# DegardinBruno/Kinetic-GAN

Measured on AMD Instinct MI355X. Metric: G+D train-step samples/sec, NTU (N,3,64,25) bs=64 at 1/2/4/8 MI355X, higher is better.
Workload: dtype f32; 1 GPU; ntu shapes (N,3,64,25), 60 classes, mlp4, G+D WGAN-GP iteration, 64 samples/GPU; global_batch=64, parallelism=dp1, launch=hipgraph

## Files before the change

### include/kgan_hip.h

```cpp
#ifndef KGAN_HIP_H
#define KGAN_HIP_H

#include <stdint.h>

#ifdef __cplusplus
extern "C" {
#endif

#define KG_ABI_VERSION 9

enum { KG_ACT_NONE = 0, KG_ACT_LRELU = 1, KG_ACT_TANH = 2 };
enum { KG_TAP_TIME = 0,
       KG_TAP_CHANBLOCK = 1  };

int         kg_abi_version(void);
const char* kg_arch(void);
const char* kg_last_error(void);
void        kg_reload_env(void);

typedef struct KgConvGroup {
    const float* x;  int64_t x_sN, x_sC;
    int32_t Cin, T_in, V_in;
    int32_t x_lead;
    const int32_t* vmap;
// ... 191 lines not shown
    const float* coef;
    const float* wg;  const float* wr;  const float* wt;  const float* b;  const float* u;
    KgPlane du, dr, gyc, zf, gx;
    KgPlane px, pu, pr;  const float* pnoise;  int32_t pact;
    const float* pmean_t;  const float* prstd_t;  const float* pgamma_t;
    const float* pmean_r;  const float* prstd_r;  const float* pgamma_r;
    float* pcoef;  float* dgamma_t;  float* dbeta_t;  float* dgamma_r;  float* dbeta_r;  float* dnw;
    float* ws;  int64_t ws_bytes;  int32_t* counters;  int32_t counters_len;
} KgGenBlockBwdArgs;
int64_t kg_genblock_lds_bytes(const KgGenBlockArgs* a);
int64_t kg_genblock_workspace_bytes(const KgGenBlockArgs* a);
int     kg_genblock_fwd(const KgGenBlockArgs* a, void* stream);
int64_t kg_genblock_bwd_lds_bytes(const KgGenBlockBwdArgs* a);
int64_t kg_genblock_bwd_workspace_bytes(const KgGenBlockBwdArgs* a);
int     kg_genblock_bwd(const KgGenBlockBwdArgs* a, void* stream);

typedef struct KgRowsumArgs {
    int32_t N, C, T, V;
    const float* x;  int64_t x_sN, x_sC;
    const float* y;  int64_t y_sN, y_sC;
    const float* shift;
    int32_t want_second;
    float* out;
    float* ws;  int64_t ws_bytes;
    int32_t accumulate;
    float* out2;
} KgRowsumArgs;

int64_t kg_rowsum_workspace_bytes(const KgRowsumArgs* a);
int     kg_rowsum(const KgRowsumArgs* a, void* stream);
int64_t kg_rowsum_many_workspace_bytes(const KgRowsumArgs* jobs, int32_t njobs);
int     kg_rowsum_many(const KgRowsumArgs* jobs, int32_t njobs, float* ws, int64_t ws_bytes, void* stream);

typedef struct KgEltArgs {
    int32_t N, C, T, V;
    const float* x;  int64_t x_sN, x_sC;
    const float* r;  int64_t r_sN, r_sC;
    const float* noise;
    const float* sx; const float* bx; const float* sr; const float* br; const float* nw;
    float* out;  int64_t o_sN, o_sC;
    int32_t act;  float slope;
    int32_t groups;
    int64_t coef_gs;
} KgEltArgs;

int kg_act_bwd(const KgEltArgs* a, void* stream);
int kg_affine_act(const KgEltArgs* a, void* stream);

typedef struct KgBnArgs {
    int32_t N, C, T, V;
    const float* x;  int64_t x_sN, x_sC;
    const float* g;  int64_t g_sN, g_sC;
    const float* gamma; const float* beta;
    float* running_mean; float* running_var;
    int64_t* num_batches_tracked;
    const float* mean; const float* rstd;
    float momentum, eps;
    int32_t training;
    float* coef;
} KgBnArgs;

int kg_bn_fwd(const KgBnArgs* a, void* stream);
int kg_bn_bwd(const KgBnArgs* a, void* stream);

typedef struct KgBnJob {
    KgBnArgs a;
    int32_t groups;
} KgBnJob;

int64_t kg_bn_bwd_many_workspace_bytes(const KgBnArgs* jobs, int32_t njobs);
int     kg_bn_bwd_many(const KgBnArgs* jobs, int32_t njobs, float* ws, int64_t ws_bytes, int32_t* counters,
                       int32_t counters_len, void* stream);
int64_t kg_bn_fwd_many_workspace_bytes(const KgBnJob* jobs, int32_t njobs);
int     kg_bn_fwd_many(const KgBnJob* jobs, int32_t njobs, float* ws, int64_t ws_bytes, int32_t* counters,
                       int32_t counters_len, void* stream);

typedef struct KgGpArgs {
    int32_t N, C, T, V;
    const float* g;  int64_t g_sN, g_sC;
    float* nrm;
    float* gp;
    const float* gout;
    float* out;  int64_t o_sN, o_sC;
} KgGpArgs;

int kg_gp_fwd(const KgGpArgs* a, void* stream);
int kg_gp_bwd(const KgGpArgs* a, void* stream);

int kg_adam_step(float* p, const float* g, float* m, float* v, int64_t n,
                 float lr, float b1, float b2, float eps, const int32_t* step, float grad_scale,
                 void* stream);
int kg_adam_step_fused(float* p, float* g, float* m, float* v, int64_t n,
                       float lr, float b1, float b2, float eps, const int32_t* step, float grad_scale,
                       int32_t zero_grad, void* stream);
int kg_adam_step_ema(float* p, float* g, float* m, float* v, float* e, int64_t n,
                     float lr, float b1, float b2, float eps, const int32_t* step, float grad_scale,
                     int32_t zero_grad, float ema_decay, float ema_warmup, void* stream);

typedef struct KgHeadArgs {
    int32_t N, C, T, V;
    const float* h;  int64_t h_sN, h_sC;
    const float* w;  const float* b;
    float* v;
    const float* gv;
    float* g;  int64_t g_sN, g_sC;
    float slope;  int32_t masked;
    float* dw;  float* db;  int32_t accumulate;
} KgHeadArgs;
int kg_head_fwd(const KgHeadArgs* a, void* stream);
int kg_head_bwd(const KgHeadArgs* a, void* stream);
int kg_head_wgrad(const KgHeadArgs* a, void* stream);

typedef struct KgLabelBiasArgs {
    int32_t N, L, J, K, C, V, W, T;
    const int64_t* labels;
    const float* emb;
    const float* w;  int64_t w_sK, w_sC;
    const float* ak;
    float* zl;
    const float* gz;  int64_t gz_sN, gz_sC;
    float* demb;  float* dw;  int32_t accumulate;
    float* dak;  int32_t dak_accumulate;
    float* ws;  int64_t ws_bytes;
} KgLabelBiasArgs;
int     kg_label_bias_fwd(const KgLabelBiasArgs* a, void* stream);
int64_t kg_label_bias_workspace_bytes(const KgLabelBiasArgs* a);
int     kg_label_bias_bwd(const KgLabelBiasArgs* a, void* stream);
int     kg_aggconv_label(const KgAggConvArgs* a, const KgLabelBiasArgs* lb, void* stream);

typedef struct KgMixArgs {
    int32_t N, C, T, V;
    const float* real;  int64_t r_sN, r_sC;
    const float* fake;  int64_t f_sN, f_sC;
    const float* alpha;
    float* out;  int64_t o_sN, o_sC;
} KgMixArgs;
int kg_mix3(const KgMixArgs* a, void* stream);

typedef struct KgMaskedAdjArgs {
    int32_t n;
    const float* a;  const float* imp;  const int64_t* sel;
    float* ak;
    const float* g;  float* dimp;  int32_t accumulate;
} KgMaskedAdjArgs;
int kg_masked_adj_fwd(const KgMaskedAdjArgs* a, void* stream);
int kg_masked_adj_bwd(const KgMaskedAdjArgs* a, void* stream);

typedef struct KgLinearArgs {
    int32_t N, Din, Dout;
    int32_t L, J;
    const float* x;  int64_t x_ld;
    const float* emb;
    const int64_t* labels;
    const float* w;  const float* bias;
    float* y;  int64_t y_ld;
    int32_t act;  float slope;
    const float* g;  int64_t g_ld;
    float* gx;  int64_t gx_ld;  int32_t gx_cols;
    float* dw;  float* db;
    float* demb;
    int32_t accumulate;
} KgLinearArgs;
int kg_linear_fwd(const KgLinearArgs* a, void* stream);
int kg_linear_bwd(const KgLinearArgs* a, void* stream);
int kg_embed_bwd(const KgLinearArgs* a, void* stream);

#define KG_COMM_ID_BYTES 128
int kg_comm_unique_id(void* id);
int kg_comm_init(void** comm, int32_t rank, int32_t world, const void* id, int32_t device);
int kg_comm_world(const void* comm);
int kg_allreduce_flat(void* comm, float* buf, int64_t n, void* stream);
int kg_comm_destroy(void* comm);

int kg_peak_mfma_f32(float* sink, int32_t iters, double* flops, void* stream);
int kg_peak_copy(const float* src, float* dst, int64_t n, void* stream);

#define KG_MMD_MAX_BW 16
typedef struct KgMmdArgs {
    const float* x;  int64_t x_sp, x_sd, x_sg, x_sc;
    const float* y;  int64_t y_sp, y_sd, y_sg, y_sc;
    int32_t m, n, dim;
    int32_t groups, classes;
    int32_t nbw;
    double bw[KG_MMD_MAX_BW];
    float* mmd2;
    float* mmd;
    float* result;
    float* mean;
    void* ws;  int64_t ws_bytes;
} KgMmdArgs;
int64_t kg_mmd_workspace_bytes(const KgMmdArgs* a);
int     kg_mmd(const KgMmdArgs* a, void* stream);

#define KG_PRDC_MAX_K 32
#define KG_PRDC_MAX_POINTS 32768
typedef struct KgPrdcArgs {
    const float* real;  int64_t r_sc, r_sp, r_so;
    const float* fake;  int64_t f_sc, f_sp, f_so;
    int32_t n, m;
    int32_t d_outer, d_inner;
    int32_t classes, k;
    float* radii_real;
    float* radii_fake;
    int32_t* fake_hits;
    uint8_t* real_flags;
    int32_t* counts;
    float* values;
    float* mean;
    void* ws;  int64_t ws_bytes;
} KgPrdcArgs;
int64_t kg_prdc_workspace_bytes(const KgPrdcArgs* a);
int     kg_prdc(const KgPrdcArgs* a, void* stream);

#define KG_PRDC_MAX_SETS 4
typedef struct KgPrdcRadiiArgs {
    const float* x;  int64_t sc, sp, so;
    int32_t n, d_outer, d_inner, classes, k;
    float* radii;
} KgPrdcRadiiArgs;
typedef struct KgPrdcSetsArgs {
    const float* real;  int64_t r_sc, r_sp, r_so;
    const float* fake[KG_PRDC_MAX_SETS];  int64_t f_sc, f_sp, f_so;
    int32_t nsets;
    int32_t n, m;
    int32_t d_outer, d_inner;
    int32_t classes, k;
    const float* radii_real;
    float* radii_fake;
    int32_t* fake_hits;
    uint8_t* real_flags;
    int32_t* counts;
    float* values;
    float* mean;
    void* ws;  int64_t ws_bytes;
} KgPrdcSetsArgs;
int     kg_prdc_radii(const KgPrdcRadiiArgs* a, void* stream);
int64_t kg_prdc_sets_workspace_bytes(const KgPrdcSetsArgs* a);
int     kg_prdc_sets(const KgPrdcSetsArgs* a, void* stream);

#define KG_NN_MAX_K 32
#define KG_NN_MAX_POINTS 16777216
#define KG_NN_MAX_SPLIT 32
typedef struct KgNnArgs {
    const float* query;  int64_t q_sc, q_sp, q_so;
// ... 221 lines not shown
```

### kinetic-gan_amd/_native.py

```python
from __future__ import annotations

import ctypes as C
import os
from typing import NamedTuple, Optional, Sequence, Tuple

import torch

_PKG = os.path.dirname(os.path.abspath(__file__))
LIB_PATH = os.environ.get("KG_LIB") or os.path.join(_PKG, "libkgan_hip.so")

ACT_NONE, ACT_LRELU, ACT_TANH = 0, 1, 2
ABI_VERSION = 9
TAP_TIME, TAP_CHANBLOCK = 0, 1

c_f32p = C.c_void_p
c_i32p = C.c_void_p


class _ConvGroup(C.Structure):
    _fields_ = [("x", c_f32p), ("x_sN", C.c_int64), ("x_sC", C.c_int64),
                ("Cin", C.c_int32), ("T_in", C.c_int32), ("V_in", C.c_int32),
                ("x_lead", C.c_int32),
                ("vmap", c_i32p),
                ("w", c_f32p), ("w_sT", C.c_int64), ("w_sO", C.c_int64), ("w_sI", C.c_int64),
# ... 39 lines not shown
    _fields_ = [("ws", c_f32p), ("dw", c_f32p), ("w_sT", C.c_int64), ("w_sO", C.c_int64), ("w_sI", C.c_int64),
                ("taps", C.c_int32), ("M", C.c_int32), ("Cin", C.c_int32), ("splits", C.c_int32),
                ("accumulate", C.c_int32)]


WGRAD_REDUCE_MAX_JOBS = 24
WGRAD_TILE_128x128, WGRAD_TILE_64x64, WGRAD_TILE_64x32, WGRAD_TILE_32x64, WGRAD_TILE_32x32 = 0, 1, 2, 3, 4
WGRAD_TILE_NAMES = {WGRAD_TILE_128x128: "128x128", WGRAD_TILE_64x64: "64x64", WGRAD_TILE_64x32: "64x32",
                    WGRAD_TILE_32x64: "32x64", WGRAD_TILE_32x32: "32x32"}
WGRAD_MAX_SPLITS = 128


class _WgradReduceJobs(C.Structure):
    _fields_ = [("njobs", C.c_int32), ("job", _WgradReduceJob * WGRAD_REDUCE_MAX_JOBS)]


class _AggArgs(C.Structure):
    _fields_ = [("N", C.c_int32), ("C", C.c_int32), ("K", C.c_int32), ("V", C.c_int32), ("W", C.c_int32),
                ("T", C.c_int32), ("rep", C.c_int32),
                ("a", c_f32p),
                ("x", c_f32p), ("x_sN", C.c_int64), ("x_sC", C.c_int64),
                ("y", c_f32p), ("y_sN", C.c_int64), ("y_sC", C.c_int64),
                ("out", c_f32p), ("o_sN", C.c_int64), ("o_sC", C.c_int64),
                ("ws", c_f32p), ("ws_bytes", C.c_int64), ("a_transposed", C.c_int32), ("defer_sum", C.c_int32),
                ("res", c_f32p), ("r_sN", C.c_int64), ("r_sC", C.c_int64), ("r_T", C.c_int32), ("r_V", C.c_int32),
                ("r_tstride", C.c_int32), ("r_inv", c_i32p),
                ("mask", c_f32p), ("m_sN", C.c_int64), ("m_sC", C.c_int64), ("slope", C.c_float)]


class _OuterSumJob(C.Structure):
    _fields_ = [("ws", c_f32p), ("out", c_f32p), ("nout", C.c_int32), ("slabs", C.c_int32)]


OUTER_SUM_MAX_JOBS = 16


class _OuterSumJobs(C.Structure):
    _fields_ = [("njobs", C.c_int32), ("job", _OuterSumJob * OUTER_SUM_MAX_JOBS)]


class _AggConvArgs(C.Structure):
    _fields_ = [("N", C.c_int32), ("Cin", C.c_int32), ("M", C.c_int32), ("T", C.c_int32), ("V", C.c_int32),
                ("W", C.c_int32), ("K", C.c_int32),
                ("x", c_f32p), ("x_sN", C.c_int64), ("x_sC", C.c_int64),
                ("a", c_f32p), ("a_transposed", C.c_int32),
                ("nbr", c_i32p), ("pcount", C.c_int32 * 3),
                ("w", c_f32p), ("w_sT", C.c_int64), ("w_sO", C.c_int64), ("w_sI", C.c_int64),
                ("out", c_f32p), ("o_sN", C.c_int64), ("o_sC", C.c_int64),
                ("add", c_f32p), ("a_sN", C.c_int64), ("a_sC", C.c_int64), ("a_tstride", C.c_int32),
                ("xa", c_f32p), ("xa_sN", C.c_int64), ("xa_sC", C.c_int64)]


class _RowsumArgs(C.Structure):
    _fields_ = [("N", C.c_int32), ("C", C.c_int32), ("T", C.c_int32), ("V", C.c_int32),
                ("x", c_f32p), ("x_sN", C.c_int64), ("x_sC", C.c_int64),
                ("y", c_f32p), ("y_sN", C.c_int64), ("y_sC", C.c_int64),
                ("shift", c_f32p),
                ("want_second", C.c_int32),
                ("out", c_f32p),
                ("ws", c_f32p), ("ws_bytes", C.c_int64), ("accumulate", C.c_int32), ("out2", c_f32p)]


class _BnArgs(C.Structure):
    _fields_ = [("N", C.c_int32), ("C", C.c_int32), ("T", C.c_int32), ("V", C.c_int32),
                ("x", c_f32p), ("x_sN", C.c_int64), ("x_sC", C.c_int64),
                ("g", c_f32p), ("g_sN", C.c_int64), ("g_sC", C.c_int64),
                ("gamma", c_f32p), ("beta", c_f32p),
                ("running_mean", c_f32p), ("running_var", c_f32p),
                ("num_batches_tracked", C.c_void_p),
                ("mean", c_f32p), ("rstd", c_f32p),
                ("momentum", C.c_float), ("eps", C.c_float),
                ("training", C.c_int32),
                ("coef", c_f32p)]


class _BnJob(C.Structure):
    _fields_ = [("a", _BnArgs), ("groups", C.c_int32)]


class _GpArgs(C.Structure):
    _fields_ = [("N", C.c_int32), ("C", C.c_int32), ("T", C.c_int32), ("V", C.c_int32),
                ("g", c_f32p), ("g_sN", C.c_int64), ("g_sC", C.c_int64),
                ("nrm", c_f32p), ("gp", c_f32p), ("gout", c_f32p),
                ("out", c_f32p), ("o_sN", C.c_int64), ("o_sC", C.c_int64)]


class _EltArgs(C.Structure):
    _fields_ = [("N", C.c_int32), ("C", C.c_int32), ("T", C.c_int32), ("V", C.c_int32),
                ("x", c_f32p), ("x_sN", C.c_int64), ("x_sC", C.c_int64),
                ("r", c_f32p), ("r_sN", C.c_int64), ("r_sC", C.c_int64),
                ("noise", c_f32p),
                ("sx", c_f32p), ("bx", c_f32p), ("sr", c_f32p), ("br", c_f32p), ("nw", c_f32p),
                ("out", c_f32p), ("o_sN", C.c_int64), ("o_sC", C.c_int64),
                ("act", C.c_int32), ("slope", C.c_float),
                ("groups", C.c_int32), ("coef_gs", C.c_int64)]


class _GenArgs(C.Structure):
    _fields_ = [("N", C.c_int32), ("C", C.c_int32), ("K", C.c_int32), ("Cr", C.c_int32), ("Tc", C.c_int32),
                ("Vc", C.c_int32), ("V", C.c_int32), ("rep", C.c_int32),
                ("a", c_f32p), ("u", c_f32p), ("b", c_f32p),
                ("y", c_f32p), ("y_out", c_f32p), ("y_sN", C.c_int64), ("y_sC", C.c_int64),
                ("z", c_f32p), ("z_sN", C.c_int64), ("z_sC", C.c_int64),
                ("zf", c_f32p), ("zf_sN", C.c_int64), ("zf_sC", C.c_int64),
                ("rs", c_f32p), ("rs_out", c_f32p), ("rs_sN", C.c_int64), ("rs_sC", C.c_int64),
                ("rbias", c_f32p),
                ("r", c_f32p), ("r_sN", C.c_int64), ("r_sC", C.c_int64)]


class _GenAdjJob(C.Structure):
    _fields_ = [("dbt", c_f32p), ("u", c_f32p), ("a", c_f32p), ("out", c_f32p),
                ("K", C.c_int32), ("Kd", C.c_int32), ("V", C.c_int32), ("Vc", C.c_int32), ("accumulate", C.c_int32)]


class _HeadArgs(C.Structure):
    _fields_ = [("N", C.c_int32), ("C", C.c_int32), ("T", C.c_int32), ("V", C.c_int32),
                ("h", c_f32p), ("h_sN", C.c_int64), ("h_sC", C.c_int64),
                ("w", c_f32p), ("b", c_f32p), ("v", c_f32p), ("gv", c_f32p),
                ("g", c_f32p), ("g_sN", C.c_int64), ("g_sC", C.c_int64),
                ("slope", C.c_float), ("masked", C.c_int32),
                ("dw", c_f32p), ("db", c_f32p), ("accumulate", C.c_int32)]


class _LinearArgs(C.Structure):
    _fields_ = [("N", C.c_int32), ("Din", C.c_int32), ("Dout", C.c_int32), ("L", C.c_int32), ("J", C.c_int32),
                ("x", c_f32p), ("x_ld", C.c_int64), ("emb", c_f32p), ("labels", C.c_void_p),
                ("w", c_f32p), ("bias", c_f32p), ("y", c_f32p), ("y_ld", C.c_int64),
                ("act", C.c_int32), ("slope", C.c_float),
                ("g", c_f32p), ("g_ld", C.c_int64),
                ("gx", c_f32p), ("gx_ld", C.c_int64), ("gx_cols", C.c_int32),
                ("dw", c_f32p), ("db", c_f32p), ("demb", c_f32p), ("accumulate", C.c_int32)]


class _LabelBiasArgs(C.Structure):
    _fields_ = [("N", C.c_int32), ("L", C.c_int32), ("J", C.c_int32), ("K", C.c_int32), ("C", C.c_int32),
                ("V", C.c_int32), ("W", C.c_int32), ("T", C.c_int32),
                ("labels", C.c_void_p), ("emb", c_f32p),
                ("w", c_f32p), ("w_sK", C.c_int64), ("w_sC", C.c_int64),
                ("ak", c_f32p), ("zl", c_f32p),
                ("gz", c_f32p), ("gz_sN", C.c_int64), ("gz_sC", C.c_int64),
                ("demb", c_f32p), ("dw", c_f32p), ("accumulate", C.c_int32),
                ("dak", c_f32p), ("dak_accumulate", C.c_int32),
                ("ws", c_f32p), ("ws_bytes", C.c_int64)]


class _MixArgs(C.Structure):
    _fields_ = [("N", C.c_int32), ("C", C.c_int32), ("T", C.c_int32), ("V", C.c_int32),
                ("real", c_f32p), ("r_sN", C.c_int64), ("r_sC", C.c_int64),
                ("fake", c_f32p), ("f_sN", C.c_int64), ("f_sC", C.c_int64),
                ("alpha", c_f32p),
                ("out", c_f32p), ("o_sN", C.c_int64), ("o_sC", C.c_int64)]


class _MaskedAdjArgs(C.Structure):
    _fields_ = [("n", C.c_int32), ("a", c_f32p), ("imp", c_f32p), ("sel", C.c_void_p), ("ak", c_f32p),
                ("g", c_f32p), ("dimp", c_f32p), ("accumulate", C.c_int32)]


class _GenTailArgs(C.Structure):
    _fields_ = [("N", C.c_int32), ("C", C.c_int32), ("T", C.c_int32), ("V", C.c_int32), ("act", C.c_int32), ("slope", C.c_float),
                ("g", c_f32p), ("g_sN", C.c_int64), ("g_sC", C.c_int64),
                ("out", c_f32p), ("o_sN", C.c_int64), ("o_sC", C.c_int64),
                ("u", c_f32p), ("u_sN", C.c_int64), ("u_sC", C.c_int64), ("mean_t", c_f32p), ("rstd_t", c_f32p), ("gamma_t", c_f32p),
                ("r", c_f32p), ("r_sN", C.c_int64), ("r_sC", C.c_int64), ("mean_r", c_f32p), ("rstd_r", c_f32p), ("gamma_r", c_f32p),
                ("noise", c_f32p), ("coef", c_f32p),
                ("dgamma_t", c_f32p), ("dbeta_t", c_f32p), ("dgamma_r", c_f32p), ("dbeta_r", c_f32p), ("dnw", c_f32p),
                ("ws", c_f32p), ("ws_bytes", C.c_int64), ("counters", C.c_void_p), ("counters_len", C.c_int32),
                ("du", c_f32p), ("du_sN", C.c_int64), ("du_sC", C.c_int64),
                ("dr", c_f32p), ("dr_sN", C.c_int64), ("dr_sC", C.c_int64)]


class _GenPrepJob(C.Structure):
    _fields_ = [("a", c_f32p), ("imp", c_f32p), ("u", c_f32p), ("aeff", c_f32p), ("b", c_f32p),
                ("K", C.c_int32), ("V", C.c_int32), ("Vc", C.c_int32)]


class _Plane(C.Structure):
    _fields_ = [("p", c_f32p), ("sN", C.c_int64), ("sC", C.c_int64)]


class _GenBnLayer(C.Structure):
    _fields_ = [("gamma", c_f32p), ("beta", c_f32p), ("running_mean", c_f32p), ("running_var", c_f32p),
                ("num_batches_tracked", C.c_void_p), ("momentum", C.c_float), ("eps", C.c_float), ("coef", c_f32p)]


class _GenBlockArgs(C.Structure):
    _fields_ = [("N", C.c_int32), ("groups", C.c_int32),
                ("Cin", C.c_int32), ("C", C.c_int32), ("K", C.c_int32), ("Kp", C.c_int32),
                ("Tc", C.c_int32), ("Vc", C.c_int32), ("T", C.c_int32), ("V", C.c_int32), ("rep", C.c_int32),
                ("res_kind", C.c_int32), ("bn_t", C.c_int32), ("act", C.c_int32), ("slope", C.c_float),
                ("x", _Plane),
                ("pu", _Plane), ("pr", _Plane), ("pcoef_t", c_f32p), ("pcoef_r", c_f32p), ("pnoise", c_f32p), ("pnw", c_f32p),
                ("pact", C.c_int32), ("xout", _Plane),
                ("wg", c_f32p), ("wr", c_f32p), ("br", c_f32p), ("wt", c_f32p), ("bt", c_f32p),
                ("b", c_f32p), ("u", c_f32p),
                ("yc", _Plane), ("z", _Plane), ("r", _Plane), ("uo", _Plane),
                ("bt_", _GenBnLayer), ("br_", _GenBnLayer),
                ("noise", c_f32p), ("nw", c_f32p), ("out", _Plane),
                ("ws", c_f32p), ("ws_bytes", C.c_int64), ("counters", C.c_void_p), ("counters_len", C.c_int32)]


class _GenBlockBwdArgs(C.Structure):
    _fields_ = [("N", C.c_int32),
                ("Cin", C.c_int32), ("C", C.c_int32), ("K", C.c_int32), ("Kp", C.c_int32),
                ("Tc", C.c_int32), ("Vc", C.c_int32), ("T", C.c_int32), ("V", C.c_int32), ("rep", C.c_int32),
                ("res_kind", C.c_int32), ("bn_t", C.c_int32), ("act", C.c_int32), ("slope", C.c_float),
                ("g", _Plane), ("out", _Plane), ("uo", _Plane), ("r", _Plane),
                ("coef", c_f32p),
                ("wg", c_f32p), ("wr", c_f32p), ("wt", c_f32p), ("b", c_f32p), ("u", c_f32p),
                ("du", _Plane), ("dr", _Plane), ("gyc", _Plane), ("zf", _Plane), ("gx", _Plane),
                ("px", _Plane), ("pu", _Plane), ("pr", _Plane), ("pnoise", c_f32p), ("pact", C.c_int32),
                ("pmean_t", c_f32p), ("prstd_t", c_f32p), ("pgamma_t", c_f32p),
                ("pmean_r", c_f32p), ("prstd_r", c_f32p), ("pgamma_r", c_f32p),
                ("pcoef", c_f32p), ("dgamma_t", c_f32p), ("dbeta_t", c_f32p), ("dgamma_r", c_f32p), ("dbeta_r", c_f32p),
                ("dnw", c_f32p),
                ("ws", c_f32p), ("ws_bytes", C.c_int64), ("counters", C.c_void_p), ("counters_len", C.c_int32)]



MMD_MAX_BW = 16


class _MmdArgs(C.Structure):
    _fields_ = [("x", c_f32p), ("x_sp", C.c_int64), ("x_sd", C.c_int64), ("x_sg", C.c_int64), ("x_sc", C.c_int64),
                ("y", c_f32p), ("y_sp", C.c_int64), ("y_sd", C.c_int64), ("y_sg", C.c_int64), ("y_sc", C.c_int64),
                ("m", C.c_int32), ("n", C.c_int32), ("dim", C.c_int32),
                ("groups", C.c_int32), ("classes", C.c_int32), ("nbw", C.c_int32),
                ("bw", C.c_double * MMD_MAX_BW),
                ("mmd2", c_f32p), ("mmd", c_f32p), ("result", c_f32p), ("mean", c_f32p),
                ("ws", C.c_void_p), ("ws_bytes", C.c_int64)]

PRDC_MAX_K = 32
PRDC_MAX_POINTS = 32768


class _PrdcArgs(C.Structure):
    _fields_ = [("real", c_f32p), ("r_sc", C.c_int64), ("r_sp", C.c_int64), ("r_so", C.c_int64),
                ("fake", c_f32p), ("f_sc", C.c_int64), ("f_sp", C.c_int64), ("f_so", C.c_int64),
                ("n", C.c_int32), ("m", C.c_int32), ("d_outer", C.c_int32), ("d_inner", C.c_int32),
# ... 1255 lines not shown

def rowsum_many(jobs: Sequence[dict]):
    lib = load_library()
    if not jobs:
        return
    arr = (_RowsumArgs * len(jobs))()
    held = []
    for i, j in enumerate(jobs):
        x = as_plane(j["x"])
        out, out2, y = j["out"], j.get("out2"), j.get("y")
        _need_cuda(x, out, out2)
        for o in (out, out2):
            if o is not None:
                _dest(o, x.shape[1], "rowsum_many: destinations must be contiguous fp32 vectors of C elements")
        _need_cuda(y)
        held.append(_rowsum_fill(arr[i], x, y, 0 if y is None else 2, out, out2, int(bool(j.get("accumulate", False)))))
    ws = _workspace("kg_rowsum_many_workspace_bytes", arr, jobs[0]["x"].device, len(jobs))
    _check(lib.kg_rowsum_many(arr, len(jobs), ws.data_ptr(), ws.numel() * 4, _stream()), "kg_rowsum_many")


def _elt_args(x, out, act, slope):
    a = _EltArgs()
    a.N, a.C, a.T, a.V = x.shape
    _bind(a, "x", "x", x)
    _bind(a, "out", "o", out)
    a.act, a.slope = act, slope
    return a


def act_bwd(g: torch.Tensor, ref: torch.Tensor, act: int, slope: float = 0.2) -> torch.Tensor:
    lib = load_library()
    g = as_plane(g)
    ref = as_plane(ref)
    _need_cuda(g, ref)
    out = new_plane(*g.shape, g.device)
    a = _elt_args(g, out, act, slope)
    _bind(a, "r", "r", ref)
    _check(lib.kg_act_bwd(C.byref(a), _stream()), "kg_act_bwd")
    return out


def affine_act(x, sx=None, bx=None, r=None, sr=None, br=None, noise=None, nw=None,
               act: int = ACT_NONE, slope: float = 0.2, out: Optional[torch.Tensor] = None,
               groups: int = 1, coef_gs: int = 0) -> torch.Tensor:
    lib = load_library()
    x = as_plane(x)
    vecs = [None if t is None else t.reshape(-1).contiguous() for t in (sx, bx, sr, br, nw)]
    _need_cuda(x, r, noise, out, *vecs)
    if out is None:
        out = new_plane(*x.shape, x.device)
    elif tuple(out.shape) != tuple(x.shape) or not is_plane(out) or out.dtype != torch.float32:
        raise ValueError("affine_act: out must be a plane tensor of x's shape")
    a = _elt_args(x, out, act, slope)
    if r is not None:
        r = _bind(a, "r", "r", r, True)
    if noise is not None:
        noise = noise.contiguous()
        a.noise = noise.data_ptr()
    a.sx, a.bx, a.sr, a.br, a.nw = [_ptr(t) for t in vecs]
    a.groups, a.coef_gs = int(groups), int(coef_gs)
    _check(lib.kg_affine_act(C.byref(a), _stream()), "kg_affine_act")
    return out


def _gp_args(g):
    a = _GpArgs()
    a.N, a.C, a.T, a.V = g.shape
    _bind(a, "g", "g", g)
    return a


def gp_fwd(g: torch.Tensor):
    lib = load_library()
    g = as_plane(g)
    _need_cuda(g)
    a = _gp_args(g)
    nrm = torch.empty(g.shape[0], dtype=torch.float32, device=g.device)
    gp = torch.empty((), dtype=torch.float32, device=g.device)
    a.nrm, a.gp = nrm.data_ptr(), gp.data_ptr()
    _check(lib.kg_gp_fwd(C.byref(a), _stream()), "kg_gp_fwd")
    return nrm, gp


def gp_bwd(g: torch.Tensor, nrm: torch.Tensor, gout: torch.Tensor) -> torch.Tensor:
    lib = load_library()
    g = as_plane(g)
    gout = gout.reshape(1).contiguous()
    _need_cuda(g, nrm, gout)
    a = _gp_args(g)
    a.nrm, a.gout = nrm.data_ptr(), gout.data_ptr()
    out = _bind(a, "out", "o", new_plane(*g.shape, g.device))
    _check(lib.kg_gp_bwd(C.byref(a), _stream()), "kg_gp_bwd")
    return out


def _vec(t: Optional[torch.Tensor], c: int, what: str):
    return None if t is None else _dest(t, c, f"{what}: expected a contiguous fp32 vector of {c} elements")


def _bn_fwd_fill(a, who: str, x, gamma, beta, running_mean, running_var, nbt, momentum, eps, training, groups: Optional[int] = None):
    n, c, t, v = x.shape
    vecs = [_vec(q, c, who) for q in (gamma, beta, running_mean, running_var)]
    _need_cuda(x, *vecs, nbt)
    a.N, a.C, a.T, a.V = n // (groups or 1), c, t, v
    _bind(a, "x", "x", x)
    a.gamma, a.beta, a.running_mean, a.running_var = [_ptr(q) for q in vecs]
    if nbt is not None:
        assert nbt.dtype == torch.int64
        a.num_batches_tracked = nbt.data_ptr()
    a.momentum, a.eps, a.training = float(momentum), float(eps), int(bool(training))
    coef = torch.empty((4, c) if groups is None else (groups, 4, c), dtype=torch.float32, device=x.device)
    a.coef = coef.data_ptr()
    return coef


def bn_fwd(x: torch.Tensor, gamma, beta, running_mean, running_var, num_batches_tracked, training: bool,
           momentum: float, eps: float) -> torch.Tensor:
    lib = load_library()
    x = as_plane(x)
    a = _BnArgs()
    coef = _bn_fwd_fill(a, "bn_fwd", x, gamma, beta, running_mean, running_var, num_batches_tracked, momentum, eps, training)
    _check(lib.kg_bn_fwd(C.byref(a), _stream()), "kg_bn_fwd")
    return coef


def _bn_many(who: str, arr, coefs):
    total_c = sum(cf.shape[-1] for cf in coefs)
    if total_c > SYNC_LEN:
        raise ValueError("%s: %d channels exceed the %d ticket counters" % (who, total_c, SYNC_LEN))
    ws = _workspace("kg_%s_workspace_bytes" % who, arr, coefs[0].device if coefs else None, len(arr))
    sync = _sync_buffer(coefs[0].device)
    _check(getattr(load_library(), "kg_" + who)(arr, len(arr), ws.data_ptr(), ws.numel() * 4, sync.data_ptr(), sync.numel(),
                                               _stream()), "kg_" + who)
    return coefs


def bn_fwd_many(jobs: Sequence[dict]):
    arr = (_BnJob * len(jobs))()
    xs, coefs = [], []
    for i, j in enumerate(jobs):
        x = as_plane(j["x"])
        groups = int(j.get("groups", 1))
        if x.shape[0] % groups:
            raise ValueError("bn_fwd_many: N=%d is not a multiple of groups=%d" % (x.shape[0], groups))
        coefs.append(_bn_fwd_fill(arr[i].a, "bn_fwd_many", x, j.get("gamma"), j.get("beta"), j.get("running_mean"),
                                  j.get("running_var"), j.get("num_batches_tracked"), j["momentum"], j["eps"], True, groups))
        arr[i].groups = groups
        xs.append(x)
    return _bn_many("bn_fwd_many", arr, coefs)


def _bn_bwd_fill(a, who: str, g, x, gamma, mean, rstd, training):
    g, x = as_plane(g), as_plane(x)
    n, c, t, v = x.shape
    gamma, mean, rstd = _vec(gamma, c, who), _vec(mean, c, who), _vec(rstd, c, who)
    _need_cuda(g, x, gamma, mean, rstd)
    a.N, a.C, a.T, a.V = n, c, t, v
    _bind(a, "x", "x", x)
    _bind(a, "g", "g", g)
    a.gamma, a.mean, a.rstd = _ptr(gamma), _ptr(mean), _ptr(rstd)
    a.training = int(bool(training))
    coef = torch.empty((5, c), dtype=torch.float32, device=x.device)
    a.coef = coef.data_ptr()
    return coef, (g, x)


def bn_bwd(g: torch.Tensor, x: torch.Tensor, gamma, mean: torch.Tensor, rstd: torch.Tensor, training: bool) -> torch.Tensor:
    lib = load_library()
    a = _BnArgs()
    coef, held = _bn_bwd_fill(a, "bn_bwd", g, x, gamma, mean, rstd, training)
    _check(lib.kg_bn_bwd(C.byref(a), _stream()), "kg_bn_bwd")
    return coef


def bn_bwd_many(jobs: Sequence[dict]):
    arr = (_BnArgs * len(jobs))()
    filled = [_bn_bwd_fill(arr[i], "bn_bwd_many", j["g"], j["x"], j.get("gamma"), j["mean"], j["rstd"], j["training"])
              for i, j in enumerate(jobs)]
    return _bn_many("bn_bwd_many", arr, [coef for coef, _ in filled])


def adam_step(p, g, m, v, lr, b1, b2, eps, step_t: torch.Tensor, grad_scale: float = 1.0, zero_grad: bool = False):
    lib = load_library()
    _need_cuda(p, g, m, v, step_t)
    assert p.is_contiguous() and g.is_contiguous() and m.is_contiguous() and v.is_contiguous()
    assert step_t.dtype == torch.int32
    if zero_grad:
        _check(lib.kg_adam_step_fused(p.data_ptr(), g.data_ptr(), m.data_ptr(), v.data_ptr(), p.numel(), lr, b1, b2, eps,
                                      step_t.data_ptr(), grad_scale, 1, _stream()), "kg_adam_step_fused")
        return
    _check(lib.kg_adam_step(p.data_ptr(), g.data_ptr(), m.data_ptr(), v.data_ptr(), p.numel(),
                            lr, b1, b2, eps, step_t.data_ptr(), grad_scale, _stream()), "kg_adam_step")


def adam_step_ema(p, g, m, v, e, lr, b1, b2, eps, step_t: torch.Tensor, grad_scale: float, zero_grad: bool, decay: float,
                  warmup: float):
    lib = load_library()
    _need_cuda(p, g, m, v, e, step_t)
    assert p.is_contiguous() and g.is_contiguous() and m.is_contiguous() and v.is_contiguous() and e.is_contiguous()
    assert g.numel() == m.numel() == v.numel() == e.numel() == p.numel() and e.dtype == torch.float32
    assert step_t.dtype == torch.int32
    _check(lib.kg_adam_step_ema(p.data_ptr(), g.data_ptr(), m.data_ptr(), v.data_ptr(), e.data_ptr(), p.numel(), lr, b1, b2, eps,
                                step_t.data_ptr(), grad_scale, 1 if zero_grad else 0, decay, warmup, _stream()),
           "kg_adam_step_ema")



def _head_args(h, w=None, gv=None):
    a = _HeadArgs()
    h = _bind(a, "h", "h", h, True)
    a.N, a.C, a.T, a.V = h.shape
    if w is not None:
        w = w.reshape(-1)
        assert w.is_contiguous() and w.numel() == h.shape[1]
        a.w = w.data_ptr()
    if gv is not None:
        assert gv.numel() == h.shape[0]
        a.gv = gv.data_ptr()
    return a, h


def head_fwd(h: torch.Tensor, w: torch.Tensor, b: Optional[torch.Tensor]) -> torch.Tensor:
    lib = load_library()
    _need_cuda(h, w, b)
    a, h = _head_args(h, w)
    a.b = _ptr(b)
    v = torch.empty(h.shape[0], dtype=torch.float32, device=h.device)
    a.v = v.data_ptr()
    _check(lib.kg_head_fwd(C.byref(a), _stream()), "kg_head_fwd")
    return v


def head_bwd(gv: torch.Tensor, w: torch.Tensor, h: torch.Tensor, masked: bool = True, slope: float = 0.2) -> torch.Tensor:
    lib = load_library()
    gv = gv.reshape(-1).contiguous()
    _need_cuda(gv, w, h)
    a, h = _head_args(h, w, gv)
    a.masked, a.slope = int(bool(masked)), slope
    g = _bind(a, "g", "g", new_plane(*h.shape, h.device))
    _check(lib.kg_head_bwd(C.byref(a), _stream()), "kg_head_bwd")
    return g


def head_wgrad(x: torch.Tensor, gv: torch.Tensor, dw: torch.Tensor, db: Optional[torch.Tensor], accumulate: bool = True):
    lib = load_library()
    gv = gv.reshape(-1).contiguous()
    _need_cuda(x, gv, dw, db)
    a, x = _head_args(x, None, gv)
    assert dw.is_contiguous() and dw.numel() == x.shape[1] and (db is None or db.numel() == 1)
    a.dw, a.db, a.accumulate = dw.data_ptr(), _ptr(db), int(bool(accumulate))
    _check(lib.kg_head_wgrad(C.byref(a), _stream()), "kg_head_wgrad")



def _cls_head_args(n: int, c: int, t: int, v: int, f: int, l: int, slope: float = 0.2) -> _ClsHeadArgs:
    a = _ClsHeadArgs()
    a.N, a.C, a.T, a.V, a.F, a.L, a.slope = int(n), int(c), int(t), int(v), int(f), int(l), float(slope)
    return a


def _cls_flat(t: torch.Tensor, n: int, dtype, what: str) -> torch.Tensor:
    if t.numel() != n or not t.is_contiguous() or t.dtype != dtype:
        raise ValueError(f"kg_cls_head: {what} must be contiguous {dtype} of {n} elements")
    return t


def cls_head_workspace_bytes(n: int, c: int, t: int, v: int, f: int, l: int) -> int:
    return _query("kg_cls_head_workspace_bytes", _cls_head_args(n, c, t, v, f, l))


def cls_head_fwd(h: torch.Tensor, w1: torch.Tensor, b1: torch.Tensor, w2: torch.Tensor, b2: torch.Tensor,
                 labels: Optional[torch.Tensor] = None, slope: float = 0.2, feat_out: Optional[torch.Tensor] = None,
                 pred_out: Optional[torch.Tensor] = None) -> dict:
    lib = load_library()
    _need_cuda(h, w1, b1, w2, b2, labels, feat_out, pred_out)
    f, l = w1.shape[0], w2.shape[0]
    a = _cls_head_args(*h.shape, f, l, slope)
    h = _bind(a, "h", "h", h, True)
    n, c = h.shape[0], h.shape[1]
    a.w1, a.b1 = _cls_flat(w1, f * c, torch.float32, "w1").data_ptr(), _cls_flat(b1, f, torch.float32, "b1").data_ptr()
    a.w2, a.b2 = _cls_flat(w2, l * f, torch.float32, "w2").data_ptr(), _cls_flat(b2, l, torch.float32, "b2").data_ptr()
    dev = h.device
    if feat_out is not None and tuple(feat_out.shape) != (n, f):
        raise ValueError(f"kg_cls_head: feat_out must be ({n}, {f}), got {tuple(feat_out.shape)}")
    if pred_out is not None and tuple(pred_out.shape) != (n,):
        raise ValueError(f"kg_cls_head: pred_out must be ({n},), got {tuple(pred_out.shape)}")
    out = dict(pooled=torch.empty((n, c), dtype=torch.float32, device=dev),
               feat=torch.empty((n, f), dtype=torch.float32, device=dev) if feat_out is None
               else _cls_flat(feat_out, n * f, torch.float32, "feat_out"),
               logits=torch.empty((n, l), dtype=torch.float32, device=dev),
               pred=torch.empty(n, dtype=torch.int32, device=dev) if pred_out is None
               else _cls_flat(pred_out, n, torch.int32, "pred_out"),
               loss_per_sample=None, loss=None, correct=None)
    a.pooled, a.feat, a.logits, a.pred = (out[k].data_ptr() for k in ("pooled", "feat", "logits", "pred"))
    if labels is not None:
        a.labels = _cls_flat(labels, n, torch.int64, "labels").data_ptr()
        out["loss_per_sample"] = torch.empty(n, dtype=torch.float32, device=dev)
        out["loss"] = torch.empty((), dtype=torch.float32, device=dev)
        out["correct"] = torch.empty((), dtype=torch.int32, device=dev)
        a.loss_per_sample, a.loss, a.correct = (out[k].data_ptr() for k in ("loss_per_sample", "loss", "correct"))
    _check(lib.kg_cls_head_fwd(C.byref(a), _stream()), "kg_cls_head_fwd")
    return out


def cls_head_bwd(gtop: torch.Tensor, h: torch.Tensor, w1: torch.Tensor, w2: torch.Tensor, labels: torch.Tensor,
                 feat: torch.Tensor, logits: torch.Tensor, masked: bool = True, slope: float = 0.2):
    lib = load_library()
    _need_cuda(gtop, h, w1, w2, labels, feat, logits)
    f, l = w1.shape[0], w2.shape[0]
    a = _cls_head_args(*h.shape, f, l, slope)
    h = _bind(a, "h", "h", h, True)
    n, c = h.shape[0], h.shape[1]
    a.w1, a.w2 = _cls_flat(w1, f * c, torch.float32, "w1").data_ptr(), _cls_flat(w2, l * f, torch.float32, "w2").data_ptr()
    a.labels = _cls_flat(labels, n, torch.int64, "labels").data_ptr()
    a.feat, a.logits = _cls_flat(feat, n * f, torch.float32, "feat").data_ptr(), _cls_flat(logits, n * l, torch.float32, "logits").data_ptr()
    a.gtop, a.masked = _cls_flat(gtop, 1, torch.float32, "gtop").data_ptr(), int(bool(masked))
    g = _bind(a, "g", "g", new_plane(*h.shape, h.device))
    ws = _workspace("kg_cls_head_workspace_bytes", a, h.device)
    _check(lib.kg_cls_head_bwd(C.byref(a), _stream()), "kg_cls_head_bwd")
    return g, ws

# ... 16 lines not shown

def cls_scores(feats: Sequence[torch.Tensor], preds: Sequence[torch.Tensor], labels: torch.Tensor, div_pairs: torch.Tensor,
               mm_pairs: torch.Tensor, n_classes: int) -> dict:
    lib = load_library()
    feats, preds, k = list(feats), list(preds), int(n_classes)
    s = len(feats)
    if len(preds) != s:
        raise ValueError(f"kg_cls_scores: {s} feature sets, {len(preds)} prediction vectors")
    if not 1 <= s <= CLS_MAX_SETS:
        raise ValueError(f"kg_cls_scores: nsets={s} outside [1, {CLS_MAX_SETS}]")
    _need_cuda(labels, div_pairs, mm_pairs, *feats, *preds)
    n, f = feats[0].shape
    ld = feats[0].stride(0) if n > 1 else max(f, feats[0].stride(0))
    for t in feats:
        if t.dtype != torch.float32 or tuple(t.shape) != (n, f) or (f > 1 and t.stride(1) != 1) or (n > 1 and t.stride(0) != ld):
            raise ValueError(f"kg_cls_scores: every feature set must be fp32 ({n}, {f}) with unit column stride and row stride {ld}")
    preds = [_cls_flat(t, n, torch.int32, "pred") for t in preds]
    labels = _cls_flat(labels, n, torch.int64, "labels")
    if div_pairs.dim() != 2 or div_pairs.shape[1] != 2 or mm_pairs.dim() != 2 or mm_pairs.shape[1] != 2 \
            or mm_pairs.shape[0] % max(k, 1):
        raise ValueError("kg_cls_scores: div_pairs (Sd, 2) and mm_pairs (n_classes * Sl, 2) expected")
    sd, sl = div_pairs.shape[0], mm_pairs.shape[0] // max(k, 1)
    div_pairs = _cls_flat(div_pairs, 2 * sd, torch.int32, "div_pairs")
    mm_pairs = _cls_flat(mm_pairs, 2 * k * sl, torch.int32, "mm_pairs")
    dev = feats[0].device
    out = dict(scores=torch.empty((s, 3), dtype=torch.float32, device=dev),
               scores64=torch.empty((s, 3), dtype=torch.float64, device=dev),
               correct=torch.empty(s, dtype=torch.int32, device=dev),
               correct_per_class=torch.empty((s, max(k, 1)), dtype=torch.int32, device=dev),
               count_per_class=torch.empty(max(k, 1), dtype=torch.int32, device=dev),
               dist=torch.empty((s, max(1, sd + k * sl)), dtype=torch.float64, device=dev))
    a = _ClsScoresArgs()
    a.nsets, a.N, a.F, a.K, a.Sd, a.Sl, a.feat_ld = s, n, f, k, sd, sl, ld
    for g in range(s):
        a.feat[g], a.pred[g] = feats[g].data_ptr(), preds[g].data_ptr()
    a.labels, a.div_pairs, a.mm_pairs = labels.data_ptr(), div_pairs.data_ptr(), mm_pairs.data_ptr()
    for key in ("dist", "scores64", "scores", "correct", "correct_per_class", "count_per_class"):
        setattr(a, key, out[key].data_ptr())
    _count("kg_cls_scores", 3.0 * s * (sd + k * sl) * f)
    _check(lib.kg_cls_scores(C.byref(a), _stream()), "kg_cls_scores")
    return out


def _label_bias_args(labels, emb, wg, K, C_out, cin, J, ak):
    a = _LabelBiasArgs()
    k, v, w = ak.shape
    assert k == K and ak.is_contiguous() and emb.is_contiguous() and labels.dtype == torch.int64 and labels.is_contiguous()
    a.N, a.L, a.J, a.K, a.C, a.V, a.W = labels.numel(), emb.shape[0], J, K, C_out, v, w
    a.labels, a.emb = labels.data_ptr(), emb.data_ptr()
    assert wg.is_contiguous()
    a.w, a.w_sK, a.w_sC = wg.data_ptr(), C_out * cin, cin
    a.ak = ak.data_ptr()
    return a


def label_bias_fwd(labels, emb, wg, K: int, C_out: int, cin: int, J: int, ak) -> torch.Tensor:
    lib = load_library()
    _need_cuda(labels, emb, wg, ak)
    a = _label_bias_args(labels, emb, wg, K, C_out, cin, J, ak)
    zl = torch.empty((labels.numel(), C_out, 1, ak.shape[2]), dtype=torch.float32, device=emb.device)
    a.zl = zl.data_ptr()
    ws = _workspace("kg_label_bias_workspace_bytes", a, emb.device)
    _check(lib.kg_label_bias_fwd(C.byref(a), _stream()), "kg_label_bias_fwd")
    return zl


def label_bias_bwd(gz, labels, emb, wg, K: int, C_out: int, cin: int, J: int, ak, demb=None, dw=None, dak=None,
                   accumulate: bool = True, dak_accumulate: bool = True):
    lib = load_library()
    gz = as_plane(gz)
    _need_cuda(gz, labels, emb, wg, ak, demb, dw, dak)
    a = _label_bias_args(labels, emb, wg, K, C_out, cin, J, ak)
    assert gz.shape[0] == labels.numel() and gz.shape[1] == C_out and gz.shape[3] == ak.shape[2]
    a.T = gz.shape[2]
    _bind(a, "gz", "gz", gz)
    for t in (demb, dw, dak):
        assert t is None or t.is_contiguous()
    a.demb, a.dw, a.dak = _ptr(demb), _ptr(dw), _ptr(dak)
    a.accumulate, a.dak_accumulate = int(bool(accumulate)), int(bool(dak_accumulate))
    ws = _workspace("kg_label_bias_workspace_bytes", a, gz.device)
    _check(lib.kg_label_bias_bwd(C.byref(a), _stream()), "kg_label_bias_bwd")


def mix3(real: torch.Tensor, fake: torch.Tensor, alpha: torch.Tensor) -> torch.Tensor:
    lib = load_library()
    real, fake = as_plane(real), as_plane(fake)
    alpha = alpha.reshape(-1).contiguous()
    _need_cuda(real, fake, alpha)
    n, c, t, v = real.shape
    assert tuple(fake.shape) == (n, c, t, v) and alpha.numel() == n
    out = torch.empty((3 * n, c, t, v), dtype=torch.float32, device=real.device)
    a = _MixArgs()
    a.N, a.C, a.T, a.V = n, c, t, v
    _bind(a, "real", "r", real)
    _bind(a, "fake", "f", fake)
    a.alpha = alpha.data_ptr()
    a.out, a.o_sN, a.o_sC = out.data_ptr(), c * t * v, t * v
    _check(lib.kg_mix3(C.byref(a), _stream()), "kg_mix3")
    return out


def masked_adj_fwd(A_all: torch.Tensor, imp_all: Optional[torch.Tensor], sel: Optional[torch.Tensor]) -> torch.Tensor:
    lib = load_library()
    _need_cuda(A_all, imp_all, sel)
    n = sel.numel() if sel is not None else A_all.numel()
    ak = torch.empty(n, dtype=torch.float32, device=A_all.device)
    a = _MaskedAdjArgs()
    a.n = n
    a.a, a.imp, a.sel, a.ak = A_all.data_ptr(), _ptr(imp_all), _ptr(sel), ak.data_ptr()
    assert A_all.is_contiguous() and (imp_all is None or imp_all.is_contiguous()) and (sel is None or (sel.dtype == torch.int64 and sel.is_contiguous()))
    _check(lib.kg_masked_adj_fwd(C.byref(a), _stream()), "kg_masked_adj_fwd")
    return ak


def masked_adj_bwd(g: torch.Tensor, A_all: torch.Tensor, sel: Optional[torch.Tensor], dimp: torch.Tensor, accumulate: bool):
    lib = load_library()
    g = g.reshape(-1).contiguous()
    _need_cuda(g, A_all, sel, dimp)
    a = _MaskedAdjArgs()
    a.n = g.numel()
    assert dimp.is_contiguous() and dimp.numel() == A_all.numel() and (sel is None or sel.numel() == g.numel())
    a.a, a.sel, a.g, a.dimp, a.accumulate = A_all.data_ptr(), _ptr(sel), g.data_ptr(), dimp.data_ptr(), int(bool(accumulate))
    _check(lib.kg_masked_adj_bwd(C.byref(a), _stream()), "kg_masked_adj_bwd")



def _linear_args(x, w, emb, labels):
    a = _LinearArgs()
    assert w.dim() == 2 and w.is_contiguous()
    a.Dout, a.Din = w.shape
    a.w = w.data_ptr()
    J = 0
    if emb is not None:
        assert emb.dim() == 2 and emb.is_contiguous() and labels is not None and labels.dtype == torch.int64 and labels.is_contiguous()
        a.L, J = emb.shape
        a.emb, a.labels = emb.data_ptr(), labels.data_ptr()
    a.J = J
    assert x.dim() == 2 and x.stride(1) == 1 and x.shape[1] == a.Din - J, (tuple(x.shape), a.Din, J)
    a.N = x.shape[0]
    a.x, a.x_ld = x.data_ptr(), x.stride(0)
    return a


def linear_fwd(x: torch.Tensor, w: torch.Tensor, b: Optional[torch.Tensor], act: int = ACT_LRELU, slope: float = 0.2,
               emb: Optional[torch.Tensor] = None, labels: Optional[torch.Tensor] = None) -> torch.Tensor:
    lib = load_library()
    _need_cuda(x, w, b, emb, labels)
    a = _linear_args(x, w, emb, labels)
    y = torch.empty(a.N, a.Dout, dtype=torch.float32, device=x.device)
    a.bias = _ptr(b)
    a.y, a.y_ld = y.data_ptr(), a.Dout
    a.act, a.slope = act, slope
    _check(lib.kg_linear_fwd(C.byref(a), _stream()), "kg_linear_fwd")
    return y


def linear_bwd(g: torch.Tensor, y: torch.Tensor, x: torch.Tensor, w: torch.Tensor, act: int = ACT_LRELU, slope: float = 0.2,
               emb: Optional[torch.Tensor] = None, labels: Optional[torch.Tensor] = None, gx_cols: Optional[int] = None,
               dw: Optional[torch.Tensor] = None, db: Optional[torch.Tensor] = None, accumulate: bool = False):
    lib = load_library()
    _need_cuda(g, y, x, w, emb, labels, dw, db)
    a = _linear_args(x, w, emb, labels)
    assert g.shape == (a.N, a.Dout) and y.shape == (a.N, a.Dout) and g.stride(1) == 1 and y.stride(1) == 1
    a.g, a.g_ld = g.data_ptr(), g.stride(0)
    a.y, a.y_ld = y.data_ptr(), y.stride(0)
    a.act, a.slope = act, slope
    cols = a.Din if gx_cols is None else gx_cols
    gx = None
    if cols > 0:
        gx = torch.empty(a.N, cols, dtype=torch.float32, device=g.device)
        a.gx, a.gx_ld = gx.data_ptr(), cols
    a.gx_cols = cols
    if dw is not None:
        assert dw.is_contiguous() and dw.numel() == a.Dout * a.Din
    if db is not None:
        assert db.is_contiguous() and db.numel() == a.Dout
    a.dw, a.db, a.accumulate = _ptr(dw), _ptr(db), int(bool(accumulate))
    _check(lib.kg_linear_bwd(C.byref(a), _stream()), "kg_linear_bwd")
    return gx


def embed_bwd(gx: torch.Tensor, labels: torch.Tensor, demb: torch.Tensor, accumulate: bool = False):
    lib = load_library()
    _need_cuda(gx, labels, demb)
    a = _LinearArgs()
    assert gx.dim() == 2 and gx.stride(1) == 1 and demb.dim() == 2 and demb.is_contiguous() and demb.shape[1] <= gx.shape[1]
    assert labels.dtype == torch.int64 and labels.is_contiguous()
    a.N = gx.shape[0]
    a.L, a.J = demb.shape
    a.gx, a.gx_ld = gx.data_ptr(), gx.stride(0)
    a.labels, a.demb, a.accumulate = labels.data_ptr(), demb.data_ptr(), int(bool(accumulate))
    _check(lib.kg_embed_bwd(C.byref(a), _stream()), "kg_embed_bwd")



COMM_ID_BYTES = 128



class MmdView(NamedTuple):
    t: torch.Tensor
    sp: int
    sd: int
    sg: int
    sc: int


def _mmd_extent_ok(v: MmdView, m: int, dim: int, groups: int, classes: int) -> bool:
    if min(v.sp, v.sd, v.sg, v.sc) < 0:
        return False
    last = (classes - 1) * v.sc + (groups - 1) * v.sg + (m - 1) * v.sp + (dim - 1) * v.sd
    return v.t.storage_offset() + last < v.t.untyped_storage().nbytes() // 4


def mmd(x: MmdView, y: MmdView, m: int, n: int, dim: int, groups: int, classes: int,
        bandwidths: Sequence[float], want_mean: bool = False) -> dict:
    lib = load_library()
    for v in (x, y):
        if v.t.dtype != torch.float32:
            raise TypeError(f"kg_mmd: fp32 only, got {v.t.dtype}")
    _need_cuda(x.t, y.t)
    bws = [float(b) for b in bandwidths]
    a = _MmdArgs()
    a.x, a.x_sp, a.x_sd, a.x_sg, a.x_sc = x.t.data_ptr(), x.sp, x.sd, x.sg, x.sc
    a.y, a.y_sp, a.y_sd, a.y_sg, a.y_sc = y.t.data_ptr(), y.sp, y.sd, y.sg, y.sc
    a.m, a.n, a.dim, a.groups, a.classes, a.nbw = int(m), int(n), int(dim), int(groups), int(classes), len(bws)
    for i, b in enumerate(bws[:MMD_MAX_BW]):
        a.bw[i] = b
    nbytes = _query("kg_mmd_workspace_bytes", a)
    for name, v, p in (("x", x, m), ("y", y, n)):
        if not _mmd_extent_ok(v, p, dim, groups, classes):
            raise ValueError(f"kg_mmd: the strides of {name} reach outside its tensor")
    dev = x.t.device
    ws = torch.empty(max(1, nbytes // 4), dtype=torch.float32, device=dev)
    out = dict(mmd2=torch.empty((classes * groups, len(bws)), dtype=torch.float32, device=dev),
               mmd=torch.empty((classes, len(bws)), dtype=torch.float32, device=dev),
               result=torch.empty(classes, dtype=torch.float32, device=dev),
# ... 655 lines not shown
```

### kinetic-gan_amd/csrc/kg_disc.hip

```cpp
#include "kg_common.h"

namespace {

constexpr int NT = 256;

__device__ __forceinline__ float wave_sum(float v) {
#pragma unroll
    for (int off = 32; off > 0; off >>= 1) v += __shfl_down(v, off, 64);
    return v;
}

__device__ __forceinline__ float block_sum(float s, float* red) {
    s = wave_sum(s);
    __syncthreads();
    if ((threadIdx.x & 63) == 0) red[threadIdx.x >> 6] = s;
    __syncthreads();
    float t = 0.f;
    if (threadIdx.x == 0)
        for (int i = 0; i < NT / 64; ++i) t += red[i];
    return t;
}

__global__ __launch_bounds__(NT) void kg_head_fwd_kernel(const KgHeadArgs a) {
    __shared__ float red[NT / 64];
    const int n = blockIdx.x, L = a.T * a.V;
    const float* base = a.h + (long)n * a.h_sN;
    float s = 0.f;
    for (int e = threadIdx.x; e < a.C * L; e += NT) {
        const int c = e / L, r = e - c * L;
        s = fmaf(a.w[c], base[(long)c * a.h_sC + r], s);
    }
    const float t = block_sum(s, red);
    if (threadIdx.x == 0) a.v[n] = t / (float)L + (a.b ? a.b[0] : 0.f);
}

__global__ __launch_bounds__(NT) void kg_head_bwd_kernel(const KgHeadArgs a) {
    const int L = a.T * a.V;
    const long total = (long)a.N * a.C * L;
    const float inv = 1.f / (float)L;
    for (long i = (long)blockIdx.x * NT + threadIdx.x; i < total; i += (long)gridDim.x * NT) {
        const int c = (int)(i / ((long)a.N * L));
        const long rem = i - (long)c * a.N * L;
        const int n = (int)(rem / L), r = (int)(rem - (long)n * L);
        float v = a.gv[n] * a.w[c] * inv;
        if (a.masked) v *= a.h[(long)n * a.h_sN + (long)c * a.h_sC + r] > 0.f ? 1.f : a.slope;
        a.g[(long)n * a.g_sN + (long)c * a.g_sC + r] = v;
    }
}

__global__ __launch_bounds__(NT) void kg_head_wgrad_kernel(const KgHeadArgs a) {
    __shared__ float red[NT / 64];
    const int c = blockIdx.x, L = a.T * a.V;
    float s = 0.f;
    if (c < a.C) {
        for (int e = threadIdx.x; e < a.N * L; e += NT) {
            const int n = e / L, r = e - n * L;
            s = fmaf(a.gv[n], a.h[(long)n * a.h_sN + (long)c * a.h_sC + r], s);
        }
        const float t = block_sum(s, red);
        if (threadIdx.x == 0) a.dw[c] = (a.accumulate ? a.dw[c] : 0.f) + t / (float)L;
    } else {
        for (int n = threadIdx.x; n < a.N; n += NT) s += a.gv[n];
        const float t = block_sum(s, red);
        if (threadIdx.x == 0 && a.db) a.db[0] = (a.accumulate ? a.db[0] : 0.f) + t;
    }
}

constexpr int LB_MAXKW = 3 * 32, LB_MAXKC = 3 * 64, LB_MAXCW = 64 * 32, LB_MAXW = 12288;

__device__ __forceinline__ void colsums(const KgLabelBiasArgs& a, float* S, float* scratch) {
    const int n = a.K * a.V * a.W;
    for (int i = threadIdx.x; i < n; i += NT) scratch[i] = a.ak[i];
    __syncthreads();
    for (int i = threadIdx.x; i < a.K * a.W; i += NT) {
        const int k = i / a.W, w = i - k * a.W;
        float s = 0.f;
        for (int v = 0; v < a.V; ++v) s += scratch[(k * a.V + v) * a.W + w];
        S[i] = s;
    }
    __syncthreads();
}

__device__ __forceinline__ void stage_wc(const KgLabelBiasArgs& a, float* Wl) {
    const int lane = threadIdx.x & 63, wave = threadIdx.x >> 6;
    const int rows = a.K * a.C;
    for (int r0 = wave * 4; r0 < rows; r0 += (NT / 64) * 4) {
        for (int j0 = 0; j0 < a.J; j0 += 64) {
            const int j = j0 + lane;
            float v[4];
#pragma unroll
            for (int q = 0; q < 4; ++q) {
                const int kc = r0 + q;
                const int k = kc / a.C, c = kc - k * a.C;
                v[q] = (kc < rows && j < a.J) ? a.w[(long)k * a.w_sK + (long)c * a.w_sC + j] : 0.f;
            }
#pragma unroll
            for (int q = 0; q < 4; ++q)
                if (r0 + q < rows && j < a.J) Wl[(r0 + q) * a.J + j] = v[q];
        }
    }
}

__global__ __launch_bounds__(NT) void kg_label_bias_table_kernel(const KgLabelBiasArgs a, float* table) {
    __shared__ float S[LB_MAXKW], P[LB_MAXKC], El[512], Wl[LB_MAXW];
    const int l = blockIdx.x;
    colsums(a, S, Wl);
    stage_wc(a, Wl);
    for (int j = threadIdx.x; j < a.J; j += NT) El[j] = a.emb[(long)l * a.J + j];
    __syncthreads();
    for (int i = threadIdx.x; i < a.K * a.C; i += NT) {
        const float* wp = Wl + i * a.J;
        float s0 = 0.f, s1 = 0.f, s2 = 0.f, s3 = 0.f;
        int j = 0;
        for (; j + 3 < a.J; j += 4) {
            s0 = fmaf(wp[j], El[j], s0);
            s1 = fmaf(wp[j + 1], El[j + 1], s1);
            s2 = fmaf(wp[j + 2], El[j + 2], s2);
            s3 = fmaf(wp[j + 3], El[j + 3], s3);
        }
        for (; j < a.J; ++j) s0 = fmaf(wp[j], El[j], s0);
        P[i] = (s0 + s1) + (s2 + s3);
    }
    __syncthreads();
    for (int i = threadIdx.x; i < a.C * a.W; i += NT) {
        const int c = i / a.W, w = i - c * a.W;
        float s = 0.f;
        for (int k = 0; k < a.K; ++k) s = fmaf(S[k * a.W + w], P[k * a.C + c], s);
        table[(long)l * a.C * a.W + i] = s;
    }
}

__global__ __launch_bounds__(NT) void kg_label_bias_lookup_kernel(const KgLabelBiasArgs a, const float* table) {
    const int CW = a.C * a.W;
    const int i = blockIdx.x * NT + threadIdx.x;
    if (i >= a.N * CW) return;
    const int n = i / CW, e = i - n * CW;
    const long lab = a.labels[n];
    a.zl[i] = (lab >= 0 && lab < a.L) ? table[lab * CW + e] : __builtin_nanf("");
}

__host__ __device__ __forceinline__ long lb_rec(const KgLabelBiasArgs& a) { return 2L * a.K * a.C + (long)a.C * a.W; }

constexpr int LB_BATCH = 4;

__global__ __launch_bounds__(NT) void kg_label_bias_bwd_class_kernel(const KgLabelBiasArgs a) {
    __shared__ float S[LB_MAXKW], El[512], Wr[3 * 512], red[LB_BATCH][NT], dT[NT], Pk[3];
    __shared__ int lst[NT], wcnt[NT / 64];
    extern __shared__ float kg_lbsm[];
// ... 76 lines not shown
        rec[tid * a.C + c] = s;
        rec[a.K * a.C + tid * a.C + c] = Pk[tid];
    }
}

__global__ __launch_bounds__(NT) void kg_label_bias_bwd_finish_kernel(const KgLabelBiasArgs a) {
    extern __shared__ float kg_lbsm[];
    const int b = blockIdx.x, tid = threadIdx.x;
    const long per = lb_rec(a);
    if (b < a.L) {
        if (!a.demb) return;
        float* Wl = kg_lbsm;
        __shared__ float Q[LB_MAXKC];
        stage_wc(a, Wl);
        for (int i = tid; i < a.K * a.C; i += NT) Q[i] = a.ws[b * per + i];
        __syncthreads();
        for (int j = tid; j < a.J; j += NT) {
            float s = 0.f;
#pragma unroll 8
            for (int i = 0; i < a.K * a.C; ++i) s = fmaf(Wl[i * a.J + j], Q[i], s);
            float* d = a.demb + (long)b * a.J + j;
            *d = (a.accumulate ? *d : 0.f) + s;
        }
        return;
    }
    if (b < a.L + a.K * a.W) {
        if (!a.dak) return;
        __shared__ float R[NT];
        __shared__ float tot;
        const int kw = b - a.L;
        const int k = kw / a.W, w = kw - k * a.W;
        float s = 0.f;
        for (int l0 = 0; l0 < a.L; l0 += NT) {
            const int l = l0 + tid;
            if (l < a.L) {
                const float* rec = a.ws + l * per;
                float r = 0.f;
#pragma unroll 8
                for (int c = 0; c < a.C; ++c) r = fmaf(rec[2 * a.K * a.C + c * a.W + w], rec[a.K * a.C + k * a.C + c], r);
                R[tid] = r;
            }
            __syncthreads();
            if (tid == 0) {
                const int nl = a.L - l0 < NT ? a.L - l0 : NT;
                for (int i = 0; i < nl; ++i) s += R[i];
            }
            __syncthreads();
        }
        if (tid == 0) tot = s;
        __syncthreads();
        for (int v = tid; v < a.V; v += NT) {
            float* d = a.dak + ((long)k * a.V + v) * a.W + w;
            *d = (a.dak_accumulate ? *d : 0.f) + tot;
        }
        return;
    }
    const int i = (b - a.L - a.K * a.W) * NT + tid;
    if (!a.dw || i >= a.K * a.C * a.J) return;
    const int kc = i / a.J, j = i - kc * a.J;
    float s = 0.f;
#pragma unroll 8
    for (int l = 0; l < a.L; ++l) s = fmaf(a.emb[(long)l * a.J + j], a.ws[l * per + kc], s);
    const int k = kc / a.C, c = kc - k * a.C;
    float* d = a.dw + (long)k * a.w_sK + (long)c * a.w_sC + j;
    *d = (a.accumulate ? *d : 0.f) + s;
}

__global__ __launch_bounds__(NT) void kg_mix3_kernel(const KgMixArgs a) {
    const int L = a.T * a.V;
    const long per = (long)a.C * L;
    const long total = (long)a.N * per;
    for (long i = (long)blockIdx.x * NT + threadIdx.x; i < total; i += (long)gridDim.x * NT) {
        const int n = (int)(i / per);
        const long rem = i - (long)n * per;
        const int c = (int)(rem / L), r = (int)(rem - (long)c * L);
        const float x = a.real[(long)n * a.r_sN + (long)c * a.r_sC + r];
        const float f = a.fake[(long)n * a.f_sN + (long)c * a.f_sC + r];
        const float al = a.alpha[n];
        float* o = a.out + (long)c * a.o_sC + r;
        o[(long)n * a.o_sN] = x;
        o[(long)(n + a.N) * a.o_sN] = f;
        o[(long)(n + 2 * a.N) * a.o_sN] = al * x + (1.f - al) * f;
    }
}

__global__ __launch_bounds__(NT) void kg_masked_adj_kernel(const KgMaskedAdjArgs a, const int backward) {
    const int i = blockIdx.x * NT + threadIdx.x;
    if (i >= a.n) return;
    const long s = a.sel ? a.sel[i] : i;
    if (!backward) {
        a.ak[i] = a.a[s] * (a.imp ? a.imp[s] : 1.f);
    } else {
        const float v = a.g[i] * a.a[s];
        a.dimp[s] = (a.accumulate ? a.dimp[s] : 0.f) + v;
    }
}

int validate_head(const KgHeadArgs* a, const char* who) {
    KG_REQUIRE(a != nullptr, "%s: null args", who);
    KG_REQUIRE(a->N > 0 && a->C > 0 && a->T > 0 && a->V > 0, "%s: bad dims", who);
    KG_REQUIRE((long)a->N * a->C * a->T * a->V < (1L << 31), "%s: too large", who);
    return 0;
}

int validate_lb(const KgLabelBiasArgs* a, const char* who) {
    KG_REQUIRE(a != nullptr, "%s: null args", who);
    KG_REQUIRE(a->N > 0 && a->L > 0 && a->J > 0 && a->K >= 1 && a->K <= 3 && a->C > 0 && a->V > 0 && a->W > 0, "%s: bad dims", who);
    KG_REQUIRE(a->K * a->W <= LB_MAXKW && a->K * a->C <= LB_MAXKC && a->C * a->W <= LB_MAXCW && a->J <= 512 &&
               a->K * a->C * a->J <= LB_MAXW && a->W <= NT && a->K * a->V * a->W <= LB_MAXW,
               "%s: K=%d C=%d W=%d J=%d exceed the kernel's LDS tables", who, a->K, a->C, a->W, a->J);
    KG_REQUIRE(a->labels && a->emb && a->w && a->ak, "%s: null pointer", who);
    return 0;
}

}

extern "C" int kg_head_fwd(const KgHeadArgs* a, void* stream) {
    if (int rc = validate_head(a, "kg_head_fwd")) return rc;
    KG_REQUIRE(a->h && a->w && a->v, "kg_head_fwd: null pointer");
    hipLaunchKernelGGL(kg_head_fwd_kernel, dim3(a->N), dim3(NT), 0, (hipStream_t)stream, *a);
    return kg_launch_status("kg_head_fwd");
}

extern "C" int kg_head_bwd(const KgHeadArgs* a, void* stream) {
    if (int rc = validate_head(a, "kg_head_bwd")) return rc;
    KG_REQUIRE(a->gv && a->w && a->g && (!a->masked || a->h), "kg_head_bwd: null pointer");
    const long total = (long)a->N * a->C * a->T * a->V;
    long grid = (total + NT - 1) / NT;
    if (grid > 4096) grid = 4096;
    hipLaunchKernelGGL(kg_head_bwd_kernel, dim3((int)grid), dim3(NT), 0, (hipStream_t)stream, *a);
    return kg_launch_status("kg_head_bwd");
}

extern "C" int kg_head_wgrad(const KgHeadArgs* a, void* stream) {
    if (int rc = validate_head(a, "kg_head_wgrad")) return rc;
    KG_REQUIRE(a->gv && a->h && a->dw, "kg_head_wgrad: null pointer");
    hipLaunchKernelGGL(kg_head_wgrad_kernel, dim3(a->C + 1), dim3(NT), 0, (hipStream_t)stream, *a);
    return kg_launch_status("kg_head_wgrad");
}

extern "C" int kg_label_bias_fwd(const KgLabelBiasArgs* a, void* stream) {
    if (int rc = validate_lb(a, "kg_label_bias_fwd")) return rc;
    KG_REQUIRE(a->zl, "kg_label_bias_fwd: null zl");
    KG_REQUIRE(a->ws && a->ws_bytes >= (int64_t)a->L * a->C * a->W * (int64_t)sizeof(float),
               "kg_label_bias_fwd: workspace too small (kg_label_bias_workspace_bytes)");
    hipLaunchKernelGGL(kg_label_bias_table_kernel, dim3(a->L), dim3(NT), 0, (hipStream_t)stream, *a, a->ws);
    if (int rc = kg_launch_status("kg_label_bias_fwd (class table)")) return rc;
    hipLaunchKernelGGL(kg_label_bias_lookup_kernel, dim3(kg_cdiv((long)a->N * a->C * a->W, NT)), dim3(NT), 0, (hipStream_t)stream,
                       *a, (const float*)a->ws);
    return kg_launch_status("kg_label_bias_fwd (lookup)");
}

extern "C" int64_t kg_label_bias_workspace_bytes(const KgLabelBiasArgs* a) {
    if (validate_lb(a, "kg_label_bias_workspace_bytes")) return -1;
    const int64_t bwd = (int64_t)a->L * lb_rec(*a);
    const int64_t fwd = (int64_t)a->L * a->C * a->W;
    return (bwd > fwd ? bwd : fwd) * (int64_t)sizeof(float);
}

extern "C" int kg_label_bias_bwd(const KgLabelBiasArgs* a, void* stream) {
    if (int rc = validate_lb(a, "kg_label_bias_bwd")) return rc;
    KG_REQUIRE(a->gz && a->T > 0, "kg_label_bias_bwd: null gz");
    KG_REQUIRE(a->ws && a->ws_bytes >= kg_label_bias_workspace_bytes(a), "kg_label_bias_bwd: workspace too small");
    KG_REQUIRE((long)a->L * a->C < (1L << 31), "kg_label_bias_bwd: L * C too large");
    static unsigned long long attr_mask = 0;
    if (kg_first_on_device(attr_mask)) {
        KG_SET_DYN_LDS(kg_label_bias_bwd_class_kernel, LB_MAXW * sizeof(float));
        KG_SET_DYN_LDS(kg_label_bias_bwd_finish_kernel, LB_MAXW * sizeof(float));
    }
    hipLaunchKernelGGL(kg_label_bias_bwd_class_kernel, dim3(a->L * a->C), dim3(NT), (size_t)a->K * a->V * a->W * sizeof(float),
                       (hipStream_t)stream, *a);
    if (int rc = kg_launch_status("kg_label_bias_bwd (classes)")) return rc;
    const int blocks = a->L + a->K * a->W + kg_cdiv((long)a->K * a->C * a->J, NT);
    hipLaunchKernelGGL(kg_label_bias_bwd_finish_kernel, dim3(blocks), dim3(NT), (size_t)a->K * a->C * a->J * sizeof(float),
                       (hipStream_t)stream, *a);
    return kg_launch_status("kg_label_bias_bwd (finish)");
}

extern "C" int kg_mix3(const KgMixArgs* a, void* stream) {
    KG_REQUIRE(a != nullptr && a->N > 0 && a->C > 0 && a->T > 0 && a->V > 0, "kg_mix3: bad dims");
    KG_REQUIRE(a->real && a->fake && a->alpha && a->out, "kg_mix3: null pointer");
    const long total = (long)a->N * a->C * a->T * a->V;
    long grid = (total + NT - 1) / NT;
    if (grid > 4096) grid = 4096;
    hipLaunchKernelGGL(kg_mix3_kernel, dim3((int)grid), dim3(NT), 0, (hipStream_t)stream, *a);
    return kg_launch_status("kg_mix3");
}

extern "C" int kg_masked_adj_fwd(const KgMaskedAdjArgs* a, void* stream) {
    KG_REQUIRE(a != nullptr && a->n > 0 && a->a && a->ak, "kg_masked_adj_fwd: bad args");
    hipLaunchKernelGGL(kg_masked_adj_kernel, dim3(kg_cdiv(a->n, NT)), dim3(NT), 0, (hipStream_t)stream, *a, 0);
    return kg_launch_status("kg_masked_adj_fwd");
}

extern "C" int kg_masked_adj_bwd(const KgMaskedAdjArgs* a, void* stream) {
    KG_REQUIRE(a != nullptr && a->n > 0 && a->a && a->g && a->dimp, "kg_masked_adj_bwd: bad args");
    hipLaunchKernelGGL(kg_masked_adj_kernel, dim3(kg_cdiv(a->n, NT)), dim3(NT), 0, (hipStream_t)stream, *a, 1);
    return kg_launch_status("kg_masked_adj_bwd");
}
```

### kinetic-gan_amd/csrc/kg_map.hip

```cpp
#include "kg_common.h"

namespace {

constexpr int NTM = 1024;
constexpr int NWV = 16;
constexpr int NJB = 6;
constexpr int NJA = 5;
constexpr unsigned OOB = 0x80000000u;
typedef float kg_f32x4 __attribute__((ext_vector_type(4)));
typedef float kg_f32x2 __attribute__((ext_vector_type(2)));

__device__ __forceinline__ __amdgpu_buffer_rsrc_t rsrc_of(const void* p, long bytes) {
    return __builtin_amdgcn_make_buffer_rsrc(kg_uniform_ptr(p), 0, p ? (int)(bytes > 0x7fffffffL ? 0x7fffffffL : bytes) : 0, 0x00020000);
}
__device__ __forceinline__ float load1(__amdgpu_buffer_rsrc_t r, unsigned off) {
    return __builtin_bit_cast(float, __builtin_amdgcn_raw_buffer_load_b32(r, off, 0, 0));
}

template <int VW>
__device__ __forceinline__ void load_vec(__amdgpu_buffer_rsrc_t r, unsigned off, float (&v)[VW]) {
    if constexpr (VW == 4) {
        const kg_f32x4 t = __builtin_bit_cast(kg_f32x4, __builtin_amdgcn_raw_buffer_load_b128(r, off, 0, 0));
        v[0] = t[0]; v[1] = t[1]; v[2] = t[2]; v[3] = t[3];
    } else if constexpr (VW == 2) {
        const kg_f32x2 t = __builtin_bit_cast(kg_f32x2, __builtin_amdgcn_raw_buffer_load_b64(r, off, 0, 0));
        v[0] = t[0]; v[1] = t[1];
    } else {
        v[0] = load1(r, off);
    }
}
template <int VW>
__device__ __forceinline__ void mask_tail(float (&v)[VW], int k, int len) {
    if (k + VW > len) {
#pragma unroll
        for (int t = 0; t < VW; ++t)
            if (k + t >= len) v[t] = 0.f;
    }
}

__device__ __forceinline__ float reduce_rows(const kg_f32x16& acc, float* red, int wave, int lane) {
#pragma unroll
    for (int r = 0; r < 16; ++r) red[(wave * 16 + r) * 64 + lane] = acc[r];
    __syncthreads();
    float v = 0.f;
#pragma unroll
    for (int w = 0; w < NWV; ++w) v += red[(w * 16 + wave) * 64 + lane];
    return v;
}
__device__ __forceinline__ int row_of_reg(int r, int h) { return (r & 3) + 8 * (r >> 2) + 4 * h; }

template <int VW>
__device__ __forceinline__ void load_xin(const KgLinearArgs& a, __amdgpu_buffer_rsrc_t rx, __amdgpu_buffer_rsrc_t re, int n, long lab, int k,
                                         bool ok, float (&v)[VW]) {
    const bool in_emb = k < a.J;
    const unsigned off_x = (unsigned)((long)n * a.x_ld + (k - a.J)) * 4u;
    const unsigned off_e = (unsigned)(lab * a.J + k) * 4u;
    load_vec<VW>(in_emb ? re : rx, (ok && k < a.Din) ? (in_emb ? off_e : off_x) : OOB, v);
    mask_tail<VW>(v, k, a.Din);
}

template <int VW>
__global__ __launch_bounds__(NTM) void kg_linear_fwd_kernel(const KgLinearArgs a) {
    __shared__ float red[NWV * 16 * 64];
    const int tid = threadIdx.x, lane = tid & 63, wave = tid >> 6;
    const int l32 = lane & 31, h = lane >> 5;
    const int o0 = blockIdx.x * 32, n0 = blockIdx.y * 32;
    const __amdgpu_buffer_rsrc_t rx = rsrc_of(a.x, (long)a.N * a.x_ld * 4), re = rsrc_of(a.emb, (long)a.L * a.J * 4);
    const __amdgpu_buffer_rsrc_t rw = rsrc_of(a.w, (long)a.Dout * a.Din * 4), rb = rsrc_of(a.bias, (long)a.Dout * 4);
    const int n = n0 + l32, o = o0 + l32;
    const bool n_ok = n < a.N, o_ok = o < a.Dout;
    const float bias = load1(rb, o_ok ? (unsigned)o * 4u : OOB);
    long lab = 0;
    if (a.J > 0 && n_ok) {
        lab = a.labels[n];
        if (lab < 0 || lab >= a.L) lab = -1;
    }
    kg_f32x16 acc;
#pragma unroll
    for (int r = 0; r < 16; ++r) acc[r] = 0.f;
    constexpr int CH = 2 * VW;
    const int nch = (a.Din + CH - 1) / CH;
    for (int c0 = wave; c0 < nch; c0 += NWV * NJB) {
        float av[NJB][VW], bv[NJB][VW];
#pragma unroll
        for (int j = 0; j < NJB; ++j) {
            const int c = c0 + NWV * j;
            const int k = c * CH + VW * h;
            const bool live = c < nch;
            load_xin<VW>(a, rx, re, n, lab < 0 ? 0 : lab, k, live && n_ok, av[j]);
            load_vec<VW>(rw, (live && o_ok && k < a.Din) ? (unsigned)((long)o * a.Din + k) * 4u : OOB, bv[j]);
            mask_tail<VW>(bv[j], k, a.Din);
            if (lab < 0 && k < a.J) {
#pragma unroll
                for (int t = 0; t < VW; ++t) av[j][t] = __builtin_nanf("");
            }
        }
#pragma unroll
        for (int j = 0; j < NJB; ++j)
#pragma unroll
            for (int t = 0; t < VW; ++t) acc = __builtin_amdgcn_mfma_f32_32x32x2f32(av[j][t], bv[j][t], acc, 0, 0, 0);
    }
    const float v = reduce_rows(acc, red, wave, lane);
    const int nn = n0 + row_of_reg(wave, h);
    if (o_ok && nn < a.N) a.y[(long)nn * a.y_ld + o] = kg_act(v + bias, a.act, a.slope);
}

template <int VW>
__global__ __launch_bounds__(NTM) void kg_linear_bwd_kernel(const KgLinearArgs a, int nwg_a, int itiles_a, int igroups_b) {
    __shared__ float red[NWV * 16 * 64];
    const int tid = threadIdx.x, lane = tid & 63, wave = tid >> 6;
    const int l32 = lane & 31, h = lane >> 5;
    const __amdgpu_buffer_rsrc_t rg = rsrc_of(a.g, (long)a.N * a.g_ld * 4), ry = rsrc_of(a.y, (long)a.N * a.y_ld * 4);
    kg_f32x16 acc;
#pragma unroll
    for (int r = 0; r < 16; ++r) acc[r] = 0.f;
    const float slope = a.slope;
    const bool lrelu = a.act == KG_ACT_LRELU;
    auto dact = [&](float gv, float yv) { return (lrelu && !(yv > 0.f)) ? gv * slope : gv; };
    if ((int)blockIdx.x < nwg_a) {
        const int it = blockIdx.x % itiles_a, nt = blockIdx.x / itiles_a;
        const int n0 = nt * 32, i0 = it * 32;
        const __amdgpu_buffer_rsrc_t rw = rsrc_of(a.w, (long)a.Dout * a.Din * 4);
        const int n = n0 + l32, i = i0 + l32;
        const bool n_ok = n < a.N, i_ok = i < a.gx_cols;
        constexpr int CH = 2 * VW;
        const int nch = (a.Dout + CH - 1) / CH;
        for (int c0 = wave; c0 < nch; c0 += NWV * NJA) {
            float gv[NJA][VW], yv[NJA][VW], bv[NJA][VW];
#pragma unroll
            for (int j = 0; j < NJA; ++j) {
                const int c = c0 + NWV * j;
                const int k = c * CH + VW * h;
                const bool live = c < nch && k < a.Dout;
                load_vec<VW>(rg, (live && n_ok) ? (unsigned)((long)n * a.g_ld + k) * 4u : OOB, gv[j]);
                load_vec<VW>(ry, (live && n_ok) ? (unsigned)((long)n * a.y_ld + k) * 4u : OOB, yv[j]);
#pragma unroll
                for (int t = 0; t < VW; ++t)
                    bv[j][t] = load1(rw, (live && i_ok && k + t < a.Dout) ? (unsigned)((long)(k + t) * a.Din + i) * 4u : OOB);
            }
#pragma unroll
            for (int j = 0; j < NJA; ++j) {
                const int k = (c0 + NWV * j) * CH + VW * h;
#pragma unroll
                for (int t = 0; t < VW; ++t) {
                    const float av = k + t < a.Dout ? dact(gv[j][t], yv[j][t]) : 0.f;
                    acc = __builtin_amdgcn_mfma_f32_32x32x2f32(av, bv[j][t], acc, 0, 0, 0);
                }
            }
        }
        const float v = reduce_rows(acc, red, wave, lane);
        const int nn = n0 + row_of_reg(wave, h);
        if (i_ok && nn < a.N) a.gx[(long)nn * a.gx_ld + i] = v;
        return;
    }
    const int wg = (int)blockIdx.x - nwg_a;
    const int ot = wg / igroups_b, ig = wg - ot * igroups_b;
    const int itl = wave & 3, kg = wave >> 2;
    const int o0 = ot * 32, i0 = (ig * 4 + itl) * 32;
    const __amdgpu_buffer_rsrc_t rx = rsrc_of(a.x, (long)a.N * a.x_ld * 4), re = rsrc_of(a.emb, (long)a.L * a.J * 4);
    const int o = o0 + l32, i = i0 + l32;
    const bool o_ok = o < a.Dout, i_ok = i < a.Din;
    const bool from_emb = i < a.J;
    float bsum = 0.f;
    const int npairs = (a.N + 1) / 2;
    for (int s0 = kg; s0 < npairs; s0 += 4 * NJB) {
        float gv[NJB], yv[NJB], xv[NJB];
        long lab[NJB];
        if (from_emb) {
#pragma unroll
            for (int j = 0; j < NJB; ++j) {
                const int n = 2 * (s0 + 4 * j) + h;
                lab[j] = n < a.N ? (long)a.labels[n] : -1;
            }
        }
#pragma unroll
        for (int j = 0; j < NJB; ++j) {
            const int n = 2 * (s0 + 4 * j) + h;
            const bool n_ok = n < a.N;
            gv[j] = load1(rg, (n_ok && o_ok) ? (unsigned)((long)n * a.g_ld + o) * 4u : OOB);
            yv[j] = load1(ry, (n_ok && o_ok) ? (unsigned)((long)n * a.y_ld + o) * 4u : OOB);
            if (from_emb) xv[j] = load1(re, (n_ok && lab[j] >= 0 && lab[j] < a.L) ? (unsigned)(lab[j] * a.J + i) * 4u : OOB);
            else          xv[j] = load1(rx, (n_ok && i_ok) ? (unsigned)((long)n * a.x_ld + (i - a.J)) * 4u : OOB);
        }
#pragma unroll
        for (int j = 0; j < NJB; ++j) {
            const float av = dact(gv[j], yv[j]);
            bsum += av;
// ... 121 lines not shown
```

### kinetic-gan_amd/csrc/kg_misc.hip

```cpp
#include <stdarg.h>
#include <stdio.h>

#include "kg_bn_math.h"
#include "kg_common.h"
#include "kg_handoff.h"

static thread_local char kg_err_buf[512] = "";

void kg_set_error(const char* fmt, ...) {
    va_list ap;
    va_start(ap, fmt);
    vsnprintf(kg_err_buf, sizeof(kg_err_buf), fmt, ap);
    va_end(ap);
}

extern "C" const char* kg_last_error(void) { return kg_err_buf; }

#include <stdlib.h>
static int kg_env_tri(const char* name) {
    const char* e = getenv(name);
    if (e && e[0] == '0') return 0;
    if (e && e[0] == '1') return 1;
    return -1;
}
// ... 618 lines not shown
    BnMany m;
    int64_t wsf = 0;
    int nc = 0;
    if (int rc = bn_many_layout(jobs, njobs, &m, &wsf, &nc)) return rc;
    KG_REQUIRE(ws != nullptr && ws_bytes >= wsf * (int64_t)sizeof(float), "kg_bn_fwd_many: workspace too small");
    KG_REQUIRE(counters != nullptr && counters_len >= nc, "kg_bn_fwd_many: %d zeroed counters needed", nc);
    m.ws = ws;
    m.counters = counters;
    hipLaunchKernelGGL(kg_bn_fwd_many_kernel, dim3(m.beg[njobs]), dim3(NT), 0, (hipStream_t)stream, m);
    return kg_launch_status("kg_bn_fwd_many");
}

extern "C" int kg_bn_bwd(const KgBnArgs* a, void* stream) {
    if (int rc = validate_bn(a, "kg_bn_bwd")) return rc;
    KG_REQUIRE(a->g && a->mean && a->rstd, "kg_bn_bwd: null pointer");
    if ((long)a->N * a->T * a->V >= 16384)
        hipLaunchKernelGGL(kg_bn_bwd_kernel<1024>, dim3(a->C), dim3(1024), 0, (hipStream_t)stream, *a);
    else
        hipLaunchKernelGGL(kg_bn_bwd_kernel<256>, dim3(a->C), dim3(256), 0, (hipStream_t)stream, *a);
    return kg_launch_status("kg_bn_bwd");
}

static int bn_bwd_many_layout(const KgBnArgs* jobs, int32_t njobs, BnBwdMany* m, int64_t* ws_floats, int* ncounters) {
    KG_REQUIRE(jobs != nullptr && njobs >= 1 && njobs <= BN_MANY_MAX, "kg_bn_bwd_many: 1..%d jobs", BN_MANY_MAX);
    long wg = 0, wsf = 0;
    int cb = 0;
    for (int i = 0; i < njobs; ++i) {
        const KgBnArgs* a = &jobs[i];
        if (int rc = validate_bn(a, "kg_bn_bwd_many")) return rc;
        KG_REQUIRE(!m || (a->g && a->mean && a->rstd), "kg_bn_bwd_many: job %d null pointer", i);
        const int P = kg_cdiv((long)a->N * a->T * a->V, BN_CHUNK);
        if (m) { m->beg[i] = (int)wg; m->P[i] = P; m->cbeg[i] = cb; m->wbeg[i] = wsf; m->job[i] = *a; }
        wg += (long)a->C * P;
        wsf += (long)a->C * P * 2;
        cb += a->C;
    }
    KG_REQUIRE(!m || wg < (1L << 31), "kg_bn_bwd_many: grid too large");
    if (m) { m->beg[njobs] = (int)wg; m->njobs = njobs; }
    *ws_floats = wsf;
    *ncounters = cb;
    return 0;
}

extern "C" int64_t kg_bn_bwd_many_workspace_bytes(const KgBnArgs* jobs, int32_t njobs) {
    int64_t wsf = 0;
    int nc = 0;
    if (bn_bwd_many_layout(jobs, njobs, nullptr, &wsf, &nc)) return -1;
    return wsf * (int64_t)sizeof(float);
}

extern "C" int kg_bn_bwd_many(const KgBnArgs* jobs, int32_t njobs, float* ws, int64_t ws_bytes, int32_t* counters,
                              int32_t counters_len, void* stream) {
    BnBwdMany m;
    int64_t wsf = 0;
    int nc = 0;
    if (int rc = bn_bwd_many_layout(jobs, njobs, &m, &wsf, &nc)) return rc;
    KG_REQUIRE(ws != nullptr && ws_bytes >= wsf * (int64_t)sizeof(float), "kg_bn_bwd_many: workspace too small");
    KG_REQUIRE(counters != nullptr && counters_len >= nc, "kg_bn_bwd_many: %d zeroed counters needed", nc);
    m.ws = ws;
    m.counters = counters;
    hipLaunchKernelGGL(kg_bn_bwd_many_kernel, dim3(m.beg[njobs]), dim3(NT), 0, (hipStream_t)stream, m);
    return kg_launch_status("kg_bn_bwd_many");
}

extern "C" int kg_act_bwd(const KgEltArgs* a, void* stream) {
    if (int rc = validate_elt(a, "kg_act_bwd")) return rc;
    KG_REQUIRE(a->r != nullptr, "kg_act_bwd: null ref");
    dim3 grid(kg_cdiv((long)a->N * a->T * a->V, NT), a->C);
    hipLaunchKernelGGL(kg_act_bwd_kernel, grid, dim3(NT), 0, (hipStream_t)stream, *a);
    return kg_launch_status("kg_act_bwd");
}

extern "C" int kg_affine_act(const KgEltArgs* a, void* stream) {
    if (int rc = validate_elt(a, "kg_affine_act")) return rc;
    KG_REQUIRE(a->groups <= 1 || (a->N % a->groups == 0 && a->coef_gs >= a->C), "kg_affine_act: groups=%d N=%d coef_gs=%ld",
               a->groups, a->N, (long)a->coef_gs);
    dim3 grid(kg_cdiv((long)a->N * a->T * a->V, NT), a->C);
    hipLaunchKernelGGL(kg_affine_act_kernel, grid, dim3(NT), 0, (hipStream_t)stream, *a);
    return kg_launch_status("kg_affine_act");
}

namespace {

__global__ __launch_bounds__(NT) void kg_gp_norm_kernel(const KgGpArgs a) {
    __shared__ float red[NT / 64];
    const int n = blockIdx.x;
    const int L = a.T * a.V;
    const long total = (long)a.C * L;
    const float* base = a.g + (long)n * a.g_sN;
    float s = 0.f;
    constexpr int PER = 8;
    for (long e0 = threadIdx.x; e0 < total; e0 += (long)NT * PER) {
        float v[PER];
#pragma unroll
        for (int u = 0; u < PER; ++u) {
            const long e = e0 + (long)u * NT;
            const bool ok = e < total;
            const int c = ok ? (int)(e / L) : 0, r = ok ? (int)(e - (long)c * L) : 0;
            const float x = base[(long)c * a.g_sC + r];
            v[u] = ok ? x : 0.f;
        }
#pragma unroll
        for (int u = 0; u < PER; ++u) s = fmaf(v[u], v[u], s);
    }
    s = wave_sum(s);
    if ((threadIdx.x & 63) == 0) red[threadIdx.x >> 6] = s;
    __syncthreads();
    if (threadIdx.x == 0) {
        float t = 0.f;
        for (int i = 0; i < NT / 64; ++i) t += red[i];
        a.nrm[n] = sqrtf(t);
    }
}

__global__ __launch_bounds__(NT) void kg_gp_mean_kernel(const KgGpArgs a) {
    __shared__ float red[NT / 64];
    float s = 0.f;
    for (int n = threadIdx.x; n < a.N; n += NT) {
        const float d = a.nrm[n] - 1.f;
        s = fmaf(d, d, s);
    }
    s = wave_sum(s);
    if ((threadIdx.x & 63) == 0) red[threadIdx.x >> 6] = s;
    __syncthreads();
    if (threadIdx.x == 0) {
        float t = 0.f;
        for (int i = 0; i < NT / 64; ++i) t += red[i];
        a.gp[0] = t / (float)a.N;
    }
}

__global__ __launch_bounds__(NT) void kg_gp_bwd_kernel(const KgGpArgs a) {
    const int L = a.T * a.V;
    const int n = blockIdx.z, c = blockIdx.y;
    const int r = blockIdx.x * NT + threadIdx.x;
    if (r >= L) return;
    const float nr = a.nrm[n];
    const float coef = nr > 0.f ? (2.f / (float)a.N) * (1.f - 1.f / nr) * a.gout[0] : 0.f;
    a.out[(long)n * a.o_sN + (long)c * a.o_sC + r] = coef * a.g[(long)n * a.g_sN + (long)c * a.g_sC + r];
}

int validate_gp(const KgGpArgs* a, const char* who) {
    KG_REQUIRE(a != nullptr, "%s: null args", who);
    KG_REQUIRE(a->N > 0 && a->C > 0 && a->T > 0 && a->V > 0 && a->N <= 65535 && a->C <= 65535, "%s: bad dims", who);
    KG_REQUIRE(a->g && a->nrm, "%s: null pointer", who);
    return 0;
}

}

extern "C" int kg_gp_fwd(const KgGpArgs* a, void* stream) {
    if (int rc = validate_gp(a, "kg_gp_fwd")) return rc;
    KG_REQUIRE(a->gp != nullptr, "kg_gp_fwd: null gp");
    hipLaunchKernelGGL(kg_gp_norm_kernel, dim3(a->N), dim3(NT), 0, (hipStream_t)stream, *a);
    if (int rc = kg_launch_status("kg_gp_fwd (norms)")) return rc;
    hipLaunchKernelGGL(kg_gp_mean_kernel, dim3(1), dim3(NT), 0, (hipStream_t)stream, *a);
    return kg_launch_status("kg_gp_fwd (mean)");
}

extern "C" int kg_gp_bwd(const KgGpArgs* a, void* stream) {
    if (int rc = validate_gp(a, "kg_gp_bwd")) return rc;
    KG_REQUIRE(a->gout && a->out, "kg_gp_bwd: null pointer");
    hipLaunchKernelGGL(kg_gp_bwd_kernel, dim3(kg_cdiv((long)a->T * a->V, NT), a->C, a->N), dim3(NT), 0, (hipStream_t)stream, *a);
    return kg_launch_status("kg_gp_bwd");
}

extern "C" int kg_adam_step(float* p, const float* g, float* m, float* v, int64_t n, float lr, float b1,
                            float b2, float eps, const int32_t* step, float grad_scale, void* stream) {
    KG_REQUIRE(p && g && m && v && step, "kg_adam_step: null pointer");
    KG_REQUIRE(n > 0, "kg_adam_step: n=%ld", (long)n);
    const bool vec = (((uintptr_t)p | (uintptr_t)g | (uintptr_t)m | (uintptr_t)v) & 15) == 0;
    if (vec)
        hipLaunchKernelGGL((kg_adam_kernel<true, false>), dim3(kg_cdiv(kg_cdiv(n, 4), NT)), dim3(NT), 0, (hipStream_t)stream, p,
                           const_cast<float*>(g), m, v, (long)n, lr, b1, b2, eps, step, grad_scale, 0);
    else
        hipLaunchKernelGGL((kg_adam_kernel<false, false>), dim3(kg_cdiv(n, NT)), dim3(NT), 0, (hipStream_t)stream, p,
                           const_cast<float*>(g), m, v, (long)n, lr, b1, b2, eps, step, grad_scale, 0);
    return kg_launch_status("kg_adam_step");
}

extern "C" int kg_adam_step_fused(float* p, float* g, float* m, float* v, int64_t n, float lr, float b1, float b2, float eps,
                                  const int32_t* step, float grad_scale, int32_t zero_grad, void* stream) {
    KG_REQUIRE(p && g && m && v && step, "kg_adam_step_fused: null pointer");
    KG_REQUIRE(n > 0, "kg_adam_step_fused: n=%ld", (long)n);
    const bool vec = (((uintptr_t)p | (uintptr_t)g | (uintptr_t)m | (uintptr_t)v) & 15) == 0;
    if (vec)
        hipLaunchKernelGGL((kg_adam_kernel<true, true>), dim3(kg_cdiv(kg_cdiv(n, 4), NT)), dim3(NT), 0, (hipStream_t)stream, p, g, m,
                           v, (long)n, lr, b1, b2, eps, step, grad_scale, (int)zero_grad);
    else
        hipLaunchKernelGGL((kg_adam_kernel<false, true>), dim3(kg_cdiv(n, NT)), dim3(NT), 0, (hipStream_t)stream, p, g, m, v,
                           (long)n, lr, b1, b2, eps, step, grad_scale, (int)zero_grad);
    return kg_launch_status("kg_adam_step_fused");
}

extern "C" int kg_adam_step_ema(float* p, float* g, float* m, float* v, float* e, int64_t n, float lr, float b1, float b2,
                                float eps, const int32_t* step, float grad_scale, int32_t zero_grad, float ema_decay,
                                float ema_warmup, void* stream) {
    KG_REQUIRE(p && g && m && v && e && step, "kg_adam_step_ema: null pointer");
    KG_REQUIRE(n > 0, "kg_adam_step_ema: n=%ld", (long)n);
    KG_REQUIRE(ema_decay >= 0.f && ema_decay < 1.f, "kg_adam_step_ema: ema_decay=%g (need 0 <= decay < 1)", (double)ema_decay);
    KG_REQUIRE(ema_warmup >= 0.f, "kg_adam_step_ema: ema_warmup=%g", (double)ema_warmup);
    const bool vec = (((uintptr_t)p | (uintptr_t)g | (uintptr_t)m | (uintptr_t)v | (uintptr_t)e) & 15) == 0;
    if (vec)
        hipLaunchKernelGGL((kg_adam_ema_kernel<true>), dim3(kg_cdiv(kg_cdiv(n, 4), NT)), dim3(NT), 0, (hipStream_t)stream, p, g, m,
                           v, e, (long)n, lr, b1, b2, eps, step, grad_scale, (int)zero_grad, ema_decay, ema_warmup);
    else
        hipLaunchKernelGGL((kg_adam_ema_kernel<false>), dim3(kg_cdiv(n, NT)), dim3(NT), 0, (hipStream_t)stream, p, g, m, v, e,
                           (long)n, lr, b1, b2, eps, step, grad_scale, (int)zero_grad, ema_decay, ema_warmup);
    return kg_launch_status("kg_adam_step_ema");
}


namespace {
constexpr int PEAK_WGS = 256 * 4;

__global__ __launch_bounds__(256) void kg_peak_mfma_kernel(float* sink, int iters) {
    kg_f32x16 acc[4];
#pragma unroll
    for (int i = 0; i < 4; ++i)
#pragma unroll
        for (int r = 0; r < 16; ++r) acc[i][r] = 0.f;
    float av[8], bv[8];
    unsigned st = 0x9e3779b9u * (threadIdx.x + 1u) + 0x85ebca6bu * (blockIdx.x + 1u);
    auto rnd = [&]() {
        float u = 0.f;
#pragma unroll
        for (int k = 0; k < 4; ++k) {
            st ^= st << 13; st ^= st >> 17; st ^= st << 5;
            u += (float)(st >> 8) * (1.f / 16777216.f);
        }
        return (u - 2.f) * 1.7320508f;
    };
#pragma unroll
    for (int i = 0; i < 8; ++i) { av[i] = rnd(); bv[i] = rnd() * 0.01f; }
    for (int it = 0; it < iters; ++it) {
#pragma unroll
// ... 33 lines not shown
```

### kinetic-gan_amd/disc_trunk.py

```python
from __future__ import annotations

import os

from typing import List, Optional

import torch
from torch.autograd import Function

from . import _native as nv
from . import ops
from ._native import ACT_LRELU, ACT_NONE, TAP_TIME, Group, WView

SLOPE = 0.2
D0_FUSED = os.environ.get("KG_D0_FUSED", "1") != "0"
_NV_LABEL_BIAS_FWD, _NV_AGGCONV = nv.label_bias_fwd, nv.aggconv


class BlockGeom:

    def __init__(self, blk, T, V, device, const_channels=0):
        p = blk._plan(T, V, device)
        self.res = blk.res_kind
        self.cin, self.cout, self.K = blk.in_channels, blk.out_channels, blk.gcn.kernel_size
        self.dw_s = blk.dw_s
# ... 44 lines not shown


class TrunkMeta:
    def __init__(self, geoms: List[BlockGeom], A_list=None, head: bool = False, label_bias: bool = False):
        self.geoms = geoms
        self.nb = len(geoms)
        self.head, self.lb = bool(head), bool(label_bias) and geoms[0].cc > 0
        self.poff = []
        off = 0
        for g in geoms:
            self.poff.append(off)
            off += g.nparam
        self.nparams = off
        self.any_single = any(g.single for g in geoms)
        self.ak_off, self.ak_shape, self.a_off = [], [], []
        if A_list is not None:
            dev = A_list[0].device
            a_parts, sel_parts = [], []
            aoff = koff = 0
            for g, A in zip(geoms, A_list):
                K, V, _ = A.shape
                idx = torch.arange(A.numel(), device=dev).view(K, V, V)
                if g.dw_s:
                    idx = idx[:, :, g.keep_l]
                sel_parts.append((idx + aoff).reshape(-1))
                a_parts.append(A.reshape(-1))
                self.a_off.append(aoff)
                self.ak_off.append(koff)
                self.ak_shape.append((K, V, g.W))
                aoff += A.numel()
                koff += K * V * g.W
            self.A_all = torch.cat(a_parts).contiguous()
            self.sel = torch.cat(sel_parts).contiguous()
            self.A_sel = self.A_all[self.sel].contiguous()
            self.ak_numel = koff

    def ak_views(self, ak_all):
        return [ak_all[o:o + s[0] * s[1] * s[2]].view(s) for o, s in zip(self.ak_off, self.ak_shape)]


def _pack(params):
    p0 = params[0]
    off = p0.storage_offset()
    ok = all(p.is_contiguous() and p.untyped_storage().data_ptr() == p0.untyped_storage().data_ptr() for p in params)
    if ok:
        for p in params:
            if p.storage_offset() != off:
                ok = False
                break
            off += p.numel()
    total = sum(p.numel() for p in params)
    if ok:
        return torch.as_strided(p0.detach(), (total,), (1,), p0.storage_offset())
    return torch.cat([p.detach().reshape(-1) for p in params])


class AdjacencyPack:

    def __init__(self, A_list):
        self.A_all = torch.cat([A.reshape(-1) for A in A_list]).contiguous()
        self.sel = None
        self.split = True
        self.ak_off, self.ak_shape = [], []
        off = 0
        for A in A_list:
            self.ak_off.append(off)
            self.ak_shape.append(tuple(A.shape))
            off += A.numel()

    def ak_views(self, ak_all):
        return [ak_all[o:o + s[0] * s[1] * s[2]].view(s) for o, s in zip(self.ak_off, self.ak_shape)]


class MaskedAdjacencyFn(Function):

    @staticmethod
    def forward(ctx, meta, *importances):
        imp_all = _pack(importances)
        ctx.meta = meta
        ctx.shapes = [tuple(p.shape) for p in importances]
        ctx.sinks = [ops._sink_of(p) for p in importances]
        ctx.split = bool(getattr(meta, "split", False))
        ak = nv.masked_adj_fwd(meta.A_all, imp_all, meta.sel)
        if ctx.split:
            ctx.set_materialize_grads(False)
            return tuple(meta.ak_views(ak))
        return ak

    @staticmethod
    @torch.autograd.function.once_differentiable
    def backward(ctx, *gs):
        meta = ctx.meta
        ops.flush_outer()
        if ctx.split:
            if all(g is None for g in gs):
                return (None,) * (1 + len(ctx.shapes))
            g = torch.cat([(g if g is not None else torch.zeros(s, device=meta.A_all.device)).reshape(-1)
                           for g, s in zip(gs, meta.ak_shape)])
        else:
            g = gs[0]
        if g is None:
            return (None,) * (1 + len(ctx.shapes))
        sinks = ctx.sinks
        if all(v is not None for v in sinks):
            adjacent = all(sinks[i + 1].data_ptr() == sinks[i].data_ptr() + 4 * sinks[i].numel() for i in range(len(sinks) - 1))
            if adjacent:
                flat = torch.as_strided(sinks[0], (meta.A_all.numel(),), (1,), sinks[0].storage_offset())
                nv.masked_adj_bwd(g, meta.A_all, meta.sel, flat, accumulate=True)
                return (None,) * (1 + len(ctx.shapes))
        dimp = torch.zeros_like(meta.A_all) if meta.sel is not None else torch.empty_like(meta.A_all)
        nv.masked_adj_bwd(g, meta.A_all, meta.sel, dimp, accumulate=False)
        outs, off = [], 0
        for shp in ctx.shapes:
            n = shp[0] * shp[1] * shp[2]
            outs.append(dimp[off:off + n].view(shp))
            off += n
        return (None,) + tuple(outs)


def _wg_view(geom: BlockGeom, wg: torch.Tensor) -> torch.Tensor:
    return wg.reshape(-1)[geom.cc:] if geom.cc else wg


def _sub(t: Optional[torch.Tensor], lo: int, hi: int):
    return None if t is None else t[lo:hi]



def _gcn(geom: BlockGeom, xa, wg, add=None, add_tstride=1):
    sp = geom.spec_g
    grp = Group(xa, _wg_view(geom, wg), sp.wv, sp.Cin, sp.taps, sp.tap_mode, 1, False, None)
    return nv.conv([grp], xa.shape[0], sp.M, sp.T_out, sp.V_out, add=add, add_tstride=add_tstride)


def _tail(geom: BlockGeom, z, x, wt, bt, wr, br, linear: bool, mask=None):
    st, sr = geom.spec_t, geom.spec_r
    groups = [Group(z, wt, st.wv, st.Cin, 3, TAP_TIME, st.t_stride, False, None)]
    add = None
    if geom.res == "conv":
        groups.append(Group(x, wr, sr.wv, sr.Cin, 1, TAP_TIME, sr.t_stride, False, sr.vmap))
    elif geom.res == "identity":
        add = x[:, :, :, geom.keep_l] if geom.dw_s else x
    return nv.conv(groups, z.shape[0], st.M, st.T_out, st.V_out,
                   bias0=None if linear else bt, bias1=None if (linear or geom.res != "conv") else br,
                   add=add, add_tstride=st.t_stride,
                   act=ACT_NONE if linear else ACT_LRELU, slope=SLOPE, mask=mask)


def _tcn_transposed_jobs(gm, wt, st):
    n = gm.shape[0]
    gz = nv.new_plane(n, st.Cin, st.T_in, st.V_in, gm.device)
    if not (st.t_stride == 2 and st.T_in % 2 == 0 and st.T_in >= 4 and wt.is_contiguous()):
        return [dict(groups=[Group(gm, wt, WView(st.wv.sT, st.wv.sI, st.wv.sO), st.M, 3, TAP_TIME, st.t_stride, True, None)],
                     N=n, M=st.Cin, T_out=st.T_in, V_out=st.V_in, out=gz)], gz
    flat = wt.reshape(-1)
    wv = WView(0, st.wv.sI, st.wv.sO)
    half = st.T_in // 2
    tap = [flat[d * st.wv.sT:] for d in range(3)]
    return [dict(groups=[Group(gm, tap[1], wv, st.M, 1)], N=n, M=st.Cin, T_out=half, V_out=st.V_in, out=gz, out_t0=0, out_tstride=2),
            dict(groups=[Group(gm, tap[2], wv, st.M, 1), Group(gm[:, :, 1:], tap[0], wv, st.M, 1)], N=n, M=st.Cin, T_out=half,
                 V_out=st.V_in, out=gz, out_t0=1, out_tstride=2)], gz


def _tcn_transposed(gm, wt, st):
    jobs, gz = _tcn_transposed_jobs(gm, wt, st)
    nv.conv_many(jobs)
    return gz


def _agg_gcn(g: BlockGeom, x, ak, wg, add, want_xa: bool):
    tstride = 0 if add is not None else 1
    if g.single:
        xa = nv.agg_expand(x, ak[:1], 1)
        sp = g.spec_g1
        return nv.conv([Group(xa, wg, sp.wv, sp.Cin, 1)], x.shape[0], sp.M, sp.T_out, sp.V_out, add=add, add_tstride=tstride), xa
    if g.fused_gcn(x.shape[0] * x.shape[2] * g.W) and not (want_xa and g.cout >= 256):
        sp = g.spec_g
        return nv.aggconv(x, ak, g.nbr, g.pcount, _wg_view(g, wg), WView(sp.wv.sT, sp.wv.sO, sp.wv.sI), sp.M,
                          add=add, add_tstride=tstride, want_xa=want_xa)
    xa = nv.agg_expand(x, ak, 1)
    return _gcn(g, xa, wg, add=add, add_tstride=tstride), xa


def _d0_fused_route(meta: TrunkMeta, x, labels, emb, want_xa: bool) -> bool:
    g = meta.geoms[0]
    if not (D0_FUSED and x.is_cuda and labels.is_cuda and nv.label_bias_fwd is _NV_LABEL_BIAS_FWD
            and nv.aggconv is _NV_AGGCONV):
        return False
    if g.single or (want_xa and g.cout >= 256) or not g.fused_gcn(x.shape[0] * x.shape[2] * g.W):
        return False
    return nv.aggconv_label_supported(g.K, g.cin - g.cc, g.cout, g.V, g.W, g.cc) and emb.shape[1] == g.cc


def fwd_pass(meta: TrunkMeta, x, zl, aks, params, want_xa: bool = True, lb0=None):
    tape = []
    for i, g in enumerate(meta.geoms):
        wg, wt, bt = params[meta.poff[i]:meta.poff[i] + 3]
        wr, br = (params[meta.poff[i] + 3], params[meta.poff[i] + 4]) if g.res == "conv" else (None, None)
        if i == 0 and lb0 is not None:
            sp = g.spec_g
            z, xa = nv.aggconv_label(x, aks[0], g.nbr, g.pcount, _wg_view(g, wg), WView(sp.wv.sT, sp.wv.sO, sp.wv.sI), sp.M,
                                     lb0[0], lb0[1], wg, g.cin, g.cc, want_xa=want_xa)
        else:
            z, xa = _agg_gcn(g, x, aks[i], wg, zl if g.cc else None, want_xa)
        out = _tail(g, z, x, wt, bt, wr, br, linear=False)
        tape.append((x, xa, z, out.detach()))
        x = out
    return x, tape


def _rows(t, r):
    return t if (r is None or t is None) else t[r[0]:r[1]]


def bwd_pass(meta: TrunkMeta, tape, g, aks, params, need_gx0: bool, want_params: bool, keep: bool,
             use_sink: bool = True, prow=None, krow=None, xrow=None, top_masked: bool = False, lb=None):
    nb = meta.nb
    dak = None
    if want_params:
        dak = (torch.zeros if meta.any_single else torch.empty)(meta.ak_numel, dtype=torch.float32, device=g.device)
    dviews = meta.ak_views(dak) if dak is not None else None
    pgr = [None] * meta.nparams if want_params else None
    tape2 = [None] * nb
    gzl = None
    outer_jobs = []
    masked = bool(top_masked)
    lb_job = None
    for i in range(nb - 1, -1, -1):
        geo = meta.geoms[i]
        x, xa, z, out = tape[i]
        wg, wt, bt = params[meta.poff[i]:meta.poff[i] + 3]
        wr = params[meta.poff[i] + 3] if geo.res == "conv" else None
        br = params[meta.poff[i] + 4] if geo.res == "conv" else None
        st, sr, sg = geo.spec_t, geo.spec_r, geo.spec_g
        gm = g if masked else nv.act_bwd(g, out, ACT_LRELU, SLOPE)
        masked = False
        need_gx = i > 0 or need_gx0
        jobs, gz = _tcn_transposed_jobs(gm, wt, st)
        sel = xrow if i == 0 else None
        gm_s = _rows(gm, sel)
        res_scatter = need_gx and geo.res == "conv" and (sr.t_stride > 1 or sr.inv_vmap is not None)
        if res_scatter:
            jobs.append(dict(groups=[Group(gm_s, wr, WView(0, sr.wv.sI, sr.wv.sO), sr.M, 1)], N=gm_s.shape[0], M=sr.Cin,
                             T_out=gm_s.shape[2], V_out=gm_s.shape[3]))
        outs = nv.conv_many(jobs)
        rs = outs[-1] if res_scatter else None
        gxa = None
        ak_i = aks[i][:1] if geo.single else aks[i]
        if need_gx or want_params:
            if geo.single:
                s1 = geo.spec_g1
                gxa = nv.conv([Group(gz, wg, WView(0, s1.wv.sI, s1.wv.sO), s1.M, 1)], gz.shape[0], s1.Cin, s1.T_in, s1.V_in)
            else:
                gxa = nv.conv([Group(gz, _wg_view(geo, wg), WView(0, sg.wv.sI, sg.wv.sO, sg.wv.sT, sg.Cin), sg.M, 1)],
                              gz.shape[0], sg.Cin * sg.taps, sg.T_in, sg.V_in)
        gx = None
        if need_gx:
            gxa_s, akT = _rows(gxa, sel), ak_i.transpose(1, 2)
            if geo.res == "conv":
                masked = i > 0
                mask_t = tape[i - 1][3] if masked else None
                if res_scatter:
                    gx = nv.agg_reduce(gxa_s, akT, 1, res=rs, res_tstride=sr.t_stride, res_inv=sr.inv_vmap, mask=mask_t, slope=SLOPE)
                else:
                    gx = nv.agg_reduce(gxa_s, akT, 1)
                    gx = nv.conv([Group(gm_s, wr, WView(0, sr.wv.sI, sr.wv.sO), sr.M, 1, TAP_TIME, sr.t_stride, True,
                                        sr.inv_vmap)], gm_s.shape[0], sr.Cin, sr.T_in, sr.V_in, add=gx,
                                 mask=mask_t, slope=SLOPE)
            elif geo.res == "identity":
                masked = i > 0
                gx = nv.agg_reduce(gxa_s, akT, 1, res=gm_s, res_tstride=geo.stride, res_inv=geo.inv_keep,
                                   mask=tape[i - 1][3] if masked else None, slope=SLOPE)
            else:
                gx = nv.agg_reduce(gxa_s, akT, 1)
        if want_params:
            po = meta.poff[i]
            xp, zp, gmp, gzp, gxap = _rows(x, prow), _rows(z, prow), _rows(gm, prow), _rows(gz, prow), _rows(gxa, prow)
            xap = nv.agg_expand(xp, ak_i, 1) if xa is None else _rows(xa, prow)
            sk = ops._sink_of if use_sink else (lambda t: None)
            pgr[po + 0] = _gcn_wgrad(geo, use_sink, xap, gzp, wg)
            pgr[po + 1] = _param_wgrad(sk(wt), zp, gmp, st, wt)
            if geo.res == "conv":
                pgr[po + 3] = _param_wgrad(sk(wr), xp, gmp, sr, wr)
            s_bt = sk(bt)
            s_br = sk(br) if br is not None else None
            if s_bt is not None and (br is None or s_br is not None):
                ops._rowsum_into([s_bt] + ([s_br] if s_br is not None else []), gmp)
            else:
                gb = nv.rowsum(gmp)[0]
                pgr[po + 2] = gb
                if br is not None:
                    pgr[po + 4] = gb
            nv.agg_outer(xp, gxap, 1 if geo.single else geo.K, 1, out=dviews[i][:1] if geo.single else dviews[i], defer=outer_jobs)
            if geo.cc and lb is not None:
                lb_job = (gzp, geo, wg, pgr, po)
            elif geo.cc:
                gzl = gzp.sum(2, keepdim=True)
        if keep:
            tape2[i] = (_rows(gm, krow), _rows(gz, krow), _rows(gxa, krow))
        g = gx
    if outer_jobs:
        nv.agg_outer_finish(outer_jobs)
    if lb_job is not None:
        gzp, geo, wg, pgr_, po = lb_job
        emb = lb["emb"]
        labels = lb["labels"] if prow is None else lb["labels"][prow[0]:prow[1]]
        s_emb = ops._sink_of(emb) if use_sink else None
        s_wg = ops._sink_of(wg) if use_sink else None
        demb = s_emb.view(emb.shape) if s_emb is not None else torch.zeros_like(emb)
        if s_wg is not None:
            dwg = s_wg
        else:
            dwg = pgr_[po + 0]
            if dwg is None:
                dwg = pgr_[po + 0] = torch.zeros_like(wg)
        nv.label_bias_bwd(gzp, labels, emb, wg, geo.K, geo.cout, geo.cin, geo.cc, aks[0].contiguous(),
                          demb=demb, dw=dwg.reshape(-1), dak=dviews[0], accumulate=True, dak_accumulate=True)
        gzl = None if s_emb is not None else demb
    return g, gzl, dak, pgr, (tape2 if keep else None)


def dbl_pass(meta: TrunkMeta, outs, tape2, h, aks, params, want_params: bool = True):
    dak = (torch.zeros if meta.any_single else torch.empty)(meta.ak_numel, dtype=torch.float32, device=h.device) if want_params else None
    dviews = meta.ak_views(dak) if dak is not None else None
    pgr = [None] * meta.nparams
    outer_jobs = []
    for i, geo in enumerate(meta.geoms):
        gm, gz, gxa = tape2[i]
        wg, wt, bt = params[meta.poff[i]:meta.poff[i] + 3]
        wr = params[meta.poff[i] + 3] if geo.res == "conv" else None
        st, sr, sg = geo.spec_t, geo.spec_r, geo.spec_g
        z, xa = _agg_gcn(geo, h, aks[i], wg, None, want_params)
        u = _tail(geo, z, h, wt, None, wr, None, linear=True, mask=outs[i])
        if want_params:
            po = meta.poff[i]
            pgr[po + 0] = _gcn_wgrad(geo, True, xa, gz, wg)
            pgr[po + 1] = _param_wgrad(ops._sink_of(wt), z, gm, st, wt)
            if geo.res == "conv":
                pgr[po + 3] = _param_wgrad(ops._sink_of(wr), h, gm, sr, wr)
            nv.agg_outer(h, gxa, 1 if geo.single else geo.K, 1, out=dviews[i][:1] if geo.single else dviews[i], defer=outer_jobs)
        h = u
    if outer_jobs:
        nv.agg_outer_finish(outer_jobs)
    return h, dak, pgr


def _gcn_wgrad(geo: BlockGeom, use_sink: bool, xa, gz, wg):
    if geo.single:
        n1 = geo.cout * geo.cin
        v = ops._sink_of(wg) if use_sink else None
        if v is not None:
            ops._wgrad_into(v[:n1], xa, gz, geo.spec_g1)
            return None
        full = torch.zeros(wg.numel(), dtype=wg.dtype, device=wg.device)
        s1 = geo.spec_g1
        nv.wgrad(gz, xa, s1.Cin, 1, s1.tap_mode, 1, None, n1, WView(s1.wv.sT, s1.wv.sO, s1.wv.sI), out=full[:n1])
        return full.view(wg.shape)
    return _param_wgrad(_sink_view(wg, geo.cc) if use_sink else None, xa, gz, geo.spec_g, wg, geo.cc)


def _sink_view(wg, cc):
    v = ops._sink_of(wg)
    if v is None or not cc:
        return v
    return v[cc:]


def _param_wgrad(view, x, g, spec, w, cc: int = 0):
    if view is not None:
        ops._wgrad_into(view, x, g, spec)
        return None
    wv = WView(spec.wv.sT, spec.wv.sO, spec.wv.sI)
    if not cc:
        flat = nv.wgrad(g, x, spec.Cin, spec.taps, spec.tap_mode, spec.t_stride, spec.vmap, w.numel(), wv)
        return flat.view(w.shape)
    full = torch.zeros(w.numel(), dtype=w.dtype, device=w.device)
    nv.wgrad(g, x, spec.Cin, spec.taps, spec.tap_mode, spec.t_stride, spec.vmap, w.numel() - cc, wv, out=full[cc:])
    return full.view(w.shape)



_CHECK_PROMISE = os.environ.get("KG_TRUNK_CHECK", "0") == "1"

def _join_parts(parts):
    if len(parts) == 1:
        return parts[0]
    a, b = parts
    if (a.is_contiguous() and b.is_contiguous() and a.untyped_storage().data_ptr() == b.untyped_storage().data_ptr()
            and b.storage_offset() == a.storage_offset() + a.numel() and a.shape[1:] == b.shape[1:]):
        return torch.as_strided(a, (a.shape[0] + b.shape[0],) + tuple(a.shape[1:]), a.stride(), a.storage_offset())
    return torch.cat((a, b), 0)


def _split_params(meta: TrunkMeta, params):
    n = meta.nparams
    blk, extra = list(params[:n]), list(params[n:])
    fw = fb = emb = None
    if meta.head:
        fw, fb = extra[0], extra[1]
        extra = extra[2:]
    if meta.lb:
        emb = extra[0]
    return blk, fw, fb, emb


def _n_extra(meta: TrunkMeta) -> int:
    return (2 if meta.head else 0) + (1 if meta.lb else 0)


def _extra_grads(meta: TrunkMeta, dfw=None, dfb=None, demb=None):
    out = []
    if meta.head:
        out += [dfw, dfb]
    if meta.lb:
        out += [demb]
    return out


def _head_param_grads(fw, fb, x, gv, use_sink: bool = True):
    sw = ops._sink_of(fw) if use_sink else None
    sb = ops._sink_of(fb) if (use_sink and fb is not None) else None
    dw = sw if sw is not None else torch.zeros(fw.numel(), dtype=torch.float32, device=fw.device)
    db = None
    if fb is not None:
        db = sb if sb is not None else torch.zeros(1, dtype=torch.float32, device=fw.device)
    nv.head_wgrad(x, gv, dw, db, accumulate=True)
    return (None if sw is not None else dw.view(fw.shape)), (None if (sb is not None or fb is None) else db.view(fb.shape))


class DiscTrunkFn(Function):

    @staticmethod
    def forward(ctx, meta: TrunkMeta, x_a, x_b, zl, ak_all, *params):
        ctx.set_materialize_grads(False)
        ctx.ga = None
        if isinstance(meta, tuple):
            meta, ctx.ga = meta
        ctx.merged = None
        params = list(params)
        blk, fw, fb, emb = _split_params(meta, params)
        aks = meta.ak_views(ak_all.detach())
        parts = [x_a] if x_b is None else [x_a, x_b]
        x = _join_parts([p.detach() for p in parts])
        want_xa = any(ctx.needs_input_grad[5:])
        with torch.no_grad():
            lb0 = None
            if meta.lb:
                g0 = meta.geoms[0]
                ctx.labels = zl
                if _d0_fused_route(meta, x, zl, emb, want_xa):
                    zl_v, lb0 = None, (zl, emb.detach())
                else:
                    zl_v = nv.label_bias_fwd(zl, emb.detach(), blk[0].detach(), g0.K, g0.cout, g0.cin, g0.cc, aks[0].contiguous())
            else:
                zl_v = None if zl is None else zl.detach()
            h, tape = fwd_pass(meta, x, zl_v, aks, [p.detach() for p in blk], want_xa, lb0=lb0)
            v = nv.head_fwd(h, fw.detach(), None if fb is None else fb.detach()).view(-1, 1) if meta.head else None
        ctx.meta = meta
        ctx.n_a = x_a.shape[0]
        ctx.n_b = 0 if x_b is None else x_b.shape[0]
        ctx.has_zl = zl is not None and not meta.lb
        ctx.tape = tape
        ctx.save_for_backward(ak_all, *params)
        res = v if meta.head else h
        if x_b is None:
            return (res,)
        return res[:ctx.n_a], res[ctx.n_a:]

    @staticmethod
    def backward(ctx, *gs):
        meta, n_a, n_b = ctx.meta, ctx.n_a, ctx.n_b
        saved = ctx.saved_tensors
        ak_all, params = saved[0], list(saved[1:])
        blk, fw, fb, emb = _split_params(meta, params)
        aks = meta.ak_views(ak_all.detach())
        nret = 5 + len(params)
        if all(g is None for g in gs):
            return (None,) * nret
        stash = None
        if ctx.merged is not None and gs[0] is not None and "result" in ctx.merged:
            if _CHECK_PROMISE and not (gs[0].is_cuda and torch.cuda.is_current_stream_capturing()):
                want = ctx.ga.view(-1, 1) if meta.head else ctx.ga.expand_as(gs[0])
                assert torch.allclose(gs[0], want, rtol=1e-6, atol=0), \
                    "DiscTrunkFn: the gradient of part a differs from the promised one"
            stash = ctx.merged.pop("result")
            gs = (None, gs[1] if len(gs) > 1 else None)
            if gs[1] is None:
                gzl_a, dak_a = stash
                gzl_full = None
                if gzl_a is not None and ctx.has_zl and ctx.needs_input_grad[3]:
                    gzl_full = gzl_a.new_zeros((n_a + n_b,) + tuple(gzl_a.shape[1:]))
                    gzl_full[:n_a] = gzl_a
                demb = gzl_a if meta.lb else None
                return (None, None, None, gzl_full, dak_a) + (None,) * meta.nparams + tuple(_extra_grads(meta, None, None, demb))
        if n_b == 0 or (gs[0] is not None and gs[1] is not None):
            lo, hi = 0, n_a + n_b
            g = gs[0] if n_b == 0 else torch.cat((gs[0], gs[1]), 0)
        elif gs[0] is not None:
            lo, hi, g = 0, n_a, gs[0]
        else:
            lo, hi, g = n_a, n_a + n_b, gs[1]
        need = ctx.needs_input_grad
        need_x = [need[1] and lo < n_a, n_b > 0 and need[2] and hi > n_a]
        need_gx0 = any(need_x)
        want_params = (not ops._SKIP_PARAM_GRADS) and any(need[3:])
        tape = [tuple(_sub(t, lo, hi) for t in b_) for b_ in ctx.tape]
        lb = dict(labels=ctx.labels[lo:hi], emb=emb.detach()) if meta.lb else None
        dfw = dfb = None
        if torch.is_grad_enabled():
            gx0 = gzl = dak = pgr = None
            merge = (ctx.ga is not None and ctx.merged is None and n_b > 0 and lo == n_a and need_gx0 and not need[1]
                     and any(need[3:]) and all(ops._sink_of(p) is not None for p in params))
            if need_gx0:
                outs = [b_[3] for b_ in tape]
                if merge:
                    ctx.merged = dict(ga=ctx.ga, tape=ctx.tape, n_a=n_a, n_b=n_b,
                                      labels=ctx.labels if meta.lb else None)
                    gx0 = DiscTrunkBwdFn.apply((meta, ctx.merged), g, ak_all, *params, *outs)
                else:
                    gx0 = DiscTrunkBwdFn.apply(meta, g, ak_all, *params, *outs)
            if want_params:
                with torch.no_grad():
                    gd = g.detach()
                    top = nv.head_bwd(gd, fw.detach(), tape[-1][3]) if meta.head else gd
                    _, gzl, dak, pgr, _ = bwd_pass(meta, tape, top, aks, [p.detach() for p in blk], False, True,
                                                   keep=False, use_sink=False, top_masked=meta.head, lb=lb)
                    if meta.head:
                        dfw, dfb = _head_param_grads(fw.detach(), fb, tape[-1][3], gd, use_sink=False)
        else:
            with torch.no_grad():
                top = nv.head_bwd(g, fw, tape[-1][3]) if meta.head else g
                gx0, gzl, dak, pgr, _ = bwd_pass(meta, tape, top, aks, blk, need_gx0, want_params, keep=False,
                                                 top_masked=meta.head, lb=lb)
                if meta.head and want_params:
                    dfw, dfb = _head_param_grads(fw, fb, tape[-1][3], g)
        gxa = gxb = None
        if gx0 is not None:
            if n_b == 0:
                gxa = gx0
            elif lo == 0 and hi == n_a + n_b:
                gxa, gxb = (gx0[:n_a] if need_x[0] else None), (gx0[n_a:] if need_x[1] else None)
            elif lo == 0:
                gxa = gx0
            else:
                gxb = gx0
        gzl_full = None
        demb = None
        if meta.lb:
            demb = gzl
        elif gzl is not None and ctx.has_zl and need[3]:
            if lo == 0 and hi == n_a + n_b:
                gzl_full = gzl
            else:
                gzl_full = gzl.new_zeros((n_a + n_b,) + tuple(gzl.shape[1:]))
                gzl_full[lo:hi] = gzl
        if stash is not None:
            gzl_a, dak_a = stash
            dak = dak_a if dak is None else dak + dak_a
            if meta.lb:
                if gzl_a is not None:
                    demb = gzl_a if demb is None else demb + gzl_a
            elif gzl_a is not None and ctx.has_zl and need[3]:
                if gzl_full is None:
                    gzl_full = gzl_a.new_zeros((n_a + n_b,) + tuple(gzl_a.shape[1:]))
                gzl_full[:n_a] += gzl_a
        out = [None, gxa, gxb, gzl_full, dak]
        out += (pgr if pgr is not None else [None] * meta.nparams)
        out += _extra_grads(meta, dfw, dfb, demb)
        return tuple(out)


class DiscTrunkBwdFn(Function):

    @staticmethod
    def forward(ctx, meta: TrunkMeta, g, ak_all, *rest):
        ctx.set_materialize_grads(False)
        merged = None
        if isinstance(meta, tuple):
            meta, merged = meta
        nb = meta.nb
        npar = meta.nparams + _n_extra(meta)
        params, outs = list(rest[:npar]), list(rest[npar:])
        blk, fw, fb, emb = _split_params(meta, params)
        with torch.no_grad():
            blk_d = [p.detach() for p in blk]
            aks = meta.ak_views(ak_all.detach())
            if merged is not None:
                n_a, n_b = merged["n_a"], merged["n_b"]
                top = merged["tape"][-1][3]
                if meta.head:
                    gv = torch.cat((merged["ga"].reshape(-1).to(g.dtype), g.detach().reshape(-1)))
                    g3 = nv.head_bwd(gv, fw.detach(), top)
                else:
                    g3 = nv.new_plane(*top.shape, top.device)
                    g3[:n_a].copy_(merged["ga"].expand(n_a, *top.shape[1:]))
                    g3[n_a:].copy_(g)
                lb = dict(labels=merged["labels"], emb=emb.detach()) if meta.lb else None
                gx0, gzl, dak, _, tape2 = bwd_pass(meta, merged["tape"], g3, aks, blk_d, need_gx0=True, want_params=True,
                                                   keep=True, prow=(0, n_a), krow=(n_a, n_a + n_b),
                                                   xrow=(n_a, n_a + n_b), top_masked=meta.head, lb=lb)
                if meta.head:
                    _head_param_grads(fw.detach(), fb, top[:n_a], gv[:n_a])
                merged["result"] = (gzl, dak)
            else:
                tape = [(None, None, None, o) for o in outs]
                top = nv.head_bwd(g.detach(), fw.detach(), outs[-1]) if meta.head else g
                gx0, _, _, _, tape2 = bwd_pass(meta, tape, top, aks, blk_d, need_gx0=True, want_params=False, keep=True,
                                               top_masked=meta.head)
        ctx.meta = meta
        ctx.tape2 = tape2
        ctx.gv = g.detach() if meta.head else None
        ctx.save_for_backward(ak_all, *params, *outs)
        return gx0

    @staticmethod
    @torch.autograd.function.once_differentiable
    def backward(ctx, h):
        meta = ctx.meta
        nb = meta.nb
        npar = meta.nparams + _n_extra(meta)
        nret = 3 + npar + nb
        if h is None:
            return (None,) * nret
        saved = ctx.saved_tensors
        ak_all, params, outs = saved[0], list(saved[1:1 + npar]), list(saved[1 + npar:])
        blk, fw, fb, emb = _split_params(meta, params)
        want = not ops._SKIP_PARAM_GRADS
        gg, dak, pgr = dbl_pass(meta, outs, ctx.tape2, h, meta.ak_views(ak_all.detach()), blk, want_params=want)
        if not meta.head:
            return (None, gg, dak) + tuple(pgr) + tuple(_extra_grads(meta)) + (None,) * nb
        dfw = None
        if want and ctx.needs_input_grad[3 + meta.nparams]:
            dfw, _ = _head_param_grads(fw, None, gg, ctx.gv)
        return (None, None, dak) + tuple(pgr) + tuple(_extra_grads(meta, dfw, None, None)) + (None,) * nb
```

### kinetic-gan_amd/generator.py

```python
from __future__ import annotations

import os

import numpy as np
import torch
import torch.nn as nn

from . import ops
from ._native import ACT_LRELU, ACT_TANH, TAP_TIME, WView
from .discriminator import _GraphModule, _adjacency_list
from .graph import build_graph
from .tgcn import ConvTemporalGraphical


def truncate_z(latent, mean_size, truncation, t=None):
    if t is None:
        t = torch.as_tensor(np.random.normal(0, 1, (mean_size, *latent.shape[1:])), dtype=latent.dtype,
                            device=latent.device)
    m = t.mean(0, keepdim=True)
    return m + truncation * (latent - m)


class NoiseInjection(nn.Module):
    def __init__(self, channel):
        super().__init__()
        self.weight = nn.Parameter(torch.zeros(1, channel, 1, 1))

    def forward(self, image, noise):
        return image + self.weight * noise


class Mapping_Net(nn.Module):
    def __init__(self, latent=1024, mlp=4):
        super().__init__()
        layers = []
        for _ in range(mlp):
            linear = nn.Linear(latent, latent)
            linear.weight.data.normal_()
            linear.bias.data.zero_()
            layers.append(linear)
            layers.append(nn.LeakyReLU(0.2))
        self.mlp = nn.Sequential(*layers)

    def forward(self, x):
        for layer in self.mlp:
            x = ops.SinkLinear.apply(x, layer.weight, layer.bias) if isinstance(layer, nn.Linear) else layer(x)
        return x


def _cat_batch(a, b):
    if a.is_contiguous() and b.is_contiguous() and a.shape == b.shape and a.dtype == b.dtype and a.device == b.device and \
            a.untyped_storage().data_ptr() == b.untyped_storage().data_ptr() and \
            b.storage_offset() == a.storage_offset() + a.numel():
        return a.as_strided((2 * a.shape[0],) + tuple(a.shape[1:]), a.stride())
    return torch.cat((a, b), 0)


class Generator(_GraphModule):
    def __init__(self, in_channels, out_channels, n_classes, t_size, mlp_dim=4,
                 edge_importance_weighting=True, dataset='ntu', **kwargs):
        super().__init__()
        self.graph = build_graph(dataset)
        self.A = _adjacency_list(self.graph)

        spatial_kernel_size = [A.size(0) for A in self.A]
        temporal_kernel_size = [3 for _ in self.A]
        kernel_size = (temporal_kernel_size, spatial_kernel_size)
        self.t_size = t_size
        g = self.graph
        self.mlp = Mapping_Net(in_channels + n_classes, mlp_dim)
        self.st_gcn_networks = nn.ModuleList((
            st_gcn(in_channels + n_classes, 512, kernel_size, 1, graph=g, lvl=3, bn=False, residual=False, up_s=False, up_t=1, **kwargs),
            st_gcn(512, 256, kernel_size, 1, graph=g, lvl=3, up_s=False, up_t=int(t_size / 16), **kwargs),
            st_gcn(256, 128, kernel_size, 1, graph=g, lvl=2, bn=False, up_s=True, up_t=int(t_size / 16), **kwargs),
            st_gcn(128, 64, kernel_size, 1, graph=g, lvl=2, up_s=False, up_t=int(t_size / 8), **kwargs),
            st_gcn(64, 32, kernel_size, 1, graph=g, lvl=1, bn=False, up_s=True, up_t=int(t_size / 4), **kwargs),
            st_gcn(32, out_channels, kernel_size, 1, graph=g, lvl=1, up_s=False, up_t=int(t_size / 2), **kwargs),
            st_gcn(out_channels, out_channels, kernel_size, 1, graph=g, lvl=0, bn=False, up_s=True, up_t=t_size, tan=True, **kwargs),
        ))
        if edge_importance_weighting:
            self.edge_importance = nn.ParameterList([
                nn.Parameter(torch.ones(self.A[i.lvl].size())) for i in self.st_gcn_networks])
        else:
            self.edge_importance = [1] * len(self.st_gcn_networks)
        self.label_emb = nn.Embedding(n_classes, n_classes)
        self._adj_pack = None
        self.use_trunk = os.environ.get("KG_GEN_TRUNK", "1") != "0"
        self.map_kernels = os.environ.get("KG_MAP_KERNELS", "1") != "0"
        self.exact_bn = os.environ.get("KG_EXACT_BN", "0") == "1"
        self.bn_group = None
        self._trunk = None

    def forward(self, x, labels, trunc=None, noise=None):
        return self.synthesis(self.mapping(x, labels, trunc), noise)

    def mapping(self, x, labels, trunc=None):
        layers = list(self.mlp.mlp)
        on_dev = (x.is_cuda and self.label_emb.weight.is_cuda) or ops.emulated()
        fused = self.map_kernels and on_dev and x.dim() == 2 and x.dtype == torch.float32 and labels.dtype == torch.int64 and \
            all(isinstance(m, nn.Linear if i % 2 == 0 else nn.LeakyReLU) for i, m in enumerate(layers)) and \
            len({m.negative_slope for m in layers[1::2]}) == 1
        if fused:
            wb = [p for m in layers[0::2] for p in (m.weight, m.bias)]
            w = ops.MappingFn.apply(x.contiguous(), labels.contiguous(), self.label_emb.weight, float(layers[1].negative_slope), *wb)
        else:
            c = self.label_emb(labels)
            x = torch.cat((c, x), -1)
            w = self.mlp(x)
        return self.truncate(w, 1000, trunc) if trunc is not None else w

    def synthesis_pair(self, w, noise_a=None, noise_b=None):
        n = w.shape[0]
        if (noise_a is None) != (noise_b is None):
            raise ValueError("synthesis_pair: give both noise lists or neither")
        noise = None if noise_a is None else [_cat_batch(a, b) for a, b in zip(noise_a, noise_b)]
        wd = w.detach()
        out, out_b = self.synthesis(torch.cat((wd, wd), 0), noise, w_b=w)
        return out[:n], out_b

    def synthesis(self, w, noise=None, w_b=None):
        trunk = self._trunk_state(w)
        x = w.view((*w.shape, 1, 1))
        x_b = w_b.view((*w_b.shape, 1, 1)) if w_b is not None else None
        if noise is None:
            n = x.shape[0]
            shapes = [(n, 1, gcn.up_t, self.graph.num_node[gcn.lvl]) for gcn in self.st_gcn_networks]
            sizes = [a * b * c * d for a, b, c, d in shapes]
            buf = torch.randn(sum(sizes), device=x.device, dtype=x.dtype)
            noise, off = [], 0
            for shp, sz in zip(shapes, sizes):
                noise.append(buf[off:off + sz].view(shp))
                off += sz
        if trunk is not None:
            from .gen_trunk import GenTrunkFn
            meta, params, bns = trunk
            cfg = (meta, bns, 2 if w_b is not None else 1)
            return GenTrunkFn.apply(cfg, w, w_b, *noise, *self.edge_importance, *params)
        if isinstance(self.edge_importance, nn.ParameterList) and x.is_cuda or getattr(self, "_pack_always", False):
            from .disc_trunk import AdjacencyPack, MaskedAdjacencyFn
            key = str(x.device)
            if self._adj_pack is None or self._adj_pack[0] != key:
                self._adj_pack = (key, AdjacencyPack([self.A[g.lvl] for g in self.st_gcn_networks]))
            pack = self._adj_pack[1]
            adjs = MaskedAdjacencyFn.apply(pack, *self.edge_importance)
            packed = True
        else:
            packed = False
            adjs = [self.A[gcn.lvl] * importance for gcn, importance in zip(self.st_gcn_networks, self.edge_importance)]
        sync = self.bn_group if self._exact_bn_active() else False
        for i, gcn in enumerate(self.st_gcn_networks):
            gcn.sync_bn = sync
            gcn.gcn.lazy_outer = packed
            if x_b is not None:
                (x, x_b), _ = gcn(x, adjs[i], noise[i], x_b)
            else:
                x, _ = gcn(x, adjs[i], noise[i])
        return x if w_b is None else (x, x_b)

    def _trunk_state(self, w):
        if not (self.use_trunk and self.training and isinstance(self.edge_importance, nn.ParameterList)):
            return None
        if self._exact_bn_active():
            return None
        if not (w.is_cuda or getattr(self, "_pack_always", False)):
            return None
        from . import gen_trunk as gt
        key = str(w.device)
        if self._trunk is None or self._trunk[0] != key:
            meta = gt.GenTrunkMeta(self, w.device)
            params, bns = gt.collect_params(self)
            self._trunk = (key, meta, params, bns, meta.ok and gt.trunk_supported(self, bns))
        _, meta, params, bns, ok = self._trunk
        if not ok:
            return None
        if torch.is_grad_enabled() and any(p.requires_grad for p in params) and not gt.all_sinks_registered(self):
            return None
        return meta, params, bns

    def _exact_bn_active(self) -> bool:
        if not (self.exact_bn and self.training):
            return False
        import torch.distributed as dist
        if not (dist.is_available() and dist.is_initialized()):
            if not getattr(self, "_exact_bn_warned", False):
                import warnings
                warnings.warn("Generator.exact_bn / KG_EXACT_BN=1 needs an initialised torch.distributed process group; "
                              "BatchNorm statistics stay per process")
                self._exact_bn_warned = True
            return False
        return dist.get_world_size(self.bn_group) > 1

    def truncate(self, w, mean, truncation, t=None):
        if t is None:
            t = torch.as_tensor(np.random.normal(0, 1, (mean, *w.shape[1:])), dtype=w.dtype, device=w.device)
        m = self.mlp(t).mean(0, keepdim=True)
        return m + truncation * (w - m)


class st_gcn(nn.Module):
    def __init__(self, in_channels, out_channels, kernel_size, stride=1, graph=None, lvl=3, dropout=0,
# ... 133 lines not shown
```

### kinetic-gan_amd/ops.py

```python
from __future__ import annotations

import os
from dataclasses import dataclass
from typing import Optional, Tuple

import torch
from torch.autograd import Function
from torch.autograd.function import once_differentiable

from . import _native as nv
from ._native import ACT_LRELU, ACT_NONE, ACT_TANH, TAP_CHANBLOCK, TAP_TIME, Group, WView

_SKIP_PARAM_GRADS = False


class no_param_grads:
    def __enter__(self):
        global _SKIP_PARAM_GRADS
        self.prev = _SKIP_PARAM_GRADS
        _SKIP_PARAM_GRADS = True

    def __exit__(self, *exc):
        global _SKIP_PARAM_GRADS
        _SKIP_PARAM_GRADS = self.prev
# ... 298 lines not shown
class AggExpand(Function):

    @staticmethod
    def forward(ctx, x, A, rep: int, pre=None):
        ctx.set_materialize_grads(False)
        ctx.rep = rep
        ctx.save_for_backward(x, A)
        return pre if pre is not None else nv.agg_expand(x, A, rep)

    @staticmethod
    def backward(ctx, g):
        if g is None:
            return (None, None, None, None)
        x, A = ctx.saved_tensors
        gx = AggReduce.apply(g, _t12(A), ctx.rep) if ctx.needs_input_grad[0] else None
        gA = None
        if ctx.needs_input_grad[1] and not _SKIP_PARAM_GRADS:
            gA = AggOuter.apply(x, g, A.shape[0], ctx.rep)
        return gx, gA, None, None


class AggReduce(Function):

    @staticmethod
    def forward(ctx, y, A, fold: int, pre=None, lazy_outer: bool = False):
        ctx.set_materialize_grads(False)
        ctx.fold = fold
        ctx.lazy_outer = lazy_outer
        ctx.save_for_backward(y, A)
        return pre if pre is not None else nv.agg_reduce(y, A, fold)

    @staticmethod
    def backward(ctx, g):
        if g is None:
            return (None, None, None, None)
        y, A = ctx.saved_tensors
        gy = AggExpand.apply(g, _t12(A), ctx.fold) if ctx.needs_input_grad[0] else None
        gA = None
        if ctx.needs_input_grad[1] and not _SKIP_PARAM_GRADS:
            if ctx.lazy_outer and not torch.is_grad_enabled():
                gA = nv.agg_outer(g, y, A.shape[0], ctx.fold, defer=_OUTER_PENDING).transpose(1, 2)
            else:
                gA = AggOuter.apply(g, y, A.shape[0], ctx.fold).transpose(1, 2)
        return gy, gA, None, None, None


class SinkLinear(Function):

    @staticmethod
    def forward(ctx, x, w, b):
        ctx.set_materialize_grads(False)
        ctx.sinks = (_sink_of(w), _sink_of(b))
        ctx.save_for_backward(x, w)
        return torch.nn.functional.linear(x, w, b)

    @staticmethod
    def backward(ctx, g):
        if g is None:
            return None, None, None
        x, w = ctx.saved_tensors
        gx = g @ w if ctx.needs_input_grad[0] else None
        gw = gb = None
        if not _SKIP_PARAM_GRADS:
            direct = _direct_param_grads()
            sw, sb = ctx.sinks
            g2, x2 = g.reshape(-1, g.shape[-1]), x.reshape(-1, x.shape[-1])
            if ctx.needs_input_grad[1]:
                if direct and sw is not None:
                    sw.view(w.shape).addmm_(g2.t(), x2)
                else:
                    gw = g2.t() @ x2
            if ctx.needs_input_grad[2]:
                if direct and sb is not None:
                    sb.add_(g2.sum(0))
                else:
                    gb = g2.sum(0)
        return gx, gw, gb


def emulated() -> bool:
    return getattr(nv.linear_fwd, "__module__", nv.__name__) != nv.__name__


class SyncBatchNorm2dFn(Function):

    @staticmethod
    def forward(ctx, x, gamma, beta, running_mean, running_var, nbt, momentum, eps, group):
        import torch.distributed as dist
        C = x.shape[1]
        xs = x.detach()
        cnt = torch.full((1,), float(x.numel() // C), dtype=xs.dtype, device=xs.device)
        packed = torch.cat((xs.sum((0, 2, 3)), (xs * xs).sum((0, 2, 3)), cnt))
        dist.all_reduce(packed, group=group)
        n = float(packed[2 * C].item())
        mean = packed[:C] / n
        var = (packed[C:2 * C] / n - mean * mean).clamp_min_(0.0)
        rstd = torch.rsqrt(var + eps)
        if running_mean is not None:
            with torch.no_grad():
                nbt += 1
                f = momentum if momentum is not None else 1.0 / float(nbt)
                running_mean.mul_(1 - f).add_(mean, alpha=f)
                running_var.mul_(1 - f).add_(var * (n / max(n - 1.0, 1.0)), alpha=f)
        xhat = (xs - mean.view(1, C, 1, 1)) * rstd.view(1, C, 1, 1)
        ctx.save_for_backward(xhat, rstd, gamma)
        ctx.n, ctx.group = n, group
        y = xhat
        if gamma is not None:
            y = y * gamma.view(1, C, 1, 1)
        if beta is not None:
            y = y + beta.view(1, C, 1, 1)
        return y

    @staticmethod
    @torch.autograd.function.once_differentiable
    def backward(ctx, g):
        import torch.distributed as dist
        xhat, rstd, gamma = ctx.saved_tensors
        C = xhat.shape[1]
        sg, sgx = g.sum((0, 2, 3)), (g * xhat).sum((0, 2, 3))
        dgamma = sgx.clone() if gamma is not None and ctx.needs_input_grad[1] else None
        dbeta = sg.clone() if ctx.needs_input_grad[2] else None
        gx = None
        if ctx.needs_input_grad[0]:
            packed = torch.cat((sg, sgx)) if gamma is None else torch.cat((sg * gamma, sgx * gamma))
            dist.all_reduce(packed, group=ctx.group)
            gs = g if gamma is None else g * gamma.view(1, C, 1, 1)
            gx = (gs - (packed[:C] / ctx.n).view(1, C, 1, 1) - xhat * (packed[C:2 * C] / ctx.n).view(1, C, 1, 1)) * rstd.view(1, C, 1, 1)
        return gx, dgamma, dbeta, None, None, None, None, None, None


class MappingFn(Function):

    @staticmethod
    def forward(ctx, z, labels, emb, slope, *wb):
        ctx.set_materialize_grads(False)
        ws, bs = wb[0::2], wb[1::2]
        ys = []
        y = nv.linear_fwd(z, ws[0], bs[0], nv.ACT_LRELU, slope, emb=emb, labels=labels)
        ys.append(y)
        for w, b in zip(ws[1:], bs[1:]):
            y = nv.linear_fwd(y, w, b, nv.ACT_LRELU, slope)
            ys.append(y)
        ctx.slope, ctx.nl = slope, len(ws)
        ctx.sinks = [(_sink_of(w), _sink_of(b)) for w, b in zip(ws, bs)] + [(_sink_of(emb), None)]
        ctx.save_for_backward(z, labels, emb, *ws, *ys)
        return y

    @staticmethod
    @torch.autograd.function.once_differentiable
    def backward(ctx, g):
        nl = ctx.nl
        if g is None:
            return (None,) * (4 + 2 * nl)
        z, labels, emb = ctx.saved_tensors[:3]
        ws = ctx.saved_tensors[3:3 + nl]
        ys = ctx.saved_tensors[3 + nl:]
        want_params = not _SKIP_PARAM_GRADS
        direct = want_params and _direct_param_grads()
        J = emb.shape[1]
        need_z = ctx.needs_input_grad[0]
        need_e = want_params and ctx.needs_input_grad[2]
        grads = [None] * (2 * nl)
        gz = gemb = None
        g = g.contiguous()
        for l in range(nl - 1, -1, -1):
            w, first = ws[l], l == 0
            x = z if first else ys[l - 1]
            sw, sb = ctx.sinks[l]
            need_w = want_params and ctx.needs_input_grad[4 + 2 * l]
            need_b = want_params and ctx.needs_input_grad[5 + 2 * l]
            dw = db = None
            acc = False
            if direct and (not need_w or sw is not None) and (not need_b or sb is not None):
                dw, db, acc = (sw if need_w else None), (sb if need_b else None), True
            else:
                dw = torch.empty_like(w) if need_w else None
                db = torch.empty(w.shape[0], dtype=w.dtype, device=w.device) if need_b else None
                grads[2 * l], grads[2 * l + 1] = dw, db
            cols = None if not first else (w.shape[1] if need_z else (J if need_e else 0))
            if first and cols == 0 and dw is None and db is None:
                break
            gx = nv.linear_bwd(g, ys[l], x, w, nv.ACT_LRELU, ctx.slope, emb=emb if first else None,
                               labels=labels if first else None, gx_cols=cols, dw=dw, db=db, accumulate=acc)
            if not first:
                g = gx
                continue
            if need_e:
                se = ctx.sinks[nl][0]
                if direct and se is not None:
                    nv.embed_bwd(gx, labels, se.view(emb.shape), accumulate=True)
                else:
                    gemb = torch.empty_like(emb)
                    nv.embed_bwd(gx, labels, gemb, accumulate=False)
            if need_z:
                gz = gx[:, J:]
        return (gz, None, gemb, None) + tuple(grads)


_OUTER_PENDING: list = []


def flush_outer():
    if _OUTER_PENDING:
        nv.agg_outer_finish(_OUTER_PENDING)


def pair_apply(F, xf, xb, *rest):
    with torch.no_grad():
        of = F.apply(xf, *rest)
    ob = F.apply(xb, *rest, of[of.shape[0] - xb.shape[0]:])
    return of, ob


class AggOuter(Function):

    @staticmethod
    def forward(ctx, x, y, K: int, rep: int):
        ctx.set_materialize_grads(False)
        ctx.K, ctx.rep = K, rep
        ctx.save_for_backward(x, y)
        return nv.agg_outer(x, y, K, rep)

    @staticmethod
    def backward(ctx, gA):
        if gA is None:
            return (None, None, None, None)
        x, y = ctx.saved_tensors
        gx = AggReduce.apply(y, _t12(gA), ctx.rep) if ctx.needs_input_grad[0] else None
        gy = AggExpand.apply(x, gA, ctx.rep) if ctx.needs_input_grad[1] else None
        return gx, gy, None, None



class ActBwd(Function):

    @staticmethod
    def forward(ctx, g, ref, act: int):
        ctx.set_materialize_grads(False)
        ctx.act = act
        ctx.save_for_backward(ref)
        return nv.act_bwd(g, ref, act)

    @staticmethod
    def backward(ctx, gg):
        if gg is None:
            return (None, None, None)
        (ref,) = ctx.saved_tensors
        if ctx.act == ACT_TANH:
            raise NotImplementedError("second derivative through tanh is not on the hot path "
                                      "(the generator is only differentiated once)")
        return ActBwd.apply(gg, ref, ctx.act), None, None


class RowSum(Function):

    @staticmethod
    def forward(ctx, x):
        ctx.set_materialize_grads(False)
        ctx.shape = tuple(x.shape)
        return nv.rowsum(x)[0]

    @staticmethod
    def backward(ctx, g):
        if g is None:
            return (None,)
        return g.view(1, -1, 1, 1).expand(ctx.shape)


class GradPenalty(Function):

    @staticmethod
    def forward(ctx, g):
        nrm, gp = nv.gp_fwd(g)
        ctx.save_for_backward(g, nrm)
        return gp

    @staticmethod
    @once_differentiable
    def backward(ctx, gout):
        g, nrm = ctx.saved_tensors
        return nv.gp_bwd(g, nrm, gout)


class CriticLoss(Function):

    @staticmethod
    def forward(ctx, both, gp, wvec, lam: float):
        ctx.lam = lam
        ctx.save_for_backward(wvec)
        ctx.shape = both.shape
        return torch.add(torch.dot(both.reshape(-1), wvec), gp, alpha=lam)

    @staticmethod
    @once_differentiable
    def backward(ctx, gout):
        (wvec,) = ctx.saved_tensors
        if getattr(gout, "_kg_unit_seed", False):
            key = (float(ctx.lam), str(gout.device), gout.dtype)
            lam = _LAM_CONSTS.get(key)
            if lam is None and not (gout.is_cuda and torch.cuda.is_current_stream_capturing()):
                lam = _LAM_CONSTS[key] = torch.full((), float(ctx.lam), dtype=gout.dtype, device=gout.device)
            if lam is not None:
                return wvec.view(ctx.shape), lam, None, None
        return (wvec * gout).view(ctx.shape), gout * ctx.lam, None, None


_LAM_CONSTS: dict = {}


def time_scatter(g, stride: int, T_in: int):
    if stride == 1:
        return g
    n, c, t, v = g.shape
    out = nv.new_plane(n, c, T_in, v, g.device, zero=True)
    out[:, :, 0:t * stride:stride] = g
    return out



class DiscTail(Function):

    @staticmethod
    def forward(ctx, z, x, wt, bt, wr, br, spec_t: ConvSpec, spec_r: Optional[ConvSpec], res: str):
        ctx.set_materialize_grads(False)
        ctx.spec_t, ctx.spec_r, ctx.res = spec_t, spec_r, res
        ctx.sinks = (_sink_of(wt), _sink_of(bt), _sink_of(wr) if res == "conv" else None,
                     _sink_of(br) if res == "conv" else None)
        groups = [Group(z, wt, spec_t.wv, spec_t.Cin, spec_t.taps, TAP_TIME, spec_t.t_stride, False, None)]
        add = None
        if res == "conv":
            groups.append(Group(x, wr, spec_r.wv, spec_r.Cin, 1, TAP_TIME, spec_r.t_stride, False, spec_r.vmap))
        elif res == "identity":
            add = x
        out = nv.conv(groups, z.shape[0], spec_t.M, spec_t.T_out, spec_t.V_out,
                      bias0=bt, bias1=br if res == "conv" else None,
                      add=add, add_tstride=spec_t.t_stride, act=ACT_LRELU, slope=0.2)
        ctx.save_for_backward(z, x, wt, wr, out)
        return out

    @staticmethod
    def backward(ctx, g):
        if g is None:
            return (None, None, None, None, None, None, None, None, None)
        z, x, wt, wr, out = ctx.saved_tensors
        st, sr, res = ctx.spec_t, ctx.spec_r, ctx.res
        need = ctx.needs_input_grad
        gm = ActBwd.apply(g, out, ACT_LRELU)
        gz = ConvT.apply(gm, wt, st) if need[0] else None
        gx = gwt = gbt = gwr = gbr = None
        params = not _SKIP_PARAM_GRADS
        direct = _direct_param_grads()
        s_wt, s_bt, s_wr, s_br = ctx.sinks
        if params and need[2]:
            if direct and s_wt is not None:
                _wgrad_into(s_wt, z, gm, st)
            else:
                gwt = WGrad.apply(z, gm, st)
        want_bt, want_br = need[3], res == "conv" and need[5]
        if params and (want_bt or want_br):
            sunk = [v for v, want in ((s_bt, want_bt), (s_br, want_br)) if want and direct and v is not None]
            if sunk:
                _rowsum_into(sunk, gm)
            if (want_bt and not (direct and s_bt is not None)) or (want_br and not (direct and s_br is not None)):
                gb = RowSum.apply(gm)
                gbt = gb if want_bt and not (direct and s_bt is not None) else None
                gbr = gb if want_br and not (direct and s_br is not None) else None
        if res == "conv":
            if need[1]:
                gx = ConvT.apply(gm, wr, sr)
            if params and need[4]:
                if direct and s_wr is not None:
                    _wgrad_into(s_wr, x, gm, sr)
                else:
                    gwr = WGrad.apply(x, gm, sr)
        elif res == "identity" and need[1]:
            gx = time_scatter(gm, st.t_stride, x.shape[2])
        return gz, gx, gwt, gbt, gwr, gbr, None, None, None



def _bn_coeffs(u, gamma, beta, rm, rv, nbt, training, momentum, eps):
    cma = training and rm is not None and momentum is None
    coef = nv.bn_fwd(u, gamma, beta, rm, rv, nbt, training, -1.0 if cma else (0.0 if momentum is None else momentum), eps)
    return coef[0], coef[1], coef[2], coef[3]


class GenTail(Function):

    @staticmethod
    def forward(ctx, u, r, noise, nw, gt, bt_, gr, br_, bn_t, bn_r, act: int, groups: int = 1, u_b=None, r_b=None):
# ... 108 lines not shown
```

### kinetic-gan_amd/wgan_gp.py

```python
from __future__ import annotations

from typing import List, Optional

import contextlib
import os
import weakref

import torch
import torch.distributed as dist

from . import _native as nv
from . import ops


def rebuild_generator(G):
    from .graph import Graph_h36m
    n_classes = G.label_emb.num_embeddings
    weighted = isinstance(G.edge_importance, torch.nn.ParameterList)
    with torch.random.fork_rng(devices=[]):
        E = type(G)(G.mlp.mlp[0].in_features - n_classes, G.st_gcn_networks[-1].out_channels, n_classes, G.t_size,
                    sum(isinstance(m, torch.nn.Linear) for m in G.mlp.mlp), edge_importance_weighting=weighted,
                    dataset="h36m" if isinstance(G.graph, Graph_h36m) else "ntu")
    E.to(next(G.parameters()).device)
    live, mine = list(G.named_parameters()), list(E.named_parameters())
# ... 36 lines not shown
        self._clean = False
        self.ema = None
        self.ema_decay = self.ema_warmup = None
        self.views = []
        keys = []
        for p, off in zip(self.params, self.offsets):
            n = p.numel()
            self.flat[off:off + n].copy_(p.data.reshape(-1))
            p.data = self.flat[off:off + n].view(p.shape)
            self.views.append(self.grad[off:off + n])
            p.grad = None
            keys.append(ops.register_param_sink(p, self.views[-1]))
        weakref.finalize(self, ops.unregister_param_sinks, keys)

    def zero_grad(self):
        ops.reset_param_sink(self.grad)
        if not self._clean:
            self.grad.zero_()
        self._clean = False
        for p in self.params:
            p.grad = None

    def gather_grads(self):
        ops.join_param_sink()
        dst, src = [], []
        for p, v in zip(self.params, self.views):
            g = p.grad
            if g is not None and g.data_ptr() != v.data_ptr():
                dst.append(v)
                src.append(g.reshape(-1))
        if dst:
            torch._foreach_add_(dst, src)
        for p, v in zip(self.params, self.views):
            p.grad = v.view(p.shape)

    def set_requires_grad(self, flag: bool):
        for p in self.params:
            p.requires_grad_(flag)

    def broadcast(self, src: int = 0):
        dist.broadcast(self.flat, src)

    def enable_ema(self, decay: float, warmup: float = 10.0):
        decay, warmup = float(decay), float(warmup)
        if not 0.0 < decay < 1.0:
            raise ValueError("FlatParams.enable_ema: decay must lie in (0, 1), got %r" % decay)
        if warmup < 0.0:
            raise ValueError("FlatParams.enable_ema: warmup must be >= 0, got %r" % warmup)
        self.ema = self.flat.detach().clone()
        self.ema_decay, self.ema_warmup = decay, warmup

    def allreduce_and_step(self, lr, b1, b2, eps=1e-8, world: int = 1, gather: bool = True, comm=None):
        if gather:
            self.gather_grads()
        if comm is not None:
            if comm.world > 1 or comm.force:
                comm.allreduce_(self.grad)
        elif world > 1:
            dist.all_reduce(self.grad, op=dist.ReduceOp.SUM)
        self.step += 1
        if self.ema is None:
            nv.adam_step(self.flat, self.grad, self.exp_avg, self.exp_avg_sq, lr, b1, b2, eps, self.step,
                         1.0 / world, zero_grad=self.fused_step)
        else:
            nv.adam_step_ema(self.flat, self.grad, self.exp_avg, self.exp_avg_sq, self.ema, lr, b1, b2, eps, self.step,
                             1.0 / world, self.fused_step, self.ema_decay, self.ema_warmup)
        self._clean = self.fused_step

    def state_dict(self) -> dict:
        return {"flat": self.flat.cpu(), "exp_avg": self.exp_avg.cpu(), "exp_avg_sq": self.exp_avg_sq.cpu(),
                "adam_step": self.step.cpu()}

    def load_state_dict(self, sd: dict) -> None:
        if sd["flat"].numel() != self.flat.numel():
            raise ValueError("FlatParams.load_state_dict: the state holds %d parameters, this module %d" % (
                sd["flat"].numel(), self.flat.numel()))
        self.flat.copy_(sd["flat"])
        self.exp_avg.copy_(sd["exp_avg"])
        self.exp_avg_sq.copy_(sd["exp_avg_sq"])
        self.step.copy_(sd["adam_step"])
        self.grad.zero_()


def penalty_of(d_inter, inter, keep: Optional[dict] = None):
    ones = _const_like(d_inter, 1.0)
    with ops.no_param_grads():
        (grads,) = torch.autograd.grad(outputs=d_inter, inputs=inter, grad_outputs=ones,
                                       create_graph=True, retain_graph=True, only_inputs=True)
    if keep is not None:
        keep["gp_grads"] = grads.detach()
    return ops.GradPenalty.apply(grads)


_CONSTS: dict = {}


def _const_like(t: torch.Tensor, value: float) -> torch.Tensor:
    key = (tuple(t.shape), t.dtype, str(t.device), float(value))
    c = _CONSTS.get(key)
    if c is None:
        if t.is_cuda and torch.cuda.is_current_stream_capturing():
            return torch.full(tuple(t.shape), float(value), dtype=t.dtype, device=t.device)
        if len(_CONSTS) > 64:
            _CONSTS.clear()
        c = _CONSTS[key] = torch.full(tuple(t.shape), float(value), dtype=t.dtype, device=t.device)
        if float(value) == 1.0:
            c._kg_unit_seed = True
    return c


def gradient_penalty(D, real, fake, labels, alpha, keep: Optional[dict] = None):
    inter = (alpha * real + (1 - alpha) * fake).requires_grad_(True)
    d_inter = D(inter, labels)
    ones = torch.ones_like(d_inter)
    with ops.no_param_grads():
        (grads,) = torch.autograd.grad(outputs=d_inter, inputs=inter, grad_outputs=ones,
                                       create_graph=True, retain_graph=True, only_inputs=True)
    if keep is not None:
        keep["gp_grads"] = grads.detach()
    grads = grads.reshape(grads.size(0), -1)
    return ((grads.norm(2, dim=1) - 1) ** 2).mean()


class Trainer:
    def __init__(self, G, D, lr=2e-4, b1=0.5, b2=0.999, lambda_gp=10.0, n_critic=5,
                 world_size: int = 1, flatten: bool = True, overlap: Optional[bool] = None, comm=None,
                 fused_step: bool = True, ema_decay: Optional[float] = None, ema_warmup: float = 10.0):
        self.G, self.D = G, D
        if ema_decay and not flatten:
            raise ValueError("Trainer: ema_decay needs the flat parameter buffers (flatten=True)")
        self.comm = comm
        if comm is not None and comm.world != world_size:
            raise ValueError("Trainer: comm.world=%d but world_size=%d" % (comm.world, world_size))
        self.lr, self.b1, self.b2 = lr, b1, b2
        self.lambda_gp, self.n_critic = lambda_gp, n_critic
        self.world = world_size
        self.fG = FlatParams(G) if flatten else None
        self.fD = FlatParams(D) if flatten else None
        for f in (self.fG, self.fD):
            if f is not None:
                f.fused_step = bool(fused_step)
        dev = next(D.parameters()).device
        self.overlap = bool(overlap) and dev.type == "cuda" and flatten
        self._side = None
        self._wvec = None
        self._promise = bool(flatten) and os.environ.get("KG_TRUNK_MERGE", "1") != "0"
        self._share_mapping = False
        self._w = None
        self._fake_g = None
        self._noise_g = None
        if self.world > 1:
            self.fG.broadcast(0)
            self.fD.broadcast(0)
            self.broadcast_buffers()
        self._ema_G = None
        if ema_decay:
            self.fG.enable_ema(ema_decay, ema_warmup)

    def ema_generator(self):
        if self.fG is None or self.fG.ema is None:
            raise RuntimeError("Trainer.ema_generator: the average is off (pass ema_decay)")
        if self._ema_G is not None:
            return self._ema_G
        G, f = self.G, self.fG
        E = rebuild_generator(G)
        live, mine = list(G.named_parameters()), list(E.named_parameters())
        if len(live) != len(f.offsets):
            raise RuntimeError("Trainer.ema_generator: could not rebuild the generator's structure")
        for (_, p), off in zip(mine, f.offsets):
            p.data = f.ema[off:off + p.numel()].view(p.shape)
            p.requires_grad_(False)
        for me, lm in zip(E.modules(), G.modules()):
            for k, b in lm._buffers.items():
                me._buffers[k] = b
        self._ema_G = E
        return E

    def broadcast_buffers(self, src: int = 0):
        for m in (self.G, self.D):
            for b in m.buffers():
                dist.broadcast(b, src)

    def d_losses(self, real, labels, z, alpha, noise: Optional[List[torch.Tensor]] = None, fake=None,
                 promise: bool = False):
        n = real.shape[0]
        if fake is None:
            exact_bn = getattr(self.G, "_exact_bn_active", None) is not None and self.G._exact_bn_active()
            if self._share_mapping and hasattr(self.G, "synthesis_pair") and self.G.training and not exact_bn and \
                    ((noise is None) == (self._noise_g is None)):
                w = self.G.mapping(z, labels)
                fake, self._fake_g = self.G.synthesis_pair(w, noise, self._noise_g)
            elif self._share_mapping and hasattr(self.G, "synthesis"):
                self._w = self.G.mapping(z, labels)
                with torch.no_grad():
                    fake = self.G.synthesis(self._w.detach(), noise)
            else:
                with torch.no_grad():
                    fake = self.G(z, labels, noise=noise)
        if getattr(self.D, "use_trunk", False):
            labels3 = torch.cat((labels, labels, labels), 0)
            buf = nv.mix3(real, fake, alpha)
            inter = buf[2 * n:].requires_grad_(True)
            key = (n, str(buf.device))
            if self._wvec is None or self._wvec[0] != key:
                w = torch.cat((torch.full((n,), -1.0 / n), torch.full((n,), 1.0 / n))).to(buf.device)
                self._wvec = (key, w)
            both, d_inter = self.D.forward_parts([(buf[:2 * n], labels3[:2 * n]), (inter, labels3[2 * n:])],
                                                 promised_grad=self._wvec[1] if promise else None)
            real_v, fake_v = both[:n], both[n:]
            out = {"fake": fake, "real_validity": real_v, "fake_validity": fake_v}
            gp = penalty_of(d_inter, inter, out)
            out["gradient_penalty"] = gp
            out["d_loss"] = ops.CriticLoss.apply(both, gp, self._wvec[1], float(self.lambda_gp))
            return out
        share = getattr(self.D, "shared_adjacency", None)
        with (share() if share is not None else contextlib.nullcontext()):
            both = self.D(torch.cat((real, fake), 0), torch.cat((labels, labels), 0))
            real_v, fake_v = both[:n], both[n:]
            out = {"fake": fake, "real_validity": real_v, "fake_validity": fake_v}
            gp = gradient_penalty(self.D, real, fake, labels, alpha, out)
        out["gradient_penalty"] = gp
        out["d_loss"] = -real_v.mean() + fake_v.mean() + self.lambda_gp * gp
        return out

    def g_losses(self, labels, z, noise: Optional[List[torch.Tensor]] = None):
        fake = self.G(z, labels, noise=noise)
        fake_v = self.D(fake, labels)
        return {"fake": fake, "fake_validity": fake_v, "g_loss": -fake_v.mean()}

    def d_compute(self, real, labels, z, alpha, noise=None, fake=None, keep: Optional[dict] = None):
        self.fD.zero_grad()
        r = self.d_losses(real, labels, z, alpha, noise, fake=fake, promise=self._promise)
        r["d_loss"].backward(_const_like(r["d_loss"], 1.0))
        self.fD.gather_grads()
        if keep is not None:
            keep.update({k: v.detach() for k, v in r.items()})
        return r["d_loss"].detach()

    def d_apply(self):
        self.fD.allreduce_and_step(self.lr, self.b1, self.b2, world=self.world, gather=False, comm=self.comm)

    def d_apply_async(self):
        if self._side is None:
            self._side = torch.cuda.Stream(device=self.fD.flat.device)
        cur = torch.cuda.current_stream(self.fD.flat.device)
        self._side.wait_stream(cur)
        with torch.cuda.stream(self._side):
            self.d_apply()

    def wait_d_apply(self):
        if self._side is not None:
            torch.cuda.current_stream(self.fD.flat.device).wait_stream(self._side)

    def g_forward(self, labels, z, noise=None):
        self.fG.zero_grad()
        fake, self._fake_g = self._fake_g, None
        if fake is not None:
            return fake
        w, self._w = self._w, None
        if w is not None:
            return self.G.synthesis(w, noise)
        return self.G(z, labels, noise=noise)

    def g_backward(self, fake, labels):
        self.fD.set_requires_grad(False)
        try:
            v = self.D(fake, labels)
            seed = _const_like(v, -1.0 / v.numel())
            g_loss = torch.dot(v.detach().reshape(-1), seed.reshape(-1))
            v.backward(seed)
        finally:
            self.fD.set_requires_grad(True)
        self.fG.gather_grads()
        return g_loss.detach()

    def g_compute(self, labels, z, noise=None):
        return self.g_backward(self.g_forward(labels, z, noise), labels)

    def g_apply(self):
        self.fG.allreduce_and_step(self.lr, self.b1, self.b2, world=self.world, gather=False, comm=self.comm)

    def d_step(self, real, labels, z, alpha, noise=None):
        loss = self.d_compute(real, labels, z, alpha, noise)
        self.d_apply()
        return loss

    def g_step(self, labels, z, noise=None):
        loss = self.g_compute(labels, z, noise)
        self.g_apply()
        return loss

    @contextlib.contextmanager
    def sharing_mapping(self, noise_g=None):
        prev, self._share_mapping = self._share_mapping, self.fG is not None
        self._noise_g = noise_g
        try:
            yield
        finally:
            self._share_mapping = prev
            self._noise_g = None

    def iteration(self, real, labels, z, alpha, noise_d=None, noise_g=None, with_g: bool = True):
        self._share_mapping = bool(with_g) and self.fG is not None and not self.overlap
        self._noise_g = noise_g if (with_g and not self.overlap) else None
        try:
            if not (self.overlap and with_g):
                d_loss = self.d_step(real, labels, z, alpha, noise_d)
                g_loss = self.g_step(labels, z, noise_g) if with_g else None
                return d_loss, g_loss
            d_loss = self.d_compute(real, labels, z, alpha, noise_d)
        finally:
            self._share_mapping = False
            self._noise_g = None
        self.d_apply_async()
        fake = self.g_forward(labels, z, noise_g)
        self.wait_d_apply()
        g_loss = self.g_backward(fake, labels)
        self.g_apply()
        return d_loss, g_loss
```

Measured before the change: 20730 samples/s.

## Fold step-end reductions and small glue ops into existing kernels

Several small launches at the ends of the G and D steps are folded into neighbouring kernels. The gradient-penalty kernel now also computes the critic loss via a last-block ticket. The head forward computes the generator loss, and the head backward fuses wgrad and zeroing. mix3 also builds the tripled label tensor, and the mapping network's last linear writes a duplicated output so synthesis_pair skips a concat. This cuts kernel count and launch overhead in a small-batch hipgraph workload, at the cost of more complex kernels using cross-block atomics/handoff counters and an N<=512 limit.

```diff
diff --git a/include/kgan_hip.h b/include/kgan_hip.h
--- a/include/kgan_hip.h
+++ b/include/kgan_hip.h
@@ -297,6 +297,9 @@
     float* gp;
     const float* gout;
     float* out;  int64_t o_sN, o_sC;
+    const float* vals;  const float* wvec;  int32_t nvals;  float lam;
+    float* d_loss;
+    int32_t* counter;
 } KgGpArgs;
 
 int kg_gp_fwd(const KgGpArgs* a, void* stream);
@@ -321,6 +324,11 @@
     float* g;  int64_t g_sN, g_sC;
     float slope;  int32_t masked;
     float* dw;  float* db;  int32_t accumulate;
+    const float* gv2;  int32_t n1;
+    int32_t wgrad_n;
+    float loss_scale;  float* loss;
+    int32_t* counter;
+    float* zero;  int32_t zero_n;
 } KgHeadArgs;
 int kg_head_fwd(const KgHeadArgs* a, void* stream);
 int kg_head_bwd(const KgHeadArgs* a, void* stream);
@@ -349,6 +357,7 @@
     const float* fake;  int64_t f_sN, f_sC;
     const float* alpha;
     float* out;  int64_t o_sN, o_sC;
+    const int64_t* labels;  int64_t* labels3;
 } KgMixArgs;
 int kg_mix3(const KgMixArgs* a, void* stream);
 
@@ -357,6 +366,7 @@
     const float* a;  const float* imp;  const int64_t* sel;
     float* ak;
     const float* g;  float* dimp;  int32_t accumulate;
+    const float* g2;
 } KgMaskedAdjArgs;
 int kg_masked_adj_fwd(const KgMaskedAdjArgs* a, void* stream);
 int kg_masked_adj_bwd(const KgMaskedAdjArgs* a, void* stream);
@@ -375,6 +385,7 @@
     float* dw;  float* db;
     float* demb;
     int32_t accumulate;
+    float* y2;
 } KgLinearArgs;
 int kg_linear_fwd(const KgLinearArgs* a, void* stream);
 int kg_linear_bwd(const KgLinearArgs* a, void* stream);
diff --git a/kinetic-gan_amd/_native.py b/kinetic-gan_amd/_native.py
--- a/kinetic-gan_amd/_native.py
+++ b/kinetic-gan_amd/_native.py
@@ -145,7 +145,9 @@
     _fields_ = [("N", C.c_int32), ("C", C.c_int32), ("T", C.c_int32), ("V", C.c_int32),
                 ("g", c_f32p), ("g_sN", C.c_int64), ("g_sC", C.c_int64),
                 ("nrm", c_f32p), ("gp", c_f32p), ("gout", c_f32p),
-                ("out", c_f32p), ("o_sN", C.c_int64), ("o_sC", C.c_int64)]
+                ("out", c_f32p), ("o_sN", C.c_int64), ("o_sC", C.c_int64),
+                ("vals", c_f32p), ("wvec", c_f32p), ("nvals", C.c_int32), ("lam", C.c_float),
+                ("d_loss", c_f32p), ("counter", C.c_void_p)]
 
 
 class _EltArgs(C.Structure):
@@ -182,7 +184,10 @@
                 ("w", c_f32p), ("b", c_f32p), ("v", c_f32p), ("gv", c_f32p),
                 ("g", c_f32p), ("g_sN", C.c_int64), ("g_sC", C.c_int64),
                 ("slope", C.c_float), ("masked", C.c_int32),
-                ("dw", c_f32p), ("db", c_f32p), ("accumulate", C.c_int32)]
+                ("dw", c_f32p), ("db", c_f32p), ("accumulate", C.c_int32),
+                ("gv2", c_f32p), ("n1", C.c_int32), ("wgrad_n", C.c_int32),
+                ("loss_scale", C.c_float), ("loss", c_f32p), ("counter", C.c_void_p),
+                ("zero", c_f32p), ("zero_n", C.c_int32)]
 
 
 class _LinearArgs(C.Structure):
@@ -192,7 +197,8 @@
                 ("act", C.c_int32), ("slope", C.c_float),
                 ("g", c_f32p), ("g_ld", C.c_int64),
                 ("gx", c_f32p), ("gx_ld", C.c_int64), ("gx_cols", C.c_int32),
-                ("dw", c_f32p), ("db", c_f32p), ("demb", c_f32p), ("accumulate", C.c_int32)]
+                ("dw", c_f32p), ("db", c_f32p), ("demb", c_f32p), ("accumulate", C.c_int32),
+                ("y2", c_f32p)]
 
 
 class _LabelBiasArgs(C.Structure):
@@ -212,12 +218,13 @@
                 ("real", c_f32p), ("r_sN", C.c_int64), ("r_sC", C.c_int64),
                 ("fake", c_f32p), ("f_sN", C.c_int64), ("f_sC", C.c_int64),
                 ("alpha", c_f32p),
-                ("out", c_f32p), ("o_sN", C.c_int64), ("o_sC", C.c_int64)]
+                ("out", c_f32p), ("o_sN", C.c_int64), ("o_sC", C.c_int64),
+                ("labels", C.c_void_p), ("labels3", C.c_void_p)]
 
 
 class _MaskedAdjArgs(C.Structure):
     _fields_ = [("n", C.c_int32), ("a", c_f32p), ("imp", c_f32p), ("sel", C.c_void_p), ("ak", c_f32p),
-                ("g", c_f32p), ("dimp", c_f32p), ("accumulate", C.c_int32)]
+                ("g", c_f32p), ("dimp", c_f32p), ("accumulate", C.c_int32), ("g2", c_f32p)]
 
 
 class _GenTailArgs(C.Structure):
@@ -1639,6 +1646,29 @@
     return nrm, gp
 
 
+GP_ONE_LAUNCH_MAX = 512
+
+
+def gp_fwd_loss(g: torch.Tensor, vals: Optional[torch.Tensor] = None, wvec: Optional[torch.Tensor] = None, lam: float = 0.0):
+    lib = load_library()
+    g = as_plane(g)
+    _need_cuda(g, vals, wvec)
+    a = _gp_args(g)
+    nrm = torch.empty(g.shape[0], dtype=torch.float32, device=g.device)
+    gp = torch.empty((), dtype=torch.float32, device=g.device)
+    a.nrm, a.gp = nrm.data_ptr(), gp.data_ptr()
+    d_loss = None
+    if vals is not None:
+        vals, wvec = vals.reshape(-1), wvec.reshape(-1)
+        assert vals.is_contiguous() and wvec.is_contiguous() and vals.numel() == wvec.numel()
+        assert vals.dtype == torch.float32 and wvec.dtype == torch.float32
+        d_loss = torch.empty((), dtype=torch.float32, device=g.device)
+        a.vals, a.wvec, a.nvals, a.lam, a.d_loss = vals.data_ptr(), wvec.data_ptr(), vals.numel(), float(lam), d_loss.data_ptr()
+    a.counter = _sync_buffer(g.device).data_ptr()
+    _check(lib.kg_gp_fwd(C.byref(a), _stream()), "kg_gp_fwd")
+    return nrm, gp, d_loss
+
+
 def gp_bwd(g: torch.Tensor, nrm: torch.Tensor, gout: torch.Tensor) -> torch.Tensor:
     lib = load_library()
     g = as_plane(g)
@@ -1763,7 +1793,7 @@
 
 
 
-def _head_args(h, w=None, gv=None):
+def _head_args(h, w=None, gv=None, gv2=None):
     a = _HeadArgs()
     h = _bind(a, "h", "h", h, True)
     a.N, a.C, a.T, a.V = h.shape
@@ -1772,28 +1802,46 @@
         assert w.is_contiguous() and w.numel() == h.shape[1]
         a.w = w.data_ptr()
     if gv is not None:
-        assert gv.numel() == h.shape[0]
+        assert gv.numel() + (0 if gv2 is None else gv2.numel()) == h.shape[0]
         a.gv = gv.data_ptr()
+        if gv2 is not None:
+            a.gv2, a.n1 = gv2.data_ptr(), gv.numel()
     return a, h
 
 
-def head_fwd(h: torch.Tensor, w: torch.Tensor, b: Optional[torch.Tensor]) -> torch.Tensor:
+def head_fwd(h: torch.Tensor, w: torch.Tensor, b: Optional[torch.Tensor], loss_scale: Optional[float] = None):
     lib = load_library()
     _need_cuda(h, w, b)
     a, h = _head_args(h, w)
     a.b = _ptr(b)
     v = torch.empty(h.shape[0], dtype=torch.float32, device=h.device)
     a.v = v.data_ptr()
+    loss = None
+    if loss_scale is not None:
+        loss = torch.empty((), dtype=torch.float32, device=h.device)
+        a.loss_scale, a.loss, a.counter = float(loss_scale), loss.data_ptr(), _sync_buffer(h.device).data_ptr()
     _check(lib.kg_head_fwd(C.byref(a), _stream()), "kg_head_fwd")
-    return v
-
-
-def head_bwd(gv: torch.Tensor, w: torch.Tensor, h: torch.Tensor, masked: bool = True, slope: float = 0.2) -> torch.Tensor:
+    return v if loss_scale is None else (v, loss)
+
+
+def head_bwd(gv: torch.Tensor, w: torch.Tensor, h: torch.Tensor, masked: bool = True, slope: float = 0.2,
+             gv2: Optional[torch.Tensor] = None, wgrad=None, zero: Optional[torch.Tensor] = None) -> torch.Tensor:
     lib = load_library()
     gv = gv.reshape(-1).contiguous()
-    _need_cuda(gv, w, h)
-    a, h = _head_args(h, w, gv)
+    if gv2 is not None:
+        gv2 = gv2.reshape(-1).contiguous()
+    _need_cuda(gv, w, h, gv2)
+    a, h = _head_args(h, w, gv, gv2)
     a.masked, a.slope = int(bool(masked)), slope
+    if wgrad is not None:
+        wn, dw, db, acc = wgrad
+        _need_cuda(dw, db)
+        assert dw.is_contiguous() and dw.numel() == h.shape[1] and (db is None or db.numel() == 1) and 0 < wn <= h.shape[0]
+        a.wgrad_n, a.dw, a.db, a.accumulate = int(wn), dw.data_ptr(), _ptr(db), int(bool(acc))
+    if zero is not None:
+        _need_cuda(zero)
+        assert zero.is_contiguous() and zero.dtype == torch.float32 and 0 < zero.numel() < (1 << 31)
+        a.zero, a.zero_n = zero.data_ptr(), zero.numel()
     g = _bind(a, "g", "g", new_plane(*h.shape, h.device))
     _check(lib.kg_head_bwd(C.byref(a), _stream()), "kg_head_bwd")
     return g
@@ -1976,7 +2024,7 @@
     _check(lib.kg_label_bias_bwd(C.byref(a), _stream()), "kg_label_bias_bwd")
 
 
-def mix3(real: torch.Tensor, fake: torch.Tensor, alpha: torch.Tensor) -> torch.Tensor:
+def mix3(real: torch.Tensor, fake: torch.Tensor, alpha: torch.Tensor, labels: Optional[torch.Tensor] = None):
     lib = load_library()
     real, fake = as_plane(real), as_plane(fake)
     alpha = alpha.reshape(-1).contiguous()
@@ -1990,8 +2038,14 @@
     _bind(a, "fake", "f", fake)
     a.alpha = alpha.data_ptr()
     a.out, a.o_sN, a.o_sC = out.data_ptr(), c * t * v, t * v
+    labels3 = None
+    if labels is not None:
+        _need_cuda(labels)
+        assert labels.dtype == torch.int64 and labels.is_contiguous() and labels.numel() == n
+        labels3 = torch.empty(3 * n, dtype=torch.int64, device=real.device)
+        a.labels, a.labels3 = labels.data_ptr(), labels3.data_ptr()
     _check(lib.kg_mix3(C.byref(a), _stream()), "kg_mix3")
-    return out
+    return out if labels is None else (out, labels3)
 
 
 def masked_adj_fwd(A_all: torch.Tensor, imp_all: Optional[torch.Tensor], sel: Optional[torch.Tensor]) -> torch.Tensor:
@@ -2007,14 +2061,19 @@
     return ak
 
 
-def masked_adj_bwd(g: torch.Tensor, A_all: torch.Tensor, sel: Optional[torch.Tensor], dimp: torch.Tensor, accumulate: bool):
+def masked_adj_bwd(g: torch.Tensor, A_all: torch.Tensor, sel: Optional[torch.Tensor], dimp: torch.Tensor, accumulate: bool,
+                   g2: Optional[torch.Tensor] = None):
     lib = load_library()
     g = g.reshape(-1).contiguous()
-    _need_cuda(g, A_all, sel, dimp)
+    _need_cuda(g, A_all, sel, dimp, g2)
     a = _MaskedAdjArgs()
     a.n = g.numel()
     assert dimp.is_contiguous() and dimp.numel() == A_all.numel() and (sel is None or sel.numel() == g.numel())
     a.a, a.sel, a.g, a.dimp, a.accumulate = A_all.data_ptr(), _ptr(sel), g.data_ptr(), dimp.data_ptr(), int(bool(accumulate))
+    if g2 is not None:
+        g2 = g2.reshape(-1).contiguous()
+        assert g2.numel() == g.numel() and g2.dtype == torch.float32
+        a.g2 = g2.data_ptr()
     _check(lib.kg_masked_adj_bwd(C.byref(a), _stream()), "kg_masked_adj_bwd")
 
 
@@ -2037,16 +2096,19 @@
 
 
 def linear_fwd(x: torch.Tensor, w: torch.Tensor, b: Optional[torch.Tensor], act: int = ACT_LRELU, slope: float = 0.2,
-               emb: Optional[torch.Tensor] = None, labels: Optional[torch.Tensor] = None) -> torch.Tensor:
+               emb: Optional[torch.Tensor] = None, labels: Optional[torch.Tensor] = None, twice: bool = False):
     lib = load_library()
     _need_cuda(x, w, b, emb, labels)
     a = _linear_args(x, w, emb, labels)
-    y = torch.empty(a.N, a.Dout, dtype=torch.float32, device=x.device)
+    yy = torch.empty((2 if twice else 1) * a.N, a.Dout, dtype=torch.float32, device=x.device)
+    y = yy[:a.N]
     a.bias = _ptr(b)
     a.y, a.y_ld = y.data_ptr(), a.Dout
+    if twice:
+        a.y2 = yy[a.N:].data_ptr()
     a.act, a.slope = act, slope
     _check(lib.kg_linear_fwd(C.byref(a), _stream()), "kg_linear_fwd")
-    return y
+    return (y, yy) if twice else y
 
 
 def linear_bwd(g: torch.Tensor, y: torch.Tensor, x: torch.Tensor, w: torch.Tensor, act: int = ACT_LRELU, slope: float = 0.2,
diff --git a/kinetic-gan_amd/csrc/kg_disc.hip b/kinetic-gan_amd/csrc/kg_disc.hip
--- a/kinetic-gan_amd/csrc/kg_disc.hip
+++ b/kinetic-gan_amd/csrc/kg_disc.hip
@@ -1,4 +1,5 @@
 #include "kg_common.h"
+#include "kg_handoff.h"
 
 namespace {
 
@@ -21,8 +22,11 @@
     return t;
 }
 
+__device__ __forceinline__ float head_gv(const KgHeadArgs& a, int n) { return (a.gv2 && n >= a.n1) ? a.gv2[n - a.n1] : a.gv[n]; }
+
 __global__ __launch_bounds__(NT) void kg_head_fwd_kernel(const KgHeadArgs a) {
     __shared__ float red[NT / 64];
+    __shared__ int last;
     const int n = blockIdx.x, L = a.T * a.V;
     const float* base = a.h + (long)n * a.h_sN;
     float s = 0.f;
@@ -31,39 +35,63 @@
         s = fmaf(a.w[c], base[(long)c * a.h_sC + r], s);
     }
     const float t = block_sum(s, red);
-    if (threadIdx.x == 0) a.v[n] = t / (float)L + (a.b ? a.b[0] : 0.f);
-}
-
-__global__ __launch_bounds__(NT) void kg_head_bwd_kernel(const KgHeadArgs a) {
+    if (a.loss == nullptr) {
+        if (threadIdx.x == 0) a.v[n] = t / (float)L + (a.b ? a.b[0] : 0.f);
+        return;
+    }
+    if (threadIdx.x == 0) {
+        kg_pub_store(a.v + n, t / (float)L + (a.b ? a.b[0] : 0.f));
+        last = kg_ticket_draw(a.counter, a.N);
+    }
+    __syncthreads();
+    if (!last) return;
+    float d = 0.f;
+    for (int i = threadIdx.x; i < a.N; i += NT) d += kg_pub_load(a.v + i) * a.loss_scale;
+    const float tot = block_sum(d, red);
+    if (threadIdx.x == 0) a.loss[0] = tot;
+}
+
+__device__ __forceinline__ void head_wgrad_body(const KgHeadArgs& a, const int c, const int N, float* red) {
+    const int L = a.T * a.V;
+    float s = 0.f;
+    if (c < a.C) {
+        for (int e = threadIdx.x; e < N * L; e += NT) {
+            const int n = e / L, r = e - n * L;
+            s = fmaf(head_gv(a, n), a.h[(long)n * a.h_sN + (long)c * a.h_sC + r], s);
+        }
+        const float t = block_sum(s, red);
+        if (threadIdx.x == 0) a.dw[c] = (a.accumulate ? a.dw[c] : 0.f) + t / (float)L;
+    } else {
+        for (int n = threadIdx.x; n < N; n += NT) s += head_gv(a, n);
+        const float t = block_sum(s, red);
+        if (threadIdx.x == 0 && a.db) a.db[0] = (a.accumulate ? a.db[0] : 0.f) + t;
+    }
+}
+
+__global__ __launch_bounds__(NT) void kg_head_bwd_kernel(const KgHeadArgs a, const int nbwd) {
+    __shared__ float red[NT / 64];
+    if ((int)blockIdx.x >= nbwd) {
+        head_wgrad_body(a, (int)blockIdx.x - nbwd, a.wgrad_n, red);
+        return;
+    }
     const int L = a.T * a.V;
     const long total = (long)a.N * a.C * L;
     const float inv = 1.f / (float)L;
-    for (long i = (long)blockIdx.x * NT + threadIdx.x; i < total; i += (long)gridDim.x * NT) {
+    for (long i = (long)blockIdx.x * NT + threadIdx.x; i < total; i += (long)nbwd * NT) {
         const int c = (int)(i / ((long)a.N * L));
         const long rem = i - (long)c * a.N * L;
         const int n = (int)(rem / L), r = (int)(rem - (long)n * L);
-        float v = a.gv[n] * a.w[c] * inv;
+        float v = head_gv(a, n) * a.w[c] * inv;
         if (a.masked) v *= a.h[(long)n * a.h_sN + (long)c * a.h_sC + r] > 0.f ? 1.f : a.slope;
         a.g[(long)n * a.g_sN + (long)c * a.g_sC + r] = v;
     }
+    if (a.zero)
+        for (long i = (long)blockIdx.x * NT + threadIdx.x; i < a.zero_n; i += (long)nbwd * NT) a.zero[i] = 0.f;
 }
 
 __global__ __launch_bounds__(NT) void kg_head_wgrad_kernel(const KgHeadArgs a) {
     __shared__ float red[NT / 64];
-    const int c = blockIdx.x, L = a.T * a.V;
-    float s = 0.f;
-    if (c < a.C) {
-        for (int e = threadIdx.x; e < a.N * L; e += NT) {
-            const int n = e / L, r = e - n * L;
-            s = fmaf(a.gv[n], a.h[(long)n * a.h_sN + (long)c * a.h_sC + r], s);
-        }
-        const float t = block_sum(s, red);
-        if (threadIdx.x == 0) a.dw[c] = (a.accumulate ? a.dw[c] : 0.f) + t / (float)L;
-    } else {
-        for (int n = threadIdx.x; n < a.N; n += NT) s += a.gv[n];
-        const float t = block_sum(s, red);
-        if (threadIdx.x == 0 && a.db) a.db[0] = (a.accumulate ? a.db[0] : 0.f) + t;
-    }
+    head_wgrad_body(a, blockIdx.x, a.N, red);
 }
 
 constexpr int LB_MAXKW = 3 * 32, LB_MAXKC = 3 * 64, LB_MAXCW = 64 * 32, LB_MAXW = 12288;
@@ -306,6 +334,13 @@
         o[(long)(n + a.N) * a.o_sN] = f;
         o[(long)(n + 2 * a.N) * a.o_sN] = al * x + (1.f - al) * f;
     }
+    if (a.labels3)
+        for (long n = (long)blockIdx.x * NT + threadIdx.x; n < a.N; n += (long)gridDim.x * NT) {
+            const int64_t l = a.labels[n];
+            a.labels3[n] = l;
+            a.labels3[n + a.N] = l;
+            a.labels3[n + 2 * (long)a.N] = l;
+        }
 }
 
 __global__ __launch_bounds__(NT) void kg_masked_adj_kernel(const KgMaskedAdjArgs a, const int backward) {
@@ -315,7 +350,8 @@
     if (!backward) {
         a.ak[i] = a.a[s] * (a.imp ? a.imp[s] : 1.f);
     } else {
-        const float v = a.g[i] * a.a[s];
+        const float gi = a.g2 ? a.g[i] + a.g2[i] : a.g[i];
+        const float v = gi * a.a[s];
         a.dimp[s] = (a.accumulate ? a.dimp[s] : 0.f) + v;
     }
 }
@@ -342,6 +378,7 @@
 extern "C" int kg_head_fwd(const KgHeadArgs* a, void* stream) {
     if (int rc = validate_head(a, "kg_head_fwd")) return rc;
     KG_REQUIRE(a->h && a->w && a->v, "kg_head_fwd: null pointer");
+    KG_REQUIRE(a->loss == nullptr || (a->counter != nullptr && a->N <= 512), "kg_head_fwd: loss needs a counter and N <= 512 (N=%d)", a->N);
     hipLaunchKernelGGL(kg_head_fwd_kernel, dim3(a->N), dim3(NT), 0, (hipStream_t)stream, *a);
     return kg_launch_status("kg_head_fwd");
 }
@@ -349,16 +386,22 @@
 extern "C" int kg_head_bwd(const KgHeadArgs* a, void* stream) {
     if (int rc = validate_head(a, "kg_head_bwd")) return rc;
     KG_REQUIRE(a->gv && a->w && a->g && (!a->masked || a->h), "kg_head_bwd: null pointer");
+    KG_REQUIRE(a->gv2 == nullptr || (a->n1 >= 0 && a->n1 <= a->N), "kg_head_bwd: n1=%d outside [0, N=%d]", a->n1, a->N);
+    KG_REQUIRE(a->wgrad_n >= 0 && a->wgrad_n <= a->N, "kg_head_bwd: wgrad_n=%d outside [0, N=%d]", a->wgrad_n, a->N);
+    KG_REQUIRE(a->wgrad_n == 0 || (a->h && a->dw), "kg_head_bwd: wgrad_n without h / dw");
+    KG_REQUIRE(a->zero == nullptr || a->zero_n > 0, "kg_head_bwd: zero_n=%d", a->zero_n);
     const long total = (long)a->N * a->C * a->T * a->V;
     long grid = (total + NT - 1) / NT;
     if (grid > 4096) grid = 4096;
-    hipLaunchKernelGGL(kg_head_bwd_kernel, dim3((int)grid), dim3(NT), 0, (hipStream_t)stream, *a);
+    const int extra = a->wgrad_n > 0 ? a->C + 1 : 0;
+    hipLaunchKernelGGL(kg_head_bwd_kernel, dim3((int)grid + extra), dim3(NT), 0, (hipStream_t)stream, *a, (int)grid);
     return kg_launch_status("kg_head_bwd");
 }
 
 extern "C" int kg_head_wgrad(const KgHeadArgs* a, void* stream) {
     if (int rc = validate_head(a, "kg_head_wgrad")) return rc;
     KG_REQUIRE(a->gv && a->h && a->dw, "kg_head_wgrad: null pointer");
+    KG_REQUIRE(a->gv2 == nullptr || (a->n1 >= 0 && a->n1 <= a->N), "kg_head_wgrad: n1=%d outside [0, N=%d]", a->n1, a->N);
     hipLaunchKernelGGL(kg_head_wgrad_kernel, dim3(a->C + 1), dim3(NT), 0, (hipStream_t)stream, *a);
     return kg_launch_status("kg_head_wgrad");
 }
@@ -404,6 +447,7 @@
 extern "C" int kg_mix3(const KgMixArgs* a, void* stream) {
     KG_REQUIRE(a != nullptr && a->N > 0 && a->C > 0 && a->T > 0 && a->V > 0, "kg_mix3: bad dims");
     KG_REQUIRE(a->real && a->fake && a->alpha && a->out, "kg_mix3: null pointer");
+    KG_REQUIRE((a->labels == nullptr) == (a->labels3 == nullptr), "kg_mix3: labels and labels3 go together");
     const long total = (long)a->N * a->C * a->T * a->V;
     long grid = (total + NT - 1) / NT;
     if (grid > 4096) grid = 4096;
diff --git a/kinetic-gan_amd/csrc/kg_map.hip b/kinetic-gan_amd/csrc/kg_map.hip
--- a/kinetic-gan_amd/csrc/kg_map.hip
+++ b/kinetic-gan_amd/csrc/kg_map.hip
@@ -102,7 +102,11 @@
     }
     const float v = reduce_rows(acc, red, wave, lane);
     const int nn = n0 + row_of_reg(wave, h);
-    if (o_ok && nn < a.N) a.y[(long)nn * a.y_ld + o] = kg_act(v + bias, a.act, a.slope);
+    if (o_ok && nn < a.N) {
+        const float yv = kg_act(v + bias, a.act, a.slope);
+        a.y[(long)nn * a.y_ld + o] = yv;
+        if (a.y2) a.y2[(long)nn * a.y_ld + o] = yv;
+    }
 }
 
 template <int VW>
diff --git a/kinetic-gan_amd/csrc/kg_misc.hip b/kinetic-gan_amd/csrc/kg_misc.hip
--- a/kinetic-gan_amd/csrc/kg_misc.hip
+++ b/kinetic-gan_amd/csrc/kg_misc.hip
@@ -724,8 +724,7 @@
 
 namespace {
 
-__global__ __launch_bounds__(NT) void kg_gp_norm_kernel(const KgGpArgs a) {
-    __shared__ float red[NT / 64];
+__device__ __forceinline__ float gp_sample_sumsq(const KgGpArgs& a, float* red) {
     const int n = blockIdx.x;
     const int L = a.T * a.V;
     const long total = (long)a.C * L;
@@ -748,27 +747,63 @@
     s = wave_sum(s);
     if ((threadIdx.x & 63) == 0) red[threadIdx.x >> 6] = s;
     __syncthreads();
-    if (threadIdx.x == 0) {
-        float t = 0.f;
+    float t = 0.f;
+    if (threadIdx.x == 0)
         for (int i = 0; i < NT / 64; ++i) t += red[i];
-        a.nrm[n] = sqrtf(t);
-    }
-}
-
-__global__ __launch_bounds__(NT) void kg_gp_mean_kernel(const KgGpArgs a) {
-    __shared__ float red[NT / 64];
+    return t;
+}
+
+template <bool PUB>
+__device__ __forceinline__ float gp_mean_of(const KgGpArgs& a, float* red) {
     float s = 0.f;
     for (int n = threadIdx.x; n < a.N; n += NT) {
-        const float d = a.nrm[n] - 1.f;
+        const float d = (PUB ? kg_pub_load(a.nrm + n) : a.nrm[n]) - 1.f;
         s = fmaf(d, d, s);
     }
     s = wave_sum(s);
     if ((threadIdx.x & 63) == 0) red[threadIdx.x >> 6] = s;
     __syncthreads();
+    float t = 0.f;
+    if (threadIdx.x == 0)
+        for (int i = 0; i < NT / 64; ++i) t += red[i];
+    return t / (float)a.N;
+}
+
+__global__ __launch_bounds__(NT) void kg_gp_norm_kernel(const KgGpArgs a) {
+    __shared__ float red[NT / 64];
+    const float t = gp_sample_sumsq(a, red);
+    if (threadIdx.x == 0) a.nrm[blockIdx.x] = sqrtf(t);
+}
+
+__global__ __launch_bounds__(NT) void kg_gp_mean_kernel(const KgGpArgs a) {
+    __shared__ float red[NT / 64];
+    const float gp = gp_mean_of<false>(a, red);
+    if (threadIdx.x == 0) a.gp[0] = gp;
+}
+
+__global__ __launch_bounds__(NT) void kg_gp_fused_kernel(const KgGpArgs a) {
+    __shared__ float red[NT / 64];
+    __shared__ int last;
+    const float t = gp_sample_sumsq(a, red);
     if (threadIdx.x == 0) {
-        float t = 0.f;
-        for (int i = 0; i < NT / 64; ++i) t += red[i];
-        a.gp[0] = t / (float)a.N;
+        kg_pub_store(a.nrm + blockIdx.x, sqrtf(t));
+        last = kg_ticket_draw(a.counter, a.N);
+    }
+    __syncthreads();
+    if (!last) return;
+    const float gp = gp_mean_of<true>(a, red);
+    if (threadIdx.x == 0) a.gp[0] = gp;
+    if (a.d_loss == nullptr) return;
+    float d = 0.f;
+    for (int i = threadIdx.x; i < a.nvals; i += NT) d = fmaf(a.vals[i], a.wvec[i], d);
+    d = wave_sum(d);
+    __syncthreads();
+    if ((threadIdx.x & 63) == 0) red[threadIdx.x >> 6] = d;
+    __syncthreads();
+    if (threadIdx.x == 0) {
+        float dot = 0.f;
+        for (int i = 0; i < NT / 64; ++i) dot += red[i];
+        a.d_loss[0] = dot + a.lam * gp;
     }
 }
 
@@ -794,6 +829,12 @@
 extern "C" int kg_gp_fwd(const KgGpArgs* a, void* stream) {
     if (int rc = validate_gp(a, "kg_gp_fwd")) return rc;
     KG_REQUIRE(a->gp != nullptr, "kg_gp_fwd: null gp");
+    KG_REQUIRE(a->d_loss == nullptr || (a->counter && a->vals && a->wvec && a->nvals > 0), "kg_gp_fwd: d_loss needs counter / vals / wvec");
+    if (a->counter != nullptr) {
+        KG_REQUIRE(a->N <= 512, "kg_gp_fwd: the one-launch form takes N <= 512 (N=%d)", a->N);
+        hipLaunchKernelGGL(kg_gp_fused_kernel, dim3(a->N), dim3(NT), 0, (hipStream_t)stream, *a);
+        return kg_launch_status("kg_gp_fwd (one launch)");
+    }
     hipLaunchKernelGGL(kg_gp_norm_kernel, dim3(a->N), dim3(NT), 0, (hipStream_t)stream, *a);
     if (int rc = kg_launch_status("kg_gp_fwd (norms)")) return rc;
     hipLaunchKernelGGL(kg_gp_mean_kernel, dim3(1), dim3(NT), 0, (hipStream_t)stream, *a);
diff --git a/kinetic-gan_amd/disc_trunk.py b/kinetic-gan_amd/disc_trunk.py
--- a/kinetic-gan_amd/disc_trunk.py
+++ b/kinetic-gan_amd/disc_trunk.py
@@ -150,6 +150,8 @@
         ctx.sinks = [ops._sink_of(p) for p in importances]
         ctx.split = bool(getattr(meta, "split", False))
         ak = nv.masked_adj_fwd(meta.A_all, imp_all, meta.sel)
+        ctx.kg_masked_adj = True
+        ctx.parked = None
         if ctx.split:
             ctx.set_materialize_grads(False)
             return tuple(meta.ak_views(ak))
@@ -167,6 +169,9 @@
                            for g, s in zip(gs, meta.ak_shape)])
         else:
             g = gs[0]
+        g2, ctx.parked = ctx.parked, None
+        if g2 is not None and g is None:
+            g, g2 = g2, None
         if g is None:
             return (None,) * (1 + len(ctx.shapes))
         sinks = ctx.sinks
@@ -174,8 +179,13 @@
             adjacent = all(sinks[i + 1].data_ptr() == sinks[i].data_ptr() + 4 * sinks[i].numel() for i in range(len(sinks) - 1))
             if adjacent:
                 flat = torch.as_strided(sinks[0], (meta.A_all.numel(),), (1,), sinks[0].storage_offset())
-                nv.masked_adj_bwd(g, meta.A_all, meta.sel, flat, accumulate=True)
+                if g2 is not None:
+                    nv.masked_adj_bwd(g, meta.A_all, meta.sel, flat, accumulate=True, g2=g2)
+                else:
+                    nv.masked_adj_bwd(g, meta.A_all, meta.sel, flat, accumulate=True)
                 return (None,) * (1 + len(ctx.shapes))
+        if g2 is not None:
+            g = g + g2
         dimp = torch.zeros_like(meta.A_all) if meta.sel is not None else torch.empty_like(meta.A_all)
         nv.masked_adj_bwd(g, meta.A_all, meta.sel, dimp, accumulate=False)
         outs, off = [], 0
@@ -282,10 +292,12 @@
 
 
 def bwd_pass(meta: TrunkMeta, tape, g, aks, params, need_gx0: bool, want_params: bool, keep: bool,
-             use_sink: bool = True, prow=None, krow=None, xrow=None, top_masked: bool = False, lb=None):
+             use_sink: bool = True, prow=None, krow=None, xrow=None, top_masked: bool = False, lb=None, dak_buf=None):
     nb = meta.nb
     dak = None
-    if want_params:
+    if want_params and dak_buf is not None:
+        dak = dak_buf
+    elif want_params:
         dak = (torch.zeros if meta.any_single else torch.empty)(meta.ak_numel, dtype=torch.float32, device=g.device)
     dviews = meta.ak_views(dak) if dak is not None else None
     pgr = [None] * meta.nparams if want_params else None
@@ -388,8 +400,11 @@
     return g, gzl, dak, pgr, (tape2 if keep else None)
 
 
-def dbl_pass(meta: TrunkMeta, outs, tape2, h, aks, params, want_params: bool = True):
-    dak = (torch.zeros if meta.any_single else torch.empty)(meta.ak_numel, dtype=torch.float32, device=h.device) if want_params else None
+def dbl_pass(meta: TrunkMeta, outs, tape2, h, aks, params, want_params: bool = True, dak_buf=None):
+    if want_params and dak_buf is not None:
+        dak = dak_buf
+    else:
+        dak = (torch.zeros if meta.any_single else torch.empty)(meta.ak_numel, dtype=torch.float32, device=h.device) if want_params else None
     dviews = meta.ak_views(dak) if dak is not None else None
     pgr = [None] * meta.nparams
     outer_jobs = []
@@ -523,7 +538,15 @@
             else:
                 zl_v = None if zl is None else zl.detach()
             h, tape = fwd_pass(meta, x, zl_v, aks, [p.detach() for p in blk], want_xa, lb0=lb0)
-            v = nv.head_fwd(h, fw.detach(), None if fb is None else fb.detach()).view(-1, 1) if meta.head else None
+            v = None
+            if meta.head:
+                want = ops._HEAD_LOSS
+                fbd = None if fb is None else fb.detach()
+                if want is not None and x_b is None and h.is_cuda and h.shape[0] <= nv.GP_ONE_LAUNCH_MAX and ops.step_ends():
+                    v, want["loss"] = nv.head_fwd(h, fw.detach(), fbd, loss_scale=want["scale"])
+                else:
+                    v = nv.head_fwd(h, fw.detach(), fbd)
+                v = v.view(-1, 1)
         ctx.meta = meta
         ctx.n_a = x_a.shape[0]
         ctx.n_b = 0 if x_b is None else x_b.shape[0]
@@ -555,6 +578,11 @@
             gs = (None, gs[1] if len(gs) > 1 else None)
             if gs[1] is None:
                 gzl_a, dak_a = stash
+                node = ak_all.grad_fn
+                if dak_a is not None and ak_all.is_cuda and ops.step_ends() and ctx.needs_input_grad[4] and \
+                        getattr(node, "kg_masked_adj", False) and not node.split and node.parked is None:
+                    node.parked = dak_a
+                    dak_a = None
                 gzl_full = None
                 if gzl_a is not None and ctx.has_zl and ctx.needs_input_grad[3]:
                     gzl_full = gzl_a.new_zeros((n_a + n_b,) + tuple(gzl_a.shape[1:]))
@@ -656,9 +684,21 @@
             if merged is not None:
                 n_a, n_b = merged["n_a"], merged["n_b"]
                 top = merged["tape"][-1][3]
+                head_done = False
+                zbuf = dak1 = dak2 = None
                 if meta.head:
-                    gv = torch.cat((merged["ga"].reshape(-1).to(g.dtype), g.detach().reshape(-1)))
-                    g3 = nv.head_bwd(gv, fw.detach(), top)
+                    ga, gb = merged["ga"].reshape(-1).to(g.dtype), g.detach().reshape(-1)
+                    sw, sb = ops._sink_of(fw), (None if fb is None else ops._sink_of(fb))
+                    if top.is_cuda and ops.step_ends() and sw is not None and (fb is None or sb is not None):
+                        if meta.any_single:
+                            half = (meta.ak_numel + 3) // 4 * 4
+                            zbuf = torch.empty(2 * half, dtype=torch.float32, device=top.device)
+                            dak1, dak2 = zbuf[:meta.ak_numel], zbuf[half:half + meta.ak_numel]
+                        g3 = nv.head_bwd(ga, fw.detach(), top, gv2=gb, wgrad=(n_a, sw, sb, True), zero=zbuf)
+                        head_done = True
+                    else:
+                        gv = torch.cat((ga, gb))
+                        g3 = nv.head_bwd(gv, fw.detach(), top)
                 else:
                     g3 = nv.new_plane(*top.shape, top.device)
                     g3[:n_a].copy_(merged["ga"].expand(n_a, *top.shape[1:]))
@@ -666,8 +706,9 @@
                 lb = dict(labels=merged["labels"], emb=emb.detach()) if meta.lb else None
                 gx0, gzl, dak, _, tape2 = bwd_pass(meta, merged["tape"], g3, aks, blk_d, need_gx0=True, want_params=True,
                                                    keep=True, prow=(0, n_a), krow=(n_a, n_a + n_b),
-                                                   xrow=(n_a, n_a + n_b), top_masked=meta.head, lb=lb)
-                if meta.head:
+                                                   xrow=(n_a, n_a + n_b), top_masked=meta.head, lb=lb, dak_buf=dak1)
+                ctx.dak2 = dak2
+                if meta.head and not head_done:
                     _head_param_grads(fw.detach(), fb, top[:n_a], gv[:n_a])
                 merged["result"] = (gzl, dak)
             else:
@@ -677,6 +718,8 @@
                                                top_masked=meta.head)
         ctx.meta = meta
         ctx.tape2 = tape2
+        if merged is None:
+            ctx.dak2 = None
         ctx.gv = g.detach() if meta.head else None
         ctx.save_for_backward(ak_all, *params, *outs)
         return gx0
@@ -694,7 +737,8 @@
         ak_all, params, outs = saved[0], list(saved[1:1 + npar]), list(saved[1 + npar:])
         blk, fw, fb, emb = _split_params(meta, params)
         want = not ops._SKIP_PARAM_GRADS
-        gg, dak, pgr = dbl_pass(meta, outs, ctx.tape2, h, meta.ak_views(ak_all.detach()), blk, want_params=want)
+        dak2, ctx.dak2 = ctx.dak2, None
+        gg, dak, pgr = dbl_pass(meta, outs, ctx.tape2, h, meta.ak_views(ak_all.detach()), blk, want_params=want, dak_buf=dak2)
         if not meta.head:
             return (None, gg, dak) + tuple(pgr) + tuple(_extra_grads(meta)) + (None,) * nb
         dfw = None
diff --git a/kinetic-gan_amd/generator.py b/kinetic-gan_amd/generator.py
--- a/kinetic-gan_amd/generator.py
+++ b/kinetic-gan_amd/generator.py
@@ -94,7 +94,7 @@
     def forward(self, x, labels, trunc=None, noise=None):
         return self.synthesis(self.mapping(x, labels, trunc), noise)
 
-    def mapping(self, x, labels, trunc=None):
+    def mapping(self, x, labels, trunc=None, pair=False):
         layers = list(self.mlp.mlp)
         on_dev = (x.is_cuda and self.label_emb.weight.is_cuda) or ops.emulated()
         fused = self.map_kernels and on_dev and x.dim() == 2 and x.dtype == torch.float32 and labels.dtype == torch.int64 and \
@@ -102,7 +102,14 @@
             len({m.negative_slope for m in layers[1::2]}) == 1
         if fused:
             wb = [p for m in layers[0::2] for p in (m.weight, m.bias)]
-            w = ops.MappingFn.apply(x.contiguous(), labels.contiguous(), self.label_emb.weight, float(layers[1].negative_slope), *wb)
+            box = [] if (pair and trunc is None and x.is_cuda and ops.step_ends()) else None
+            ops.MappingFn.pair_box = box
+            try:
+                w = ops.MappingFn.apply(x.contiguous(), labels.contiguous(), self.label_emb.weight, float(layers[1].negative_slope), *wb)
+            finally:
+                ops.MappingFn.pair_box = None
+            if box:
+                w._kg_pair = box[0]
         else:
             c = self.label_emb(labels)
             x = torch.cat((c, x), -1)
@@ -114,8 +121,11 @@
         if (noise_a is None) != (noise_b is None):
             raise ValueError("synthesis_pair: give both noise lists or neither")
         noise = None if noise_a is None else [_cat_batch(a, b) for a, b in zip(noise_a, noise_b)]
-        wd = w.detach()
-        out, out_b = self.synthesis(torch.cat((wd, wd), 0), noise, w_b=w)
+        ww = getattr(w, "_kg_pair", None)
+        if ww is None or tuple(ww.shape) != (2 * n,) + tuple(w.shape[1:]):
+            wd = w.detach()
+            ww = torch.cat((wd, wd), 0)
+        out, out_b = self.synthesis(ww, noise, w_b=w)
         return out[:n], out_b
 
     def synthesis(self, w, noise=None, w_b=None):
diff --git a/kinetic-gan_amd/ops.py b/kinetic-gan_amd/ops.py
--- a/kinetic-gan_amd/ops.py
+++ b/kinetic-gan_amd/ops.py
@@ -404,6 +404,29 @@
     return getattr(nv.linear_fwd, "__module__", nv.__name__) != nv.__name__
 
 
+def step_ends() -> bool:
+    return os.environ.get("KG_STEP_ENDS", "1") != "0" and not emulated()
+
+
+_HEAD_LOSS = None
+
+
+class head_loss:
+
+    def __init__(self, scale: float):
+        self.box = dict(scale=float(scale))
+
+    def __enter__(self):
+        global _HEAD_LOSS
+        self.prev, _HEAD_LOSS = _HEAD_LOSS, self.box
+        return self.box
+
+    def __exit__(self, *exc):
+        global _HEAD_LOSS
+        _HEAD_LOSS = self.prev
+        return False
+
+
 class SyncBatchNorm2dFn(Function):
 
     @staticmethod
@@ -454,15 +477,22 @@
 
 class MappingFn(Function):
 
+    pair_box = None
+
     @staticmethod
     def forward(ctx, z, labels, emb, slope, *wb):
         ctx.set_materialize_grads(False)
         ws, bs = wb[0::2], wb[1::2]
+        box = MappingFn.pair_box
         ys = []
         y = nv.linear_fwd(z, ws[0], bs[0], nv.ACT_LRELU, slope, emb=emb, labels=labels)
         ys.append(y)
-        for w, b in zip(ws[1:], bs[1:]):
-            y = nv.linear_fwd(y, w, b, nv.ACT_LRELU, slope)
+        for l, (w, b) in enumerate(zip(ws[1:], bs[1:]), 1):
+            if box is not None and l == len(ws) - 1:
+                y, yy = nv.linear_fwd(y, w, b, nv.ACT_LRELU, slope, twice=True)
+                box.append(yy)
+            else:
+                y = nv.linear_fwd(y, w, b, nv.ACT_LRELU, slope)
             ys.append(y)
         ctx.slope, ctx.nl = slope, len(ws)
         ctx.sinks = [(_sink_of(w), _sink_of(b)) for w, b in zip(ws, bs)] + [(_sink_of(emb), None)]
@@ -618,17 +648,42 @@
     @once_differentiable
     def backward(ctx, gout):
         (wvec,) = ctx.saved_tensors
-        if getattr(gout, "_kg_unit_seed", False):
-            key = (float(ctx.lam), str(gout.device), gout.dtype)
-            lam = _LAM_CONSTS.get(key)
-            if lam is None and not (gout.is_cuda and torch.cuda.is_current_stream_capturing()):
-                lam = _LAM_CONSTS[key] = torch.full((), float(ctx.lam), dtype=gout.dtype, device=gout.device)
-            if lam is not None:
-                return wvec.view(ctx.shape), lam, None, None
-        return (wvec * gout).view(ctx.shape), gout * ctx.lam, None, None
+        return _critic_loss_grads(wvec, ctx.shape, ctx.lam, gout) + (None, None)
+
+
+def _critic_loss_grads(wvec, shape, lam_value: float, gout):
+    if getattr(gout, "_kg_unit_seed", False):
+        key = (float(lam_value), str(gout.device), gout.dtype)
+        lam = _LAM_CONSTS.get(key)
+        if lam is None and not (gout.is_cuda and torch.cuda.is_current_stream_capturing()):
+            lam = _LAM_CONSTS[key] = torch.full((), float(lam_value), dtype=gout.dtype, device=gout.device)
+        if lam is not None:
+            return wvec.view(shape), lam
+    return (wvec * gout).view(shape), gout * lam_value
 
 
 _LAM_CONSTS: dict = {}
+
+
+class PenaltyCriticLoss(Function):
+
+    @staticmethod
+    def forward(ctx, g, both, wvec, lam: float):
+        ctx.set_materialize_grads(False)
+        nrm, gp, d_loss = nv.gp_fwd_loss(g, both, wvec, lam)
+        ctx.lam, ctx.shape = lam, both.shape
+        ctx.save_for_backward(g, nrm, wvec)
+        return gp, d_loss
+
+    @staticmethod
+    @once_differentiable
+    def backward(ctx, ggp, gdl):
+        g, nrm, wvec = ctx.saved_tensors
+        gboth, gout = None, ggp
+        if gdl is not None:
+            gboth, glam = _critic_loss_grads(wvec, ctx.shape, ctx.lam, gdl)
+            gout = glam if ggp is None else ggp + glam
+        return (None if gout is None else nv.gp_bwd(g, nrm, gout)), gboth, None, None
 
 
 def time_scatter(g, stride: int, T_in: int):
diff --git a/kinetic-gan_amd/wgan_gp.py b/kinetic-gan_amd/wgan_gp.py
--- a/kinetic-gan_amd/wgan_gp.py
+++ b/kinetic-gan_amd/wgan_gp.py
@@ -142,13 +142,15 @@
         self.grad.zero_()
 
 
-def penalty_of(d_inter, inter, keep: Optional[dict] = None):
+def penalty_of(d_inter, inter, keep: Optional[dict] = None, loss=None):
     ones = _const_like(d_inter, 1.0)
     with ops.no_param_grads():
         (grads,) = torch.autograd.grad(outputs=d_inter, inputs=inter, grad_outputs=ones,
                                        create_graph=True, retain_graph=True, only_inputs=True)
     if keep is not None:
         keep["gp_grads"] = grads.detach()
+    if loss is not None:
+        return ops.PenaltyCriticLoss.apply(grads, *loss)
     return ops.GradPenalty.apply(grads)
 
 
@@ -248,7 +250,7 @@
             exact_bn = getattr(self.G, "_exact_bn_active", None) is not None and self.G._exact_bn_active()
             if self._share_mapping and hasattr(self.G, "synthesis_pair") and self.G.training and not exact_bn and \
                     ((noise is None) == (self._noise_g is None)):
-                w = self.G.mapping(z, labels)
+                w = self.G.mapping(z, labels, pair=True)
                 fake, self._fake_g = self.G.synthesis_pair(w, noise, self._noise_g)
             elif self._share_mapping and hasattr(self.G, "synthesis"):
                 self._w = self.G.mapping(z, labels)
@@ -258,8 +260,12 @@
                 with torch.no_grad():
                     fake = self.G(z, labels, noise=noise)
         if getattr(self.D, "use_trunk", False):
-            labels3 = torch.cat((labels, labels, labels), 0)
-            buf = nv.mix3(real, fake, alpha)
+            ends = ops.step_ends() and real.is_cuda
+            if ends and labels.dtype == torch.int64 and labels.dim() == 1:
+                buf, labels3 = nv.mix3(real, fake, alpha, labels=labels.contiguous())
+            else:
+                labels3 = torch.cat((labels, labels, labels), 0)
+                buf = nv.mix3(real, fake, alpha)
             inter = buf[2 * n:].requires_grad_(True)
             key = (n, str(buf.device))
             if self._wvec is None or self._wvec[0] != key:
@@ -269,6 +275,10 @@
                                                  promised_grad=self._wvec[1] if promise else None)
             real_v, fake_v = both[:n], both[n:]
             out = {"fake": fake, "real_validity": real_v, "fake_validity": fake_v}
+            if ends and n <= nv.GP_ONE_LAUNCH_MAX and both.is_contiguous():
+                gp, out["d_loss"] = penalty_of(d_inter, inter, out, loss=(both, self._wvec[1], float(self.lambda_gp)))
+                out["gradient_penalty"] = gp
+                return out
             gp = penalty_of(d_inter, inter, out)
             out["gradient_penalty"] = gp
             out["d_loss"] = ops.CriticLoss.apply(both, gp, self._wvec[1], float(self.lambda_gp))
@@ -325,9 +335,16 @@
     def g_backward(self, fake, labels):
         self.fD.set_requires_grad(False)
         try:
-            v = self.D(fake, labels)
+            box = {}
+            if ops.step_ends() and fake.is_cuda:
+                with ops.head_loss(-1.0 / fake.shape[0]) as box:
+                    v = self.D(fake, labels)
+            else:
+                v = self.D(fake, labels)
             seed = _const_like(v, -1.0 / v.numel())
-            g_loss = torch.dot(v.detach().reshape(-1), seed.reshape(-1))
+            g_loss = box.get("loss") if v.numel() == fake.shape[0] else None
+            if g_loss is None:
+                g_loss = torch.dot(v.detach().reshape(-1), seed.reshape(-1))
             v.backward(seed)
         finally:
             self.fD.set_requires_grad(True)
```

Result: no change. 20910 samples/s, median of 6 (+0.9%).
